# lidq92/LBDRN-MSIC

Hardware: AMD Instinct MI355X
Metric: Mpixels/s encode+decode (and bpp/PSNR parity) on D2/K5/bc64/nl2 (higher is better)
Workload: dtype f32; 1 GPU; synthetic 8-band 2048x2048 uint16 tile per step, K=5 D=2 bc=64 nl=2 bs=8192 e=10 (BASELINE.json configs[1] by default); encode fit + 16-bit weight truncation + decode; tiles_per_gpu=50, tiles_in_flight_per_gpu=4, tiles_per_launch=2, parallelism=image-sharded x1

## Files before the change

lbdrn-msic_amd/csrc/cabi.hip:

```cpp
#include <string>

#include "common.hpp"

namespace lbdrn {
const char* last_error();
bool mfma_train_supported(const lbdrn_geom& g, const lbdrn_net& net, int bs = 0);
int mfma_train_step_features(const lbdrn_geom& g, const lbdrn_net& net);
bool mfma_train_takes_groups(const lbdrn_geom& g, const lbdrn_net& net);
size_t mfma_train_workspace(const lbdrn_geom& g, const lbdrn_net& net, int bs);
int mfma_train_prepare(const lbdrn_geom& g, const lbdrn_net& net, const uint16_t* img,
                       const uint16_t* msb, int bs, void* ws, size_t ws_bytes, hipStream_t s);
int mfma_train_epoch(const lbdrn_geom& g, const lbdrn_net& net, const uint16_t* img,
                     const uint16_t* msb, const int64_t* perm, int64_t n, int bs, float* params,
                     float* m, float* v, int64_t step0, double lr, float* losses, void* ws,
                     size_t ws_bytes, hipStream_t s, bool alone);
int train_profile_mode(int mode);
size_t randperm_workspace(int64_t n, int count);
size_t plane_bound(int C, int H, int W);
size_t plane_workspace(int C, int H, int W);
int plane_encode(const uint16_t* planes, int C, int H, int W, void* body, size_t body_cap, uint64_t* body_bytes,
                 void* ws, size_t ws_bytes, hipStream_t s);
int plane_decode(const void* body, size_t body_bytes, int C, int H, int W, uint16_t* planes, int* status, void* ws,
                 size_t ws_bytes, hipStream_t s);
int64_t mt19937_jump_poly(int segment, uint32_t* out);
// ... 163 lines not shown
    if (check_geom(g) || check_net(net)) return 0;
    size_t a = generic_apply_workspace(*g, *net);
    size_t b = mfma_apply_supported(*g, *net) ? mfma_apply_workspace(*g, *net) : 0;
    return a > b ? a : b;
}

static int pick_apply(const lbdrn_geom* g, const lbdrn_net* net, int32_t path, bool* use_mfma)
{
    const bool ok = mfma_apply_supported(*g, *net);
    if (path == LBDRN_PATH_MFMA && !ok) {
        set_error("fused MFMA apply kernel does not support bc=%d nl=%d C=%d D=%d", net->bc, net->nl,
                  net->C, g->D);
        return LBDRN_E_UNSUPPORTED;
    }
    LBDRN_REQUIRE(path >= LBDRN_PATH_AUTO && path <= LBDRN_PATH_MFMA, "unknown path %d", path);
    *use_mfma = ok && path != LBDRN_PATH_GENERIC;
    return 0;
}

int lbdrn_decode_fused(const lbdrn_geom* g, const lbdrn_net* net, const uint16_t* msb,
                       const float* params, uint16_t* out, float* y_out, void* workspace,
                       size_t workspace_bytes, int32_t path, void* stream)
{
    if (int rc = check_geom(g)) return rc;
    if (int rc = check_net(net)) return rc;
    if (int rc = net_matches(g, net)) return rc;
    LBDRN_REQUIRE(msb && params && out, "msb, params and out must not be null");
    NEED_DEVICE();
    bool use_mfma = false;
    if (int rc = pick_apply(g, net, path, &use_mfma)) return rc;
    if (int rc = workspace_fits("apply", workspace, workspace_bytes, lbdrn_apply_workspace(g, net))) return rc;
    if (use_mfma)
        return mfma_decode(*g, *net, msb, params, out, y_out, workspace, workspace_bytes, (hipStream_t)stream);
    return generic_decode(*g, *net, msb, params, out, y_out, workspace, workspace_bytes, (hipStream_t)stream);
}

int lbdrn_eval_sse(const lbdrn_geom* g, const lbdrn_net* net, const uint16_t* img, const uint16_t* msb,
                   const float* params, double* sse, void* workspace, size_t workspace_bytes,
                   int32_t path, void* stream)
{
    if (int rc = check_geom(g)) return rc;
    if (int rc = check_net(net)) return rc;
    if (int rc = net_matches(g, net)) return rc;
    LBDRN_REQUIRE(img && msb && params && sse, "img, msb, params and sse must not be null");
    NEED_DEVICE();
    const bool background = (path & LBDRN_EVAL_BACKGROUND) != 0, fast = (path & LBDRN_EVAL_FAST) != 0;
    const bool x16 = fast && (path & LBDRN_EVAL_X16) != 0;
    path &= ~(LBDRN_EVAL_BACKGROUND | LBDRN_EVAL_FAST | LBDRN_EVAL_X16);
    bool use_mfma = false;
    if (int rc = pick_apply(g, net, path, &use_mfma)) return rc;
    if (int rc = workspace_fits("apply", workspace, workspace_bytes, lbdrn_apply_workspace(g, net))) return rc;
    if (use_mfma)
        return mfma_eval_sse(*g, *net, img, msb, params, sse, workspace, workspace_bytes, background, fast, x16,
                             (hipStream_t)stream);
    return generic_eval_sse(*g, *net, img, msb, params, sse, workspace, workspace_bytes, (hipStream_t)stream);
}

size_t lbdrn_train_workspace(const lbdrn_geom* g, const lbdrn_net* net, int32_t batch_size)
{
    if (check_geom(g) || check_net(net) || batch_size < 1) return 0;
    size_t a = generic_train_workspace(*net, batch_size);
    size_t b = mfma_train_supported(*g, *net, batch_size) ? mfma_train_workspace(*g, *net, batch_size) : 0;
    return a > b ? a : b;
}

int lbdrn_train_prepare(const lbdrn_geom* g, const lbdrn_net* net, const uint16_t* img,
                        const uint16_t* msb, int32_t batch_size, void* workspace, size_t workspace_bytes,
                        int32_t path, void* stream)
{
    if (int rc = check_geom(g)) return rc;
    if (int rc = check_net(net)) return rc;
    if (int rc = net_matches(g, net)) return rc;
    LBDRN_REQUIRE(img && msb && batch_size >= 1, "null pointer or bad batch size");
    LBDRN_REQUIRE(path >= LBDRN_PATH_AUTO && path <= LBDRN_PATH_MFMA, "unknown path %d", path);
    NEED_DEVICE();
    const bool ok = mfma_train_supported(*g, *net, batch_size);
    if (path == LBDRN_PATH_MFMA && !ok) {
        set_error("fused MFMA train kernel does not support this shape or minibatch size");
        return LBDRN_E_UNSUPPORTED;
    }
    if (int rc = workspace_fits("train", workspace, workspace_bytes, lbdrn_train_workspace(g, net, batch_size))) return rc;
    if (ok && path != LBDRN_PATH_GENERIC)
        return mfma_train_prepare(*g, *net, img, msb, batch_size, workspace, workspace_bytes, (hipStream_t)stream);
    return 0;
}

int lbdrn_train_epoch(const lbdrn_geom* g, const lbdrn_net* net, const uint16_t* img,
                      const uint16_t* msb, const int64_t* perm, int64_t n, int32_t batch_size,
                      float* params, float* exp_avg, float* exp_avg_sq, int64_t adam_step0, double lr,
                      float* losses, void* workspace, size_t workspace_bytes, int32_t path,
                      void* stream)
{
    if (int rc = check_geom(g)) return rc;
    if (int rc = check_net(net)) return rc;
    if (int rc = net_matches(g, net)) return rc;
    LBDRN_REQUIRE(img && msb && perm && params && exp_avg && exp_avg_sq, "null pointer");
    LBDRN_REQUIRE(n >= 0 && batch_size >= 1 && adam_step0 >= 0, "bad n/batch_size/adam_step0");
    NEED_DEVICE();
    const bool alone = (path & LBDRN_TRAIN_ALONE) != 0;
    path &= ~LBDRN_TRAIN_ALONE;
    const bool ok = mfma_train_supported(*g, *net, batch_size);
    if (path == LBDRN_PATH_MFMA && !ok) {
        set_error("fused MFMA train kernel does not support this shape or minibatch size");
        return LBDRN_E_UNSUPPORTED;
    }
    LBDRN_REQUIRE(path >= LBDRN_PATH_AUTO && path <= LBDRN_PATH_MFMA, "unknown path %d", path);
    if (int rc = workspace_fits("train", workspace, workspace_bytes, lbdrn_train_workspace(g, net, batch_size))) return rc;
    if (ok && path != LBDRN_PATH_GENERIC)
        return mfma_train_epoch(*g, *net, img, msb, perm, n, batch_size, params, exp_avg, exp_avg_sq,
                                adam_step0, lr, losses, workspace, workspace_bytes, (hipStream_t)stream, alone);
    return generic_train_epoch(*g, *net, img, msb, perm, n, batch_size, params, exp_avg, exp_avg_sq,
                               adam_step0, lr, losses, workspace, workspace_bytes, (hipStream_t)stream);
}

int lbdrn_train_group_max(void) { return 4; }

int32_t lbdrn_train_group_size(const lbdrn_geom* g, const lbdrn_net* net)
{
    if (!g || !net) return 1;
    return mfma_train_takes_groups(*g, *net) ? lbdrn_train_group_max() : 1;
}

int32_t lbdrn_train_step_features(const lbdrn_geom* g, const lbdrn_net* net)
{
    if (!g || !net) return 0;
    return mfma_train_step_features(*g, *net);
}

int lbdrn_train_epoch_group(int32_t count, const lbdrn_geom* const* g, const lbdrn_net* net, const uint16_t* const* img,
                            const uint16_t* const* msb, const int64_t* const* perm, int64_t n, int32_t batch_size,
                            float* const* params, float* const* exp_avg, float* const* exp_avg_sq, int64_t adam_step0,
                            double lr, float* const* losses, void* const* workspace, size_t workspace_bytes, int32_t path,
                            void* stream)
{
    LBDRN_REQUIRE(count >= 1 && count <= lbdrn_train_group_max(), "group of %d fits (1..%d)", count, lbdrn_train_group_max());
    LBDRN_REQUIRE(g && img && msb && perm && params && exp_avg && exp_avg_sq && workspace, "null pointer array");
    if (int rc = check_net(net)) return rc;
    for (int f = 0; f < count; ++f) {
        LBDRN_REQUIRE(g[f] && img[f] && msb[f] && perm[f] && params[f] && exp_avg[f] && exp_avg_sq[f], "null pointer (fit %d)", f);
        if (int rc = check_geom(g[f])) return rc;
        if (int rc = net_matches(g[f], net)) return rc;
        LBDRN_REQUIRE(g[f]->C == g[0]->C && g[f]->H == g[0]->H && g[f]->W == g[0]->W && g[f]->K == g[0]->K &&
                      g[f]->D == g[0]->D && g[f]->P == g[0]->P && g[f]->use_colors == g[0]->use_colors &&
                      g[f]->relative == g[0]->relative, "the fits of a group must have one shape (fit %d differs)", f);
    }
    LBDRN_REQUIRE(n >= 0 && batch_size >= 1 && adam_step0 >= 0, "bad n/batch_size/adam_step0");
    const int32_t hint = count == 1 ? (path & LBDRN_TRAIN_ALONE) : 0;
    path &= ~LBDRN_TRAIN_ALONE;
    LBDRN_REQUIRE(path >= LBDRN_PATH_AUTO && path <= LBDRN_PATH_MFMA, "unknown path %d", path);
    NEED_DEVICE();
    for (int f = 0; f < count; ++f)
        if (int rc = workspace_fits("train", workspace[f], workspace_bytes, lbdrn_train_workspace(g[f], net, batch_size))) return rc;
    if (count > 1 && path != LBDRN_PATH_GENERIC && mfma_train_supported(*g[0], *net, batch_size)) {
        const int rc = mfma_train_epoch_group(count, *g[0], *net, perm, n, batch_size, params, exp_avg, exp_avg_sq,
                                              adam_step0, lr, losses, workspace, workspace_bytes, (hipStream_t)stream, false);
        if (rc != LBDRN_E_UNSUPPORTED) return rc;
    }
    for (int f = 0; f < count; ++f)
        if (int rc = lbdrn_train_epoch(g[f], net, img[f], msb[f], perm[f], n, batch_size, params[f], exp_avg[f],
                                       exp_avg_sq[f], adam_step0, lr, losses ? losses[f] : nullptr, workspace[f],
                                       workspace_bytes, path | hint, stream))
            return rc;
    return 0;
}

int lbdrn_train_profile_mode(int32_t mode)
{
    LBDRN_REQUIRE(mode >= 0 && mode <= 5, "mode must be 0 .. 5");
    return train_profile_mode(mode);
}

size_t lbdrn_randperm_workspace(int64_t n, int32_t count)
{
    if (n < 0 || count < 1 || count > 32) return 0;
    return randperm_workspace(n, count);
}

int lbdrn_randperm(const uint64_t* seeds, int32_t count, int64_t n, int64_t* perm, void* workspace,
                   size_t workspace_bytes, void* stream)
{
    LBDRN_REQUIRE(n >= 0 && (perm || n == 0), "bad n or null output");
    NEED_DEVICE();
    return randperm_batch(seeds, count, n, perm, workspace, workspace_bytes, (hipStream_t)stream);
}

int64_t lbdrn_mt19937_jump_poly(int32_t segment, uint32_t* poly624)
{
    LBDRN_REQUIRE(poly624, "null output");
    return mt19937_jump_poly(segment, poly624);
}

size_t lbdrn_plane_bound(int32_t C, int32_t H, int32_t W) { return plane_bound(C, H, W); }
size_t lbdrn_plane_workspace(int32_t C, int32_t H, int32_t W) { return plane_workspace(C, H, W); }

int lbdrn_plane_encode(const uint16_t* planes, int32_t C, int32_t H, int32_t W, void* body, size_t body_capacity,
                       uint64_t* body_bytes, void* workspace, size_t workspace_bytes, void* stream)
{
    LBDRN_REQUIRE(C >= 1 && H >= 1 && W >= 1 && C <= 65535, "bad raster geometry");
    NEED_DEVICE();
    return plane_encode(planes, C, H, W, body, body_capacity, body_bytes, workspace, workspace_bytes,
                        (hipStream_t)stream);
}

int lbdrn_plane_decode(const void* body, size_t body_bytes, int32_t C, int32_t H, int32_t W, uint16_t* planes,
                       int32_t* status, void* workspace, size_t workspace_bytes, void* stream)
{
    LBDRN_REQUIRE(C >= 1 && H >= 1 && W >= 1 && C <= 65535, "bad raster geometry");
    NEED_DEVICE();
    return plane_decode(body, body_bytes, C, H, W, planes, status, workspace, workspace_bytes, (hipStream_t)stream);
}

int64_t lbdrn_jp2k_block_count(int32_t C, int32_t H, int32_t W) { return jp2k_block_count(C, H, W); }
size_t lbdrn_jp2k_bound(int32_t C, int32_t H, int32_t W) { return jp2k_bound(C, H, W); }
size_t lbdrn_jp2k_workspace(int32_t C, int32_t H, int32_t W) { return jp2k_workspace(C, H, W); }

int lbdrn_jp2k_encode(const uint16_t* planes, int32_t C, int32_t H, int32_t W, int32_t bits, void* out, size_t capacity,
                      size_t* nbytes, void* workspace, size_t workspace_bytes, void* stream)
{
    if (int rc = device_ok()) return rc;
    return jp2k_encode(planes, C, H, W, bits, (uint8_t*)out, capacity, nbytes, workspace, workspace_bytes, (hipStream_t)stream);
}

size_t lbdrn_weights_bound(int64_t n) { return n < 0 ? 0 : weights_bound(n); }

int lbdrn_weights_encode(const float* values, int64_t n, int32_t precision, void* out, size_t capacity, size_t* nbytes)
{
    LBDRN_REQUIRE((values || n == 0) && out && nbytes && n >= 0 && n < ((int64_t)1 << 32), "null pointer or bad count");
    LBDRN_REQUIRE(precision == 0 || (precision >= 2 && precision <= 32), "precision %d is not 0 or 2..32", precision);
    return weights_encode(values, n, precision, (uint8_t*)out, capacity, nbytes);
}

int lbdrn_weights_info(const void* stream, size_t nbytes, int64_t* n, int32_t* precision)
{
    LBDRN_REQUIRE(stream && n && precision, "null pointer");
    int prec = 0;
    const int rc = weights_info((const uint8_t*)stream, nbytes, n, &prec);
    *precision = prec;
    return rc;
}

int lbdrn_weights_decode(const void* stream, size_t nbytes, float* values, int64_t capacity)
{
    LBDRN_REQUIRE(stream && (values || capacity == 0) && capacity >= 0, "null pointer or bad capacity");
    return weights_decode((const uint8_t*)stream, nbytes, values, capacity);
}

int lbdrn_train_step(const lbdrn_net* net, const float* x, const float* t, int32_t B, float* params,
                     float* exp_avg, float* exp_avg_sq, int64_t adam_step, double lr,
                     int32_t apply_adam, float* loss, float* grads, void* workspace,
                     size_t workspace_bytes, void* stream)
{
    if (int rc = check_net(net)) return rc;
    LBDRN_REQUIRE(x && t && params, "x, t and params must not be null");
    LBDRN_REQUIRE(!apply_adam || (exp_avg && exp_avg_sq && adam_step >= 1), "Adam state missing or adam_step < 1");
    NEED_DEVICE();
    return generic_train_step(*net, x, t, B, params, exp_avg, exp_avg_sq, adam_step, lr, apply_adam,
                              loss, grads, workspace, workspace_bytes, (hipStream_t)stream);
}

}
```

lbdrn-msic_amd/csrc/common.hpp:

```cpp
#pragma once
#include <hip/hip_runtime.h>
#include <stdint.h>
#include <stdio.h>

#include <atomic>

#include "../../include/lbdrn_hip.h"

namespace lbdrn {

void set_error(const char* fmt, ...);

#define LBDRN_HIP_TRY(expr)                                                                  \
    do {                                                                                     \
        hipError_t e_ = (expr);                                                              \
        if (e_ != hipSuccess) {                                                              \
            ::lbdrn::set_error("%s failed: %s (%s:%d)", #expr, hipGetErrorString(e_), __FILE__, \
                               __LINE__);                                                    \
            return LBDRN_E_DEVICE;                                                           \
        }                                                                                    \
    } while (0)

#define LBDRN_REQUIRE(cond, ...)            \
    do {                                    \
        if (!(cond)) {                      \
            ::lbdrn::set_error(__VA_ARGS__); \
            return LBDRN_E_ARG;             \
        }                                   \
    } while (0)

#define LBDRN_LAUNCH_CHECK() LBDRN_HIP_TRY(hipGetLastError())

inline int64_t param_count(const lbdrn_net& n)
{
    int64_t c = 0;
    for (int l = 0; l < n.nl; ++l) c += (int64_t)n.bc * (l ? n.bc : n.F) + n.bc;
    return c + (int64_t)n.C * n.bc + n.C;
}
inline int64_t layer_offset(const lbdrn_net& n, int l)
{
    int64_t c = 0;
    for (int i = 0; i < l; ++i) c += (int64_t)n.bc * (i ? n.bc : n.F) + n.bc;
    return c;
}
inline int feature_dim(const lbdrn_geom& g)
{
    const int side = 2 * g.D + 1;
    return 2 * g.P + (g.use_colors ? g.C * side * side : 0);
}
inline size_t align_up(size_t x, size_t a) { return (x + a - 1) / a * a; }

template <class K>
static int configure_lds_once(K kern, int bytes, std::atomic<unsigned long long>& configured)
{
    int dev = 0;
    (void)hipGetDevice(&dev);
    const unsigned long long bit = 1ull << (dev & 63);
    if (!(configured.load(std::memory_order_relaxed) & bit)) {
        LBDRN_HIP_TRY(hipFuncSetAttribute(reinterpret_cast<const void*>(kern), hipFuncAttributeMaxDynamicSharedMemorySize, bytes));
        configured.fetch_or(bit, std::memory_order_relaxed);
    }
    return 0;
}

int check_geom(const lbdrn_geom* g);
int check_net(const lbdrn_net* n);

int generic_split_bits(const uint16_t* img, int C, int H, int W, int K, uint16_t* msb, int32_t* mx,
                       hipStream_t s);
int generic_labels(const uint16_t* img, int C, int H, int W, int K, const int64_t* idx, int64_t n,
                   float* labels, hipStream_t s);
int generic_features(const lbdrn_geom& g, const uint16_t* msb, const int64_t* idx, int64_t n,
                     int64_t first, float* out, hipStream_t s);
size_t generic_forward_workspace(const lbdrn_net& net, int64_t B);
int generic_forward(const lbdrn_net& net, const float* params, const float* x, int64_t B, float* y,
                    void* ws, size_t ws_bytes, hipStream_t s);
size_t generic_apply_workspace(const lbdrn_geom& g, const lbdrn_net& net);
int generic_decode(const lbdrn_geom& g, const lbdrn_net& net, const uint16_t* msb,
                   const float* params, uint16_t* out, float* y_out, void* ws, size_t ws_bytes,
                   hipStream_t s);
int generic_eval_sse(const lbdrn_geom& g, const lbdrn_net& net, const uint16_t* img,
                     const uint16_t* msb, const float* params, double* sse, void* ws,
                     size_t ws_bytes, hipStream_t s);
size_t generic_train_workspace(const lbdrn_net& net, int B);
int generic_train_step(const lbdrn_net& net, const float* x, const float* t, int B, float* params,
                       float* m, float* v, int64_t adam_step, double lr, int apply_adam,
                       float* loss, float* grads, void* ws, size_t ws_bytes, hipStream_t s);
size_t generic_tape_bytes(const lbdrn_net& net, int64_t B);
size_t generic_backward_workspace(const lbdrn_net& net, int64_t B);
int generic_forward_tape(const lbdrn_net& net, const float* params, const float* x, int64_t B, float* y, void* tape,
                         size_t tape_bytes, hipStream_t s);
int generic_backward(const lbdrn_net& net, const float* params, const float* x, int64_t B, const void* tape,
                     size_t tape_bytes, const float* y, const float* dy, float* grads, float* dx, void* ws,
                     size_t ws_bytes, hipStream_t s);
int generic_train_epoch(const lbdrn_geom& g, const lbdrn_net& net, const uint16_t* img,
                        const uint16_t* msb, const int64_t* perm, int64_t n, int bs, float* params,
                        float* m, float* v, int64_t step0, double lr, float* losses, void* ws,
                        size_t ws_bytes, hipStream_t s);

bool mfma_apply_supported(const lbdrn_geom& g, const lbdrn_net& net);
size_t mfma_apply_workspace(const lbdrn_geom& g, const lbdrn_net& net);
int mfma_decode(const lbdrn_geom& g, const lbdrn_net& net, const uint16_t* msb, const float* params,
                uint16_t* out, float* y_out, void* ws, size_t ws_bytes, hipStream_t s);
int mfma_eval_sse(const lbdrn_geom& g, const lbdrn_net& net, const uint16_t* img,
                  const uint16_t* msb, const float* params, double* sse, void* ws, size_t ws_bytes,
                  bool background, bool fast, bool x16, hipStream_t s);

int mfma_train_epoch_group(int count, const lbdrn_geom& g, const lbdrn_net& net, const int64_t* const* perm, int64_t n,
                           int bs, float* const* params, float* const* m, float* const* v, int64_t step0, double lr,
                           float* const* losses, void* const* ws, size_t ws_bytes, hipStream_t s, bool alone);

}
```

lbdrn-msic_amd/csrc/train_mfma.hip:

```cpp
#include <cmath>
#include <cstdlib>
#include <utility>
#include <vector>

#include "common.hpp"
#include "lbdrn_math.hpp"

namespace lbdrn {

typedef float f32x4 __attribute__((ext_vector_type(4)));

constexpr int MAX_GROUP = 4;
constexpr int TB = 32;
constexpr int TBC = 64;
constexpr int HP = 68;
constexpr int TP = 36;
constexpr int OP = 20;
constexpr int RED_SLICES = 8;
constexpr int RED_LANES = 32;
constexpr int SLAB_ROT = 4;
constexpr int TRAIN_THREADS = 512;

constexpr int WB = 64;
constexpr int WAVE_THREADS = 256;
constexpr int WOP = 16;
__host__ __device__ constexpr int wave_xp(int LQ) { return LQ == 16 ? 80 : LQ == 32 ? 144 : LQ == 48 || LQ == 52 ? 208 : 272; }
constexpr int TBC_W = 64;
constexpr int WPT = 68;

struct FeatMap {
    int Fe;
    int zP, zs2, zc;
};
__host__ __device__ __forceinline__ int feat_of_slot(int j, const FeatMap& m)
{
    if (m.zs2 == 0 || j < m.zP) return j;
    const int cj = j - m.zP, c = cj / (m.zs2 - 1), r = cj - c * (m.zs2 - 1);
    return m.zP + c * m.zs2 + r + (r >= m.zc ? 1 : 0);
}
__host__ __device__ __forceinline__ int slot_of_feat(int k, const FeatMap& m)
{
    if (m.zs2 == 0 || k < m.zP) return k;
    const int ck = k - m.zP, c = ck / m.zs2, r = ck - c * m.zs2;
    if (r == m.zc) return -1;
    return m.zP + c * (m.zs2 - 1) + r - (r > m.zc ? 1 : 0);
}

static FeatMap centre_skipping_map(const lbdrn_geom& g, const lbdrn_net& net)
{
    const int side = 2 * g.D + 1;
    if (g.use_colors && g.relative && g.D > 0 && net.F == 2 * g.P + g.C * side * side)
        return FeatMap{net.F - g.C, 2 * g.P, side * side, g.D * side + g.D};
    return FeatMap{net.F, 0, 0, 0};
}

constexpr int STEP_TILE = 0;
constexpr int STEP_STREAM = 2;

struct TrainPlan {
    FeatMap fm;
    int LQ;
    int XP;
    int NT0;
    int RP;
    int64_t NP;
    int64_t offW[5], offB[5];
    int pk_w0, pk_wh, pk_wl, pack_floats;
    int wave;
    int pk_wht, pk_wlt;
    int w_dp, w_df;
    int wave_lds_floats;
    int sl_hid, sl_out, sl_bias, slab_floats;
    int lds_x, lds_xt, lds_h, lds_ht, lds_z, lds_zt, lds_zo, lds_zot, lds_pix, lds_red, lds_floats;
};

#define STREAM_INSTANCES(X) \
    X(16, 1, 0) X(16, 2, 0)              \
    X(24, 1, 0) X(24, 2, 0) X(24, 2, 6)  \
    X(32, 1, 0) X(32, 2, 0)              \
    X(48, 1, 0) X(48, 2, 0) X(48, 2, 12) \
    X(52, 1, 0)             X(52, 2, 13) \
    X(64, 1, 0) X(64, 2, 0) X(64, 2, 16)
#define SPLIT_INSTANCES(X) X(24, 6) X(48, 12) X(64, 16) X(96, 24)
constexpr int SPLIT_WIDE_LQ = 96;
#define TILE_INSTANCES(X) X(16, 3) X(32, 3) X(52, 3)

#define X(LQ, NL, NT0C) if (lq == LQ && nl == NL && nt0 == NT0C) return NT0C;
constexpr int stream_nt0c(int lq, int nl, int nt0) { STREAM_INSTANCES(X) return 0; }
#undef X
#define X(LQ, NL, NT0C) if (nl == NL && fe <= 4 * LQ) return LQ;
constexpr int stream_lq(int fe, int nl) { STREAM_INSTANCES(X) return 0; }
#undef X
#define X(LQ, NT0C) if (lq == LQ) return NT0C;
constexpr int split_nt0c(int lq) { SPLIT_INSTANCES(X) return 0; }
#undef X
#define X(LQ, NL) static_assert(4 * LQ % 16 == 0, "16 NT0 > XP: dW0's last strip passes the X row"); if (nl == NL && F <= 4 * LQ && RP <= 4 * LQ + 4) return LQ;
constexpr int tile_lq(int F, int RP, int nl) { TILE_INSTANCES(X) return 0; }
#undef X

__host__ __device__ constexpr int stream_rp(int LQ);
static int stream_lds_total(int LQ, int NL);

static bool make_train_plan(const lbdrn_geom& g, const lbdrn_net& net, TrainPlan* out)
{
    if ((net.act != LBDRN_ACT_SINE && net.act != LBDRN_ACT_RELU) || net.bc != TBC || net.nl < 1 || net.nl > 3 || net.C > 16 || net.F < 1) return false;
    if (net.act == LBDRN_ACT_RELU && net.nl > 2) return false;
    TrainPlan p;
    p.wave = net.nl <= 2 ? STEP_STREAM : STEP_TILE;
    if (p.wave == STEP_STREAM) {
        p.fm = centre_skipping_map(g, net);
        p.LQ = stream_lq(p.fm.Fe, net.nl);
        if (!p.LQ && net.nl == 2 && p.fm.Fe <= 4 * SPLIT_WIDE_LQ) p.LQ = SPLIT_WIDE_LQ;
        if (!p.LQ) return false;
        p.NT0 = p.LQ == SPLIT_WIDE_LQ ? split_nt0c(SPLIT_WIDE_LQ) : (p.fm.Fe + 15) / 16;
        p.RP = stream_rp(p.LQ);
        p.wave_lds_floats = p.LQ == SPLIT_WIDE_LQ ? 0 : stream_lds_total(p.LQ, net.nl);
    } else {
        p.fm = FeatMap{net.F, 0, 0, 0};
        p.RP = (net.F + net.C + 3) / 4 * 4;
        p.LQ = tile_lq(net.F, p.RP, net.nl);
        if (!p.LQ) return false;
        p.NT0 = (net.F + 15) / 16;
        p.wave_lds_floats = 0;
    }
    p.XP = 4 * p.LQ + 4;
    p.NP = param_count(net);
    int64_t o = 0;
    for (int l = 0; l < net.nl; ++l) {
        int nin = l ? TBC : net.F;
        p.offW[l] = o; o += (int64_t)TBC * nin;
        p.offB[l] = o; o += TBC;
    }
    p.offW[net.nl] = o; o += (int64_t)net.C * TBC;
    p.offB[net.nl] = o;
    int k = 0;
    p.pk_w0 = k; k += 4 * p.LQ * 64;
    p.pk_wh = k; k += (net.nl - 1) * 4 * 16 * 64;
    p.pk_wl = k; k += 16 * 64;
    p.pk_wht = k; k += (net.nl - 1) * 4 * 16 * 64;
    p.pk_wlt = k; k += 16 * 64;
    p.pack_floats = k;
    p.w_dp = p.w_df = 0;
    int s = 4 * p.NT0 * 256;
    p.sl_hid = s; s += (net.nl - 1) * 16 * 256;
    p.sl_out = s; s += 4 * 256;
    p.sl_bias = s; s += net.nl * TBC + 16;
    p.slab_floats = (s + 127) / 128 * 128;
    int f = 0;
    p.lds_x = f; f += TB * p.XP;
    p.lds_xt = f; f += 16 * p.NT0 * TP;
    p.lds_h = f; f += net.nl * TB * HP;
    p.lds_ht = f; f += net.nl * TBC * TP;
    p.lds_z = f; f += net.nl * TB * HP;
    p.lds_zt = f; f += net.nl * TBC * TP;
    p.lds_zo = f; f += TB * OP;
    p.lds_zot = f; f += 16 * TP;
    p.lds_pix = f; f += TB;
    p.lds_red = f; f += 16;
    p.lds_floats = f;
    if (p.wave == STEP_TILE && (size_t)f * 4 > 160 * 1024) return false;
    *out = p;
    return true;
}

struct WidePlan;
static bool make_wide_plan(const lbdrn_geom& g, const lbdrn_net& net, WidePlan* out);
static bool wide_supported(const lbdrn_geom& g, const lbdrn_net& net);
static size_t wide_workspace(const lbdrn_geom& g, const lbdrn_net& net, int bs);

static bool slabs_addressable(const TrainPlan& p, int bs);

bool mfma_train_supported(const lbdrn_geom& g, const lbdrn_net& net, int bs)
{
    TrainPlan p;
    if (make_train_plan(g, net, &p)) return bs <= 0 || slabs_addressable(p, bs);
    return wide_supported(g, net);
}

bool mfma_train_takes_groups(const lbdrn_geom& g, const lbdrn_net& net)
{
    TrainPlan p;
    return make_train_plan(g, net, &p) && p.wave == STEP_STREAM;
}


struct TrainWsLayout {
    size_t off_rows, off_pack, off_slab, slab_bytes, off_loss, off_stage, stage_bytes, off_map, total;
};

static TrainWsLayout train_ws_layout(const lbdrn_geom& g, const lbdrn_net& net, const TrainPlan& p, int bs)
{
    TrainWsLayout L;
    size_t o = 0;
    L.off_rows = o; o += align_up((size_t)g.H * g.W * p.RP * sizeof(float), 256);
    L.off_pack = o; o += align_up((size_t)p.pack_floats * sizeof(float), 256);
    const size_t nwg = std::max((size_t)(bs + TB - 1) / TB, 2 * ((size_t)(bs + WB - 1) / WB));
    L.slab_bytes = align_up(nwg * (size_t)p.slab_floats * sizeof(float), 256);
    L.off_slab = o; o += SLAB_ROT * L.slab_bytes;
    L.off_loss = o; o += align_up(nwg * sizeof(double), 256);
    L.stage_bytes = align_up(align_up((size_t)bs, WB) * p.RP * sizeof(float), 256);
    L.off_stage = o; o += 2 * L.stage_bytes;
    L.off_map = o; o += align_up((size_t)p.slab_floats * 4 * sizeof(int), 256);
    L.total = o;
    return L;
}

static bool slabs_addressable(const TrainPlan& p, int bs)
{
    const size_t nwg = std::max((size_t)(bs + TB - 1) / TB, 2 * ((size_t)(bs + WB - 1) / WB));
    return nwg * (size_t)p.slab_floats * sizeof(float) < ((size_t)1 << 31);
}

size_t mfma_train_workspace(const lbdrn_geom& g, const lbdrn_net& net, int bs)
{
    TrainPlan p;
    if (!make_train_plan(g, net, &p)) return wide_workspace(g, net, bs);
    return train_ws_layout(g, net, p, bs).total;
}


__device__ __forceinline__ int row_source(int pos, int LQs, int F, int C, const FeatMap& fm)
{
    if (LQs == 0) return pos < fm.Fe ? feat_of_slot(pos, fm) : pos < fm.Fe + C ? F + (pos - fm.Fe) : -1;
    const int g = pos >> 4;
    if (g < (LQs >> 2)) {
        const int j = ((pos >> 2) & 3) * LQs + 4 * g + (pos & 3);
        return j < fm.Fe ? feat_of_slot(j, fm) : -1;
    }
    const int ch = pos - 4 * LQs;
    return ch < C ? F + ch : -1;
}

__global__ void __launch_bounds__(256)
    k_build_rows(lbdrn_geom g, int F, int RP, int LQs, FeatMap fm, const uint16_t* __restrict__ msb,
                 const uint16_t* __restrict__ img, float* __restrict__ rows)
{
    const int64_t HW = (int64_t)g.H * g.W;
    const int64_t e = (int64_t)blockIdx.x * blockDim.x + threadIdx.x;
    if (e >= HW * RP) return;
    const int64_t pix = e / RP;
    const int f = row_source((int)(e - pix * RP), LQs, F, g.C, fm);
    const int y = (int)(pix / g.W), x = (int)(pix - (int64_t)y * g.W);
    float v = 0.0f;
    if (f < 0) {
    } else if (f < g.P) {
        v = g.rowtab[(int64_t)y * g.P + f];
    } else if (f < 2 * g.P) {
        v = g.coltab[(int64_t)x * g.P + (f - g.P)];
    } else if (f < F) {
        const int side = 2 * g.D + 1;
        int cf = f - 2 * g.P;
        int c = cf / (side * side);
        int r = cf - c * side * side;
        int dy = r / side, dx = r - dy * side;
        const uint16_t* pl = msb + (int64_t)c * HW;
        const float mx = (float)g.msb_max;
        int yy = reflect_fast(y + dy - g.D, g.H), xx = reflect_fast(x + dx - g.D, g.W);
        v = (float)pl[(int64_t)yy * g.W + xx] / mx;
        if (g.relative && g.D > 0) v = v - (float)pl[pix] / mx;
    } else if (f < F + g.C) {
        const int mask = (1 << g.K) - 1;
        v = (float)((int)img[(int64_t)(f - F) * HW + pix] & mask) / (float)mask;
    }
    rows[e] = v;
}

constexpr int BR_TW = 32;
__global__ void __launch_bounds__(256)
    k_build_rows_tiled(lbdrn_geom g, int F, int RP, int LQs, FeatMap fm, const uint16_t* __restrict__ msb,
                       const uint16_t* __restrict__ img, float* __restrict__ rows)
{
    extern __shared__ float br_lds[];
    const int side = 2 * g.D + 1, SW = BR_TW + 2 * g.D;
    const int ncolor = F - 2 * g.P;
    float* tile = br_lds;
    int* nbo = reinterpret_cast<int*>(br_lds + g.C * side * SW);
    int* cto = nbo + ncolor;
    const int64_t HW = (int64_t)g.H * g.W;
    const int tiles_x = (g.W + BR_TW - 1) / BR_TW;
    const int y = blockIdx.x / tiles_x, x0 = (blockIdx.x - y * tiles_x) * BR_TW;
    const int tw = min(BR_TW, g.W - x0);
    const int tid = threadIdx.x;
    if (g.use_colors) {
        const float mx = (float)g.msb_max;
        const int total = g.C * side * SW;
        for (int e = tid; e < total; e += 256) {
            const int c = e / (side * SW), r = e - c * side * SW;
            const int sy = r / SW, sx = r - sy * SW;
            const int yy = reflect_fast(y + sy - g.D, g.H), xx = reflect_fast(min(x0 + sx - g.D, g.W - 1 + g.D), g.W);
            tile[e] = (float)msb[(int64_t)c * HW + (int64_t)yy * g.W + xx] / mx;
        }
        for (int k = tid; k < ncolor; k += 256) {
            const int c = k / (side * side), r = k - c * side * side;
            const int dy = r / side, dx = r - dy * side;
            nbo[k] = (c * side + dy) * SW + dx;
            cto[k] = (c * side + g.D) * SW + g.D;
        }
    }
    __syncthreads();
    const bool rel = g.relative && g.D > 0;
    int2* ptab = reinterpret_cast<int2*>(cto + ncolor);
    float* labs = reinterpret_cast<float*>(ptab + RP);
    {
        const int lmask = (1 << g.K) - 1;
        const float lmaskf = (float)lmask;
        for (int e = tid; e < g.C * BR_TW; e += 256) {
            const int c = e / BR_TW, px = e - c * BR_TW;
            labs[e] = (float)((int)img[(int64_t)c * HW + (int64_t)y * g.W + min(x0 + px, g.W - 1)] & lmask) / lmaskf;
        }
    }
    for (int pos = tid; pos < RP; pos += 256) {
        const int f = row_source(pos, LQs, F, g.C, fm);
        int2 t = make_int2(-1, 0);
        if (f < 0) {
        } else if (f < g.P) t = make_int2(-2, f);
        else if (f < 2 * g.P) t = make_int2(-3, f - g.P);
        else if (f < F) t = make_int2(nbo[f - 2 * g.P], rel ? cto[f - 2 * g.P] : -1);
        else if (f < F + g.C) t = make_int2(-4, f - F);
        ptab[pos] = t;
    }
    __syncthreads();
    float* out = rows + ((int64_t)y * g.W + x0) * RP;
    auto value = [&](int pos, int pix) -> float {
        const int2 t = ptab[pos];
        if (t.x >= 0) {
            const float nb = tile[t.x + pix];
            return t.y >= 0 ? nb - tile[t.y + pix] : nb;
        }
        if (t.x == -1) return 0.0f;
        if (t.x == -2) return g.rowtab[(int64_t)y * g.P + t.y];
        if (t.x == -3) return g.coltab[(int64_t)(x0 + pix) * g.P + t.y];
        return labs[t.y * BR_TW + pix];
    };
    if ((RP & 3) == 0) {
        const int RQ = RP >> 2;
        int pix = tid / RQ, pq = tid - pix * RQ;
        const int dp = 256 / RQ, dq = 256 - dp * RQ;
        while (pix < tw) {
            const int pos = 4 * pq;
            const float4 v = make_float4(value(pos, pix), value(pos + 1, pix), value(pos + 2, pix), value(pos + 3, pix));
            *reinterpret_cast<float4*>(out + (int64_t)pix * RP + pos) = v;
            pix += dp;
            pq += dq;
            if (pq >= RQ) { pq -= RQ; pix += 1; }
        }
    } else {
        int pix = tid / RP, pos = tid - pix * RP;
        const int dp = 256 / RP, df = 256 - dp * RP;
        for (int e = tid; pix < tw; e += 256) {
            out[e] = value(pos, pix);
            pix += dp;
            pos += df;
            if (pos >= RP) { pos -= RP; pix += 1; }
        }
    }
}

__device__ __forceinline__ int2 frag_pos(int64_t idx, const TrainPlan& p, int F, int nl, int C)
{
    if (idx < p.offB[0]) {
        int n = (int)(idx / F), k = slot_of_feat((int)(idx - (int64_t)n * F), p.fm);
        if (k < 0) return make_int2(-1, -1);
        int q = k / p.LQ, s = k - q * p.LQ;
        return make_int2(p.pk_w0 + ((((n >> 4) * (p.LQ >> 2) + (s >> 2)) * 64 + q * 16 + (n & 15)) * 4 + (s & 3)), -1);
    }
    for (int l = 1; l < nl; ++l) {
        if (idx >= p.offW[l] && idx < p.offB[l]) {
            int e = (int)(idx - p.offW[l]);
            int n = e >> 6, k = e & 63;
            if (!p.wave) {
                int sq = k & 15;
                return make_int2(p.pk_wh + (((((l - 1) * 4 + (n >> 4)) * 4 + (sq >> 2)) * 64 + (k >> 4) * 16 + (n & 15)) * 4 + (sq & 3)), -1);
            }
            const int fwd = p.pk_wh + (((((l - 1) * 4 + (n >> 4)) * 4 + (k >> 4)) * 64 + ((k >> 2) & 3) * 16 + (n & 15)) * 4 + (k & 3));
            const int bwd = p.pk_wht + (((((l - 1) * 4 + (k >> 4)) * 4 + (n >> 4)) * 64 + ((n >> 2) & 3) * 16 + (k & 15)) * 4 + (n & 3));
            return make_int2(fwd, bwd);
        }
    }
    if (idx >= p.offW[nl] && idx < p.offB[nl]) {
        int e = (int)(idx - p.offW[nl]);
        int c = e >> 6, k = e & 63;
        if (!p.wave) {
            int sq = k & 15;
            return make_int2(p.pk_wl + (((sq >> 2) * 64 + (k >> 4) * 16 + c) * 4 + (sq & 3)), -1);
        }
        const int fwd = p.pk_wl + (((k >> 4) * 64 + ((k >> 2) & 3) * 16 + c) * 4 + (k & 3));
        const int bwd = p.pk_wlt + (((k >> 4) * 64 + (c >> 2) * 16 + (k & 15)) * 4 + (c & 3));
        return make_int2(fwd, bwd);
    }
    return make_int2(-1, -1);
}

__device__ __forceinline__ int64_t slab_to_param(int e, const TrainPlan& p, int F, int nl, int C)
{
    if (e >= p.sl_bias) {
        int b = e - p.sl_bias;
        if (b < nl * TBC) return p.offB[b >> 6] + (b & 63);
        int ch = b - nl * TBC;
        return ch < C ? p.offB[nl] + ch : -1;
    }
    const int tile = e >> 8, lane = (e >> 2) & 63, r = e & 3;
    const int row = 4 * (lane >> 4) + r, col = lane & 15;
    if (e < p.sl_hid) {
        int w = tile / p.NT0, nt = tile - w * p.NT0;
        int k = 16 * nt + col;
        return k < p.fm.Fe ? p.offW[0] + (int64_t)(16 * w + row) * F + feat_of_slot(k, p.fm) : -1;
    }
    if (e < p.sl_out) {
        int t2 = tile - 4 * p.NT0;
        int l = 1 + (t2 >> 4), w = (t2 >> 2) & 3, nt = t2 & 3;
        return p.offW[l] + (int64_t)(16 * w + row) * TBC + 16 * nt + col;
    }
    int w = tile - (p.sl_out >> 8);
    return row < C ? p.offW[nl] + (int64_t)row * TBC + 16 * w + col : -1;
}

__global__ void __launch_bounds__(256)
    k_pack_train(const float* __restrict__ params, TrainPlan p, int F, int nl, int C, float* __restrict__ packed)
{
    int64_t idx = (int64_t)blockIdx.x * blockDim.x + threadIdx.x;
    if (idx >= p.NP) return;
    const int2 pos = frag_pos(idx, p, F, nl, C);
    if (pos.x >= 0) packed[pos.x] = params[idx];
    if (pos.y >= 0) packed[pos.y] = params[idx];
}

__global__ void __launch_bounds__(256)
    k_build_map(TrainPlan p, int F, int nl, int C, int4* __restrict__ map)
{
    int e = blockIdx.x * blockDim.x + threadIdx.x;
    if (e >= p.slab_floats) return;
    int64_t idx = e < p.sl_bias + nl * TBC + 16 ? slab_to_param(e, p, F, nl, C) : -1;
    const int2 pos = idx >= 0 ? frag_pos(idx, p, F, nl, C) : make_int2(-1, -1);
    map[e] = make_int4((int)idx, pos.x, pos.y, 0);
}

constexpr int RED_AUX = 0x00;
#ifdef LBDRN_TIMELINE
constexpr int TL_SLOTS = 2048;
__device__ __forceinline__ void timeline_store(unsigned long long* tl, int slot, bool drain)
{
    if (!tl || slot >= TL_SLOTS) return;
    unsigned long long t;
    if (drain) asm volatile("s_waitcnt vmcnt(0)" ::: "memory");
    asm volatile("s_memrealtime %0\n\ts_waitcnt lgkmcnt(0)" : "=s"(t)::"memory");
    tl[slot] = t;
}
#endif
struct ReduceFit {
    const float* slabs;
    float *params, *m, *v, *packed;
    const double* loss_part;
    float* loss_out;
};
struct ReduceArgs {
    ReduceFit fit[MAX_GROUP];
    unsigned long long* tl;
    int nloss;
};

__global__ void __launch_bounds__(RED_SLICES * RED_LANES)
    k_reduce_adam(ReduceArgs R, int nwg, int slab_floats, const int4* __restrict__ map, float step_size, float bc2_sqrt,
                  double loss_count, int pairs)
{
    __shared__ __attribute__((aligned(16))) float part[RED_SLICES][4 * RED_LANES];
    __builtin_amdgcn_s_setprio(3);
#ifdef LBDRN_TIMELINE
    if (threadIdx.x == 0 && blockIdx.x == 0 && blockIdx.y == 0) timeline_store(R.tl, 1, false);
#endif
    const ReduceFit& F = R.fit[blockIdx.y];
    const float* __restrict__ slabs = F.slabs;
    float* __restrict__ params = F.params;
    float* __restrict__ m = F.m;
    float* __restrict__ v = F.v;
    float* __restrict__ packed = F.packed;
    const int l16 = threadIdx.x % RED_LANES, slice = threadIdx.x / RED_LANES;
    const int base = blockIdx.x * (4 * RED_LANES);
    int4 me = make_int4(-1, -1, -1, 0);
    float pm = 0.f, pv = 0.f, pp = 0.f;
    if (threadIdx.x < 4 * RED_LANES) {
        me = map[base + threadIdx.x];
        const int j = me.x < 0 ? 0 : me.x;
        pm = m[j]; pv = v[j]; pp = params[j];
    }
    const int per = (nwg + RED_SLICES - 1) / RED_SLICES;
    const int w0 = slice * per, w1 = min(nwg, w0 + per);
    float4 acc = make_float4(0.f, 0.f, 0.f, 0.f);
    const __amdgpu_buffer_rsrc_t srs = __builtin_amdgcn_make_buffer_rsrc(const_cast<float*>(slabs), (short)0,
                                                                         (int)((size_t)nwg * (pairs ? 2 : 1) * slab_floats * 4), 0x00020000);
    const int voff = (base + 4 * l16) * 4;
    auto slab4 = [&](int slab) -> float4 {
        typedef int v4i __attribute__((ext_vector_type(4)));
        const v4i x = __builtin_amdgcn_raw_buffer_load_b128(srs, voff + slab * slab_floats * 4, 0, RED_AUX);
        return make_float4(__int_as_float(x[0]), __int_as_float(x[1]), __int_as_float(x[2]), __int_as_float(x[3]));
    };
    int w = w0;
    if (pairs) {
        for (; w + 8 <= w1; w += 8) {
            float4 t[8], o[8];
#pragma unroll
            for (int u = 0; u < 8; ++u) {
                t[u] = slab4(2 * (w + u));
                o[u] = slab4(2 * (w + u) + 1);
            }
#pragma unroll
            for (int u = 0; u < 8; ++u) { acc.x += t[u].x + o[u].x; acc.y += t[u].y + o[u].y; acc.z += t[u].z + o[u].z; acc.w += t[u].w + o[u].w; }
        }
        for (; w < w1; ++w) {
            const float4 t = slab4(2 * w), o = slab4(2 * w + 1);
            acc.x += t.x + o.x; acc.y += t.y + o.y; acc.z += t.z + o.z; acc.w += t.w + o.w;
        }
    }
    for (; w + 16 <= w1; w += 16) {
        float4 t[16];
#pragma unroll
        for (int u = 0; u < 16; ++u) t[u] = slab4(w + u);
#pragma unroll
        for (int u = 0; u < 16; ++u) { acc.x += t[u].x; acc.y += t[u].y; acc.z += t[u].z; acc.w += t[u].w; }
    }
    for (; w < w1; ++w) {
        const float4 t = slab4(w);
        acc.x += t.x; acc.y += t.y; acc.z += t.z; acc.w += t.w;
    }
    *reinterpret_cast<float4*>(&part[slice][4 * l16]) = acc;
    __syncthreads();
    if (threadIdx.x < 4 * RED_LANES && me.x >= 0) {
        float g = part[0][threadIdx.x];
#pragma unroll
        for (int s = 1; s < RED_SLICES; ++s) g += part[s][threadIdx.x];
        const float w1c = (float)(1.0 - 0.9), b2 = 0.999f, w2c = (float)(1.0 - 0.999), eps = 1e-8f;
        float mi = pm + w1c * (g - pm);
        float vi = pv * b2 + w2c * (g * g);
        float denom = __builtin_sqrtf(vi) / bc2_sqrt + eps;
        float pi = pp + (-step_size) * (mi / denom);
        m[me.x] = mi;
        v[me.x] = vi;
        params[me.x] = pi;
        if (me.y >= 0) packed[me.y] = pi;
        if (me.z >= 0) packed[me.z] = pi;
    }
    if (blockIdx.x == 0 && threadIdx.x == 0 && F.loss_out) {
        double s = 0.0;
        if (pairs) for (int k = 0; k + 1 < R.nloss; k += 2) s += F.loss_part[k] + F.loss_part[k + 1];
        else for (int k = 0; k < R.nloss; ++k) s += F.loss_part[k];
        *F.loss_out = (float)(s / loss_count);
    }
#ifdef LBDRN_TIMELINE
    __syncthreads();
    if (threadIdx.x == 0 && blockIdx.y == 0) timeline_store(R.tl, 514 + blockIdx.x, true);
#endif
}

static void launch_reduce(const ReduceArgs& R, int blocks, int count, bool pairs, int nwg, int slab_floats, const int4* map,
                          float step_size, float bc2_sqrt, double loss_count, hipStream_t s)
{
    k_reduce_adam<<<dim3((unsigned)blocks, (unsigned)count), RED_SLICES * RED_LANES, 0, s>>>(R, nwg, slab_floats, map, step_size, bc2_sqrt,
                                                                                            loss_count, pairs ? 1 : 0);
}


struct TrainFit {
    const float* rows;
    const int64_t* perm;
    const float* params;
    const float* packed;
    float* slabs;
    double* loss_part;
};
struct TrainArgs {
    lbdrn_net net;
    TrainPlan p;
    int64_t npix;
    int batch_n;
    float inv;
    TrainFit fit[MAX_GROUP];
    const float* stage_in;
    float* stage_out;
    const int64_t* perm_next;
    int next_n;
    int touch_row_bytes;
    unsigned long long* stamps;
    unsigned long long* tl;
};
constexpr int TOUCH_ROW_BYTES = 256;


#ifdef LBDRN_TRAIN_STAMPS
#define STAMP(k)                                                                        \
    do {                                                                                \
        __builtin_amdgcn_sched_barrier(0);                                              \
        asm volatile("s_memtime %0\n\ts_waitcnt lgkmcnt(0)" : "=s"(stamp[k])::"memory"); \
        __builtin_amdgcn_sched_barrier(0);                                              \
    } while (0)
#else
#define STAMP(k)
#endif

#define MFMA16(a, b, c) __builtin_amdgcn_mfma_f32_16x16x4f32((a), (b), (c), 0, 0, 0)

typedef int v4i32 __attribute__((ext_vector_type(4)));
struct WtBuf {
    __amdgpu_buffer_rsrc_t r;
    float* base;
    __device__ __forceinline__ WtBuf(float* p, size_t bytes) : base(p)
    {
        r = __builtin_amdgcn_make_buffer_rsrc(p, (short)0, (int)bytes, 0x00020000);
    }
    __device__ __forceinline__ void store_plain(int float_off, float a, float b, float c, float d) const
    {
        *reinterpret_cast<float4*>(base + float_off) = make_float4(a, b, c, d);
    }
    __device__ __forceinline__ void store(int float_off, float a, float b, float c, float d) const
    {
        v4i32 v = {__float_as_int(a), __float_as_int(b), __float_as_int(c), __float_as_int(d)};
        __builtin_amdgcn_raw_buffer_store_b128(v, r, float_off * 4, 0, 16 );
    }
};

template <int N>
__device__ __forceinline__ void lds_load(const float* src, float (&dst)[N])
{
#pragma unroll
    for (int g = 0; g < N / 4; ++g) {
        float4 v = *reinterpret_cast<const float4*>(src + 4 * g);
        dst[4 * g] = v.x; dst[4 * g + 1] = v.y; dst[4 * g + 2] = v.z; dst[4 * g + 3] = v.w;
    }
}

template <int LQ, int NL>
__global__ void __launch_bounds__(TRAIN_THREADS, 2) k_train_mfma(TrainArgs A)
{
    extern __shared__ __attribute__((aligned(16))) float lds[];
    const TrainPlan& p = A.p;
    const TrainFit& Ft = A.fit[0];
    const int tid = threadIdx.x, lane = tid & 63, w8 = tid >> 6;
    const int w = w8 & 3, st = w8 >> 2;
    const int i = lane & 15, q = lane >> 4;
    const int C = A.net.C, F = A.net.F;
    constexpr int XP = 4 * LQ + 4;
    float* Xs = lds + p.lds_x;
    float* XT = lds + p.lds_xt;
    float* Hs = lds + p.lds_h;
    float* HT = lds + p.lds_ht;
    float* Zs = lds + p.lds_z;
    float* ZT = lds + p.lds_zt;
    float* Zo = lds + p.lds_zo;
    float* ZoT = lds + p.lds_zot;
    int* pixs = reinterpret_cast<int*>(lds + p.lds_pix);
    double* red = reinterpret_cast<double*>(lds + p.lds_red);
    const int wg = blockIdx.x;
    const int first = wg * TB;
    const int nvalid = min(TB, A.batch_n - first);
    const int srow = i + 16 * st;
    float* slab = Ft.slabs + (size_t)wg * p.slab_floats;
    const WtBuf slabw(slab, (size_t)p.slab_floats * 4);
#ifdef LBDRN_TRAIN_STAMPS
    unsigned long long stamp[16] = {};
    asm volatile("s_memrealtime %0\n\ts_waitcnt lgkmcnt(0)" : "=s"(stamp[12])::"memory");
#endif
    STAMP(0);

    const bool staged = A.stage_in != nullptr;
    int64_t mypix = 0;
    if (!staged && tid < TB) mypix = Ft.perm[first + min(tid, nvalid - 1)];
    const int rs = tid >> 4, rsub = tid & 15;
    constexpr int NLD = (XP / 4 + 15) / 16;
    const int rp4 = p.RP >> 2;
    float4 v[NLD];
    if (staged) {
        const float* src = A.stage_in + ((size_t)wg * TB + rs) * p.RP;
#pragma unroll
        for (int u = 0; u < NLD; ++u) v[u] = *reinterpret_cast<const float4*>(src + 4 * min(rsub + 16 * u, rp4 - 1));
    }
    int64_t nextpix = -1;
    if (A.stage_out && first < A.next_n) nextpix = A.perm_next[min(first + rs, A.next_n - 1)];

    float a0[LQ];
    {
        const float4* wf0 = reinterpret_cast<const float4*>(Ft.packed + p.pk_w0) + (size_t)w * (LQ / 4) * 64 + lane;
#pragma unroll
        for (int g = 0; g < LQ / 4; ++g) {
            const float4 t = wf0[g * 64];
            a0[4 * g] = t.x; a0[4 * g + 1] = t.y; a0[4 * g + 2] = t.z; a0[4 * g + 3] = t.w;
        }
    }
    float ah[NL > 1 ? NL - 1 : 1][16];
#pragma unroll
    for (int l = 1; l < NL; ++l) {
        const float4* wfh = reinterpret_cast<const float4*>(Ft.packed + p.pk_wh) + (size_t)((l - 1) * 4 + w) * 4 * 64 + lane;
#pragma unroll
        for (int g = 0; g < 4; ++g) {
            const float4 t = wfh[g * 64];
            ah[l - 1][4 * g] = t.x; ah[l - 1][4 * g + 1] = t.y; ah[l - 1][4 * g + 2] = t.z; ah[l - 1][4 * g + 3] = t.w;
        }
    }
    float al[16];
    {
        const float4* wfl = reinterpret_cast<const float4*>(Ft.packed + p.pk_wl) + lane;
#pragma unroll
        for (int g = 0; g < 4; ++g) {
            const float4 t = wfl[g * 64];
            al[4 * g] = t.x; al[4 * g + 1] = t.y; al[4 * g + 2] = t.z; al[4 * g + 3] = t.w;
        }
    }
    float atl[4];
#pragma unroll
    for (int s = 0; s < 4; ++s) {
        int ch = 4 * q + s;
        atl[s] = ch < C ? Ft.params[p.offW[NL] + (int64_t)ch * TBC + 16 * w + i] : 0.0f;
    }
    float ath[NL > 1 ? NL - 1 : 1][16];
#pragma unroll
    for (int l = 1; l < NL; ++l)
#pragma unroll
        for (int s = 0; s < 16; ++s) ath[l - 1][s] = Ft.params[p.offW[l] + (int64_t)(16 * q + s) * TBC + 16 * w + i];
    f32x4 bias[NL];
#pragma unroll
    for (int l = 0; l < NL; ++l) {
        float4 b4 = *reinterpret_cast<const float4*>(Ft.params + p.offB[l] + 16 * w + 4 * q);
        bias[l][0] = b4.x; bias[l][1] = b4.y; bias[l][2] = b4.z; bias[l][3] = b4.w;
// ... 107 lines not shown
#pragma unroll
        for (int r = 0; r < 4; ++r) ZoT[(4 * q + r) * TP + srow] = dzo[r];
        for (int o = 32; o > 0; o >>= 1) lsum += __shfl_down(lsum, o);
        if (lane == 0) red[st] = lsum;
    }
    __syncthreads();
    if (tid == 0) Ft.loss_part[wg] = red[0] + red[1];
    STAMP(6);
    if (nextpix >= 0) {
        const WtBuf stw(A.stage_out + (size_t)wg * TB * p.RP, (size_t)TB * p.RP * 4);
#pragma unroll
        for (int u = 0; u < NLD; ++u) {
            const int c4 = rsub + 16 * u;
            if (c4 < rp4) stw.store(rs * p.RP + 4 * c4, vnext[u].x, vnext[u].y, vnext[u].z, vnext[u].w);
        }
    }

    auto backprop_store = [&](int l) {
        float dz[4];
#pragma unroll
        for (int r = 0; r < 4; ++r) dz[r] = (acc[r] * cs[l][r]) * 30.0f;
        *reinterpret_cast<float4*>(Zs + (size_t)l * TB * HP + srow * HP + 16 * w + 4 * q) =
            make_float4(dz[0], dz[1], dz[2], dz[3]);
#pragma unroll
        for (int r = 0; r < 4; ++r) ZT[(size_t)l * TBC * TP + (16 * w + 4 * q + r) * TP + srow] = dz[r];
    };

    {
        const f32x4 zero = {0.f, 0.f, 0.f, 0.f};
        acc = zero;
        float bz[4];
        lds_load<4>(Zo + srow * OP + 4 * q, bz);
#pragma unroll
        for (int s = 0; s < 4; ++s) acc = MFMA16(atl[s], bz[s], acc);
        backprop_store(NL - 1);
    }
    __syncthreads();
#pragma unroll
    for (int l = NL - 1; l >= 1; --l) {
        const f32x4 zero = {0.f, 0.f, 0.f, 0.f};
        acc = zero;
        float bz[16];
        lds_load<16>(Zs + (size_t)l * TB * HP + srow * HP + 16 * q, bz);
#pragma unroll
        for (int s = 0; s < 16; ++s) acc = MFMA16(ath[l - 1][s], bz[s], acc);
        backprop_store(l - 1);
        __syncthreads();
    }
    STAMP(7);

    auto grad_tiles = [&](const float* zt, const float* bt, int ntiles, int out, bool early) {
        float az[8];
        lds_load<8>(zt + (16 * w + i) * TP + 8 * q, az);
        for (int nt = st; nt < ntiles; nt += 4) {
            const int nt1 = nt + 2;
            const bool two = nt1 < ntiles;
            float b0[8], b1[8];
            lds_load<8>(bt + (16 * nt + i) * TP + 8 * q, b0);
            lds_load<8>(bt + (16 * (two ? nt1 : nt) + i) * TP + 8 * q, b1);
            const f32x4 zero = {0.f, 0.f, 0.f, 0.f};
            f32x4 g0 = zero, g1 = zero;
#pragma unroll
            for (int s = 0; s < 8; ++s) {
                g0 = MFMA16(az[s], b0[s], g0);
                g1 = MFMA16(az[s], b1[s], g1);
            }
            if (early) {
                slabw.store(out + ((w * ntiles + nt) * 64 + lane) * 4, g0[0], g0[1], g0[2], g0[3]);
                if (two) slabw.store(out + ((w * ntiles + nt1) * 64 + lane) * 4, g1[0], g1[1], g1[2], g1[3]);
            } else {
                slabw.store_plain(out + ((w * ntiles + nt) * 64 + lane) * 4, g0[0], g0[1], g0[2], g0[3]);
                if (two) slabw.store_plain(out + ((w * ntiles + nt1) * 64 + lane) * 4, g1[0], g1[1], g1[2], g1[3]);
            }
        }
    };
    grad_tiles(ZT, XT, p.NT0, 0, true);
    STAMP(10);
#pragma unroll
    for (int l = 1; l < NL; ++l)
        grad_tiles(ZT + (size_t)l * TBC * TP, HT + (size_t)(l - 1) * TBC * TP, 4, p.sl_hid + (l - 1) * 16 * 256, false);
    if (st == 0) {
        float az[8], bv[8];
        lds_load<8>(ZoT + i * TP + 8 * q, az);
        lds_load<8>(HT + (size_t)(NL - 1) * TBC * TP + (16 * w + i) * TP + 8 * q, bv);
        const f32x4 zero = {0.f, 0.f, 0.f, 0.f};
        f32x4 g0 = zero, g1 = zero;
#pragma unroll
        for (int s = 0; s < 8; s += 2) {
            g0 = MFMA16(az[s], bv[s], g0);
            g1 = MFMA16(az[s + 1], bv[s + 1], g1);
        }
        slabw.store_plain(p.sl_out + (w * 64 + lane) * 4, g0[0] + g1[0], g0[1] + g1[1], g0[2] + g1[2], g0[3] + g1[3]);
    }
    STAMP(11);
    for (int u = tid; u < NL * TBC + 16; u += TRAIN_THREADS) {
        float zz[TB];
        lds_load<TB>(u < NL * TBC ? ZT + (size_t)u * TP : ZoT + (size_t)(u - NL * TBC) * TP, zz);
        float v = 0.0f;
#pragma unroll
        for (int s = 0; s < TB; ++s) v += zz[s];
        slab[p.sl_bias + u] = v;
    }
    for (int u = p.sl_bias + NL * TBC + 16 + tid; u < p.slab_floats; u += TRAIN_THREADS) slab[u] = 0.0f;
    STAMP(8);
#ifdef LBDRN_TRAIN_STAMPS
    asm volatile("s_waitcnt vmcnt(0)" ::: "memory");
    STAMP(9);
    asm volatile("s_memrealtime %0\n\ts_waitcnt lgkmcnt(0)" : "=s"(stamp[13])::"memory");
    if (tid == 0 && A.stamps)
        for (int k = 0; k < 16; ++k) A.stamps[(size_t)wg * 16 + k] = stamp[k];
#endif
}

__device__ __forceinline__ float train_sigmoid(float z) { return fast_sigmoid(z); }
template <int ACT> __device__ __forceinline__ void train_act(float z, float& h, float& d);
template <int ACT> __device__ __forceinline__ float train_act_back(float dh, float d)
{
    if constexpr (ACT == LBDRN_ACT_RELU) return d != 0.0f ? dh : 0.0f;
    else return (dh * d) * 30.0f;
}
__device__ __forceinline__ void train_sincos(float x, float& sn, float& cs) { fast_sincos(x, sn, cs); }
template <int ACT> __device__ __forceinline__ void train_act(float z, float& h, float& d)
{
    if constexpr (ACT == LBDRN_ACT_RELU) { h = z > 0.0f ? z : 0.0f; d = z > 0.0f ? 1.0f : 0.0f; }
    else train_sincos(30.0f * z, h, d);
}

__device__ __forceinline__ float row_sum16(float x)
{
    x += __int_as_float(__builtin_amdgcn_update_dpp(0, __float_as_int(x), 0x111, 0xf, 0xf, true));
    x += __int_as_float(__builtin_amdgcn_update_dpp(0, __float_as_int(x), 0x112, 0xf, 0xf, true));
    x += __int_as_float(__builtin_amdgcn_update_dpp(0, __float_as_int(x), 0x114, 0xf, 0xf, true));
    x += __int_as_float(__builtin_amdgcn_update_dpp(0, __float_as_int(x), 0x118, 0xf, 0xf, true));
    return x;
}

__device__ __forceinline__ float wave_sum(float x)
{
    const int xi = __float_as_int(row_sum16(x));
    const float a = __int_as_float(__builtin_amdgcn_readlane(xi, 15)), b = __int_as_float(__builtin_amdgcn_readlane(xi, 31));
    const float c = __int_as_float(__builtin_amdgcn_readlane(xi, 47)), d = __int_as_float(__builtin_amdgcn_readlane(xi, 63));
    return (a + b) + (c + d);
}

static thread_local int g_prof_mode = 0;
int train_profile_mode(int mode)
{
    g_prof_mode = mode;
    return 0;
}

#include "train_stream.inc"

static int stream_lds_total(int LQ, int NL) { return stream_lds(LQ, NL).total; }
#define X(LQ, NL, NT0C) static_assert(stream_lds(LQ, NL).total * 4 <= 160 * 1024, "k_train_stream's LDS map passes 160 KB");
STREAM_INSTANCES(X)
#undef X

#include "train_split.inc"

#include "train_wide.inc"

int mfma_train_step_features(const lbdrn_geom& g, const lbdrn_net& net)
{
    TrainPlan p;
    if (make_train_plan(g, net, &p)) return p.fm.Fe;
    WidePlan wp;
    return make_wide_plan(g, net, &wp) ? wide_plan_features(wp) : net.F;
}

static bool wide_supported(const lbdrn_geom& g, const lbdrn_net& net)
{
    WidePlan p;
    return make_wide_plan(g, net, &p);
}
static size_t wide_workspace(const lbdrn_geom& g, const lbdrn_net& net, int bs)
{
    WidePlan p;
    if (!make_wide_plan(g, net, &p)) return 0;
    return wide_ws_layout(g, net, p, bs).total;
}


template <int LQ, int NL>
static int launch_train(const TrainArgs& A, int nwg, hipStream_t s)
{
    auto kern = k_train_mfma<LQ, NL>;
    const size_t lds_bytes = (size_t)A.p.lds_floats * 4;
    static std::atomic<unsigned long long> configured{0};
    if (int rc = configure_lds_once(kern, 160 * 1024, configured)) return rc;
    kern<<<nwg, TRAIN_THREADS, lds_bytes, s>>>(A);
    LBDRN_LAUNCH_CHECK();
    return 0;
}

template <int LQ, int NL, int NT0C, int ACT>
static int launch_stream(const TrainArgs& A, int nwg, int count, hipStream_t s)
{
    auto kern = k_train_stream<LQ, NL, STREAM_PD, NT0C, ACT>;
    static std::atomic<unsigned long long> configured{0};
    if (int rc = configure_lds_once(kern, A.p.wave_lds_floats * 4, configured)) return rc;
    kern<<<dim3((unsigned)nwg, (unsigned)count), STREAM_THREADS, (size_t)A.p.wave_lds_floats * 4, s>>>(A);
    LBDRN_LAUNCH_CHECK();
    return 0;
}

template <int LQ, int NT0C, int ACT>
static int launch_split(const TrainArgs& A, int nwg, int count, hipStream_t s)
{
    auto kern = k_train_split<LQ, NT0C, ACT>;
    constexpr int bytes = split_lds(LQ).total * 4;
    static std::atomic<unsigned long long> configured{0};
    if (int rc = configure_lds_once(kern, bytes, configured)) return rc;
    kern<<<dim3((unsigned)nwg, (unsigned)count), WAVE_THREADS, (size_t)bytes, s>>>(A);
    LBDRN_LAUNCH_CHECK();
    return 0;
}

static bool split_available(const TrainPlan& p, const lbdrn_net& net)
{
    return p.wave == STEP_STREAM && net.nl == 2 && split_nt0c(p.LQ) == p.NT0;
}
static bool split_only(const TrainPlan& p) { return p.LQ == SPLIT_WIDE_LQ; }

static int dispatch_train(const TrainArgs& A, int nwg, int count, bool split, hipStream_t s)
{
    const TrainPlan& p = A.p;
    const int nl = A.net.nl, nt0c = stream_nt0c(p.LQ, nl, p.NT0);
    const bool relu = A.net.act == LBDRN_ACT_RELU;
#define ACTS(launch, ...) return relu ? launch<__VA_ARGS__, LBDRN_ACT_RELU>(A, nwg, count, s) : launch<__VA_ARGS__, LBDRN_ACT_SINE>(A, nwg, count, s);
#define SPLIT(lq, c) if (split && p.LQ == lq && p.NT0 == c) ACTS(launch_split, lq, c)
#define STREAM(lq, n, c) if (!split && p.wave == STEP_STREAM && p.LQ == lq && nl == n && nt0c == c) ACTS(launch_stream, lq, n, c)
#define TILE(lq, n) if (!split && p.wave == STEP_TILE && p.LQ == lq && nl == n) return launch_train<lq, n>(A, nwg, s);
    SPLIT_INSTANCES(SPLIT) STREAM_INSTANCES(STREAM) TILE_INSTANCES(TILE)
#undef ACTS
#undef SPLIT
#undef STREAM
#undef TILE
    set_error("no fused step is built for LQ = %d, nl = %d, NT0 = %d%s", p.LQ, nl, p.NT0, split ? " (k_train_split)" : "");
    return LBDRN_E_UNSUPPORTED;
}

int mfma_train_prepare(const lbdrn_geom& g, const lbdrn_net& net, const uint16_t* img,
                       const uint16_t* msb, int bs, void* ws, size_t ws_bytes, hipStream_t s)
{
    TrainPlan p;
    size_t need = 0, off_rows = 0;
    int LQs = 0;
    if (make_train_plan(g, net, &p)) {
        const TrainWsLayout L = train_ws_layout(g, net, p, bs);
        need = L.total; off_rows = L.off_rows;
        if (p.wave == STEP_STREAM) LQs = p.LQ;
    } else {
        WidePlan wp;
        if (!make_wide_plan(g, net, &wp)) {
            set_error("shape not supported by the MFMA train kernels");
            return LBDRN_E_UNSUPPORTED;
        }
        const WideWsLayout L = wide_ws_layout(g, net, wp, bs);
        need = L.total; off_rows = L.off_rows;
        p.RP = wp.RP;
        p.fm = wp.fm;
    }
    if (!ws || ws_bytes < need) {
        set_error("train workspace too small: %zu < %zu", ws_bytes, need);
        return LBDRN_E_WORKSPACE;
    }
    float* rows = (float*)((char*)ws + off_rows);
    const int64_t total = (int64_t)g.H * g.W * p.RP;
    LBDRN_REQUIRE((total + 255) / 256 < ((int64_t)1 << 31), "image too large for one launch");
    const int side = 2 * g.D + 1;
    const size_t ncol = (size_t)std::max(net.F - 2 * g.P, 0);
    const size_t tile_lds = ((size_t)g.C * side * (BR_TW + 2 * g.D) + 2 * ncol + 2 * (size_t)p.RP + (size_t)g.C * BR_TW) * 4;
    const int64_t nblk = (int64_t)g.H * ((g.W + BR_TW - 1) / BR_TW);
    if (tile_lds <= 48 * 1024 && g.D < g.H && g.D < g.W && nblk < ((int64_t)1 << 31)) {
        k_build_rows_tiled<<<(unsigned)nblk, 256, tile_lds, s>>>(g, net.F, p.RP, LQs, p.fm, msb, img, rows);
    } else {
        k_build_rows<<<(unsigned)((total + 255) / 256), 256, 0, s>>>(g, net.F, p.RP, LQs, p.fm, msb, img, rows);
    }
    LBDRN_LAUNCH_CHECK();
    return 0;
}


int mfma_train_epoch_group(int count, const lbdrn_geom& g, const lbdrn_net& net, const int64_t* const* perm, int64_t n,
                           int bs, float* const* params, float* const* m, float* const* v, int64_t step0, double lr,
                           float* const* losses, void* const* ws, size_t ws_bytes, hipStream_t s, bool alone)
{
    TrainArgs A;
    if (!make_train_plan(g, net, &A.p)) {
        if (count != 1) { set_error("groups of fits run on the bc = 64 fused step only"); return LBDRN_E_UNSUPPORTED; }
        return wide_train_epoch(g, net, perm[0], n, bs, params[0], m[0], v[0], step0, lr, losses ? losses[0] : nullptr,
                                ws[0], ws_bytes, s);
    }
    if (count < 1 || count > MAX_GROUP || (count > 1 && A.p.wave != STEP_STREAM)) {
        set_error("a group of %d fits is not supported by this shape's train kernel", count);
        return LBDRN_E_UNSUPPORTED;
    }
    if (!slabs_addressable(A.p, bs)) {
        set_error("minibatch of %d rows: one step's gradient slabs pass 2 GiB, the fused step does not address them", bs);
        return LBDRN_E_UNSUPPORTED;
    }
    const TrainWsLayout L = train_ws_layout(g, net, A.p, bs);
    if (ws_bytes < L.total) {
        set_error("train workspace too small: %zu < %zu", ws_bytes, L.total);
        return LBDRN_E_WORKSPACE;
    }
    A.net = net; A.npix = (int64_t)g.H * g.W;
    ReduceArgs R;
    for (int f = 0; f < MAX_GROUP; ++f) {
        const int k = f < count ? f : 0;
        if (!ws[k]) { set_error("null train workspace"); return LBDRN_E_WORKSPACE; }
        float* packed = (float*)((char*)ws[k] + L.off_pack);
        A.fit[f].rows = (float*)((char*)ws[k] + L.off_rows);
        A.fit[f].params = params[k];
        A.fit[f].packed = packed;
        A.fit[f].slabs = (float*)((char*)ws[k] + L.off_slab);
        A.fit[f].loss_part = (double*)((char*)ws[k] + L.off_loss);
        A.fit[f].perm = perm[k];
        R.fit[f].slabs = A.fit[f].slabs; R.fit[f].params = params[k]; R.fit[f].m = m[k]; R.fit[f].v = v[k];
        R.fit[f].packed = packed; R.fit[f].loss_part = A.fit[f].loss_part; R.fit[f].loss_out = nullptr;
        if (f < count) {
            LBDRN_HIP_TRY(hipMemsetAsync(packed, 0, (size_t)A.p.pack_floats * sizeof(float), s));
            k_pack_train<<<(unsigned)((A.p.NP + 255) / 256), 256, 0, s>>>(params[k], A.p, net.F, net.nl, net.C, packed);
            LBDRN_LAUNCH_CHECK();
        }
    }
    int4* map = (int4*)((char*)ws[0] + L.off_map);
    k_build_map<<<(unsigned)((A.p.slab_floats + 255) / 256), 256, 0, s>>>(A.p, net.F, net.nl, net.C, map);
    LBDRN_LAUNCH_CHECK();
    float* stage[2] = {(float*)((char*)ws[0] + L.off_stage), (float*)((char*)ws[0] + L.off_stage + L.stage_bytes)};
    A.stamps = nullptr;
#ifdef LBDRN_TRAIN_STAMPS
    const int max_wg = (bs + TB - 1) / TB;
    LBDRN_HIP_TRY(hipMalloc(&A.stamps, (size_t)max_wg * 8 * 16 * sizeof(unsigned long long)));
#endif
    A.tl = nullptr; R.tl = nullptr;
#ifdef LBDRN_TIMELINE
    const int tl_steps = (int)((n + bs - 1) / bs);
    unsigned long long* tl_buf = nullptr;
    {
        LBDRN_HIP_TRY(hipMalloc(&tl_buf, (size_t)tl_steps * TL_SLOTS * sizeof(unsigned long long)));
        LBDRN_HIP_TRY(hipMemset(tl_buf, 0, (size_t)tl_steps * TL_SLOTS * sizeof(unsigned long long)));
    }
#endif
    const int rows_per_wg = A.p.wave == STEP_STREAM ? WB : TB;
    const bool split = (alone && count == 1 && split_available(A.p, net)) || split_only(A.p);
    const int red_blocks = A.p.slab_floats / (4 * RED_LANES);
    int64_t step = step0;
    int si = 0;
    for (int64_t first = 0; first < n; first += bs, ++si) {
        const int B = (int)std::min<int64_t>(bs, n - first);
        const int nwg = (B + rows_per_wg - 1) / rows_per_wg;
        for (int f = 0; f < MAX_GROUP; ++f) {
            const int k = f < count ? f : 0;
            A.fit[f].perm = perm[k] + first;
            R.fit[f].loss_out = (f < count && losses && losses[k]) ? losses[k] + si : nullptr;
        }
        A.batch_n = B;
        for (int f = 0; f < MAX_GROUP; ++f) {
            const int k = f < count ? f : 0;
            A.fit[f].slabs = (float*)((char*)ws[k] + L.off_slab + (size_t)(si % SLAB_ROT) * L.slab_bytes);
            R.fit[f].slabs = A.fit[f].slabs;
        }
#ifdef LBDRN_TIMELINE
        A.tl = tl_buf + (size_t)TL_SLOTS * si; R.tl = A.tl;
#endif
        A.inv = 1.0f / ((float)B * (float)net.C);
        const int64_t nextB = std::max<int64_t>(0, std::min<int64_t>(bs, n - first - bs));
        A.stage_in = si > 0 ? stage[si & 1] : nullptr;
        A.stage_out = nextB > 0 ? stage[(si + 1) & 1] : nullptr;
        if (A.p.wave == STEP_STREAM) A.stage_in = nullptr, A.stage_out = nullptr;
        A.perm_next = perm[0] + first + bs;
        A.next_n = (int)nextB;
        A.touch_row_bytes = (alone && count == 1) ? TOUCH_ROW_BYTES : 0;
        const bool split_now = split && (B >= 2 || split_only(A.p));
        auto train_launch = [&]() { return dispatch_train(A, split_now ? 2 * nwg : nwg, count, split_now, s); };
        if (int rc = train_launch()) return rc;
        if (g_prof_mode == 2)
            if (int rc = train_launch()) return rc;
        ++step;
        const double bc1 = 1.0 - std::pow(0.9, (double)step), bc2 = 1.0 - std::pow(0.999, (double)step);
        R.nloss = split_now ? 2 * nwg : nwg;
        if (g_prof_mode != 3 && g_prof_mode != 4)
                launch_reduce(R, red_blocks, count, split_now, nwg, A.p.slab_floats, map, (float)(lr / bc1), (float)std::sqrt(bc2), (double)B * net.C, s);
        if (g_prof_mode == 1) {
            ReduceArgs R0 = R;
            for (int f = 0; f < MAX_GROUP; ++f) R0.fit[f].loss_out = nullptr;
            launch_reduce(R0, red_blocks, count, split_now, nwg, A.p.slab_floats, map, 0.0f, (float)std::sqrt(bc2), (double)B * net.C, s);
        }
        LBDRN_LAUNCH_CHECK();
    }
#ifdef LBDRN_TIMELINE
    {
        LBDRN_HIP_TRY(hipStreamSynchronize(s));
        std::vector<unsigned long long> h((size_t)tl_steps * TL_SLOTS);
        LBDRN_HIP_TRY(hipMemcpy(h.data(), tl_buf, h.size() * sizeof(unsigned long long), hipMemcpyDeviceToHost));
        (void)hipFree(tl_buf);
        double tr = 0, g1 = 0, rd = 0, g2 = 0; int cnt = 0;
        auto last = [&](int k, int lo, int hi) { unsigned long long m = 0; for (int j = lo; j < hi; ++j) m = std::max(m, h[(size_t)k * TL_SLOTS + j]); return m; };
        for (int k = 8; k + 1 < tl_steps; ++k) {
            const unsigned long long ts = h[(size_t)k * TL_SLOTS], rs = h[(size_t)k * TL_SLOTS + 1], te = last(k, 2, 514), re = last(k, 514, TL_SLOTS);
            const unsigned long long ts2 = h[(size_t)(k + 1) * TL_SLOTS];
            tr += (double)(te - ts); g1 += (double)((long long)(rs - te)); rd += (double)(re - rs); g2 += (double)((long long)(ts2 - re));
            ++cnt;
        }
        const double u = 0.01 / std::max(cnt, 1);
        fprintf(stderr, "[lbdrn timeline] per step over %d steps: train first start -> last end %.2f us | -> reduce starts %.2f | reduce %.2f | -> next train starts %.2f | step %.2f us\n",
                cnt, tr * u, g1 * u, rd * u, g2 * u, (tr + g1 + rd + g2) * u);
    }
#endif
#ifdef LBDRN_TRAIN_STAMPS
    if (A.p.wave == STEP_STREAM) {
        LBDRN_HIP_TRY(hipStreamSynchronize(s));
        const int nw = ((int)std::min<int64_t>(bs, n) + rows_per_wg - 1) / rows_per_wg * 4 * count * (split ? 2 : 1);
        std::vector<unsigned long long> h((size_t)nw * 16);
        LBDRN_HIP_TRY(hipMemcpy(h.data(), A.stamps, h.size() * sizeof(unsigned long long), hipMemcpyDeviceToHost));
        (void)hipFree(A.stamps);
        double d[14] = {}, clk = 0, span = 0;
        unsigned long long t0min = ~0ull, t1max = 0;
        for (int k = 0; k < nw; ++k) {
            for (int j = 1; j <= 13; ++j) d[j] += (double)(h[k * 16 + j] - h[k * 16 + j - 1]);
            clk += (double)(h[k * 16 + 13] - h[k * 16 + 0]) / (double)(h[k * 16 + 15] - h[k * 16 + 14]) * 100.0;
            span += (double)(h[k * 16 + 13] - h[k * 16 + 0]);
            t0min = std::min(t0min, h[k * 16 + 14]);
            t1max = std::max(t1max, h[k * 16 + 15]);
        }
        if (split)
            fprintf(stderr, "[lbdrn stamps, split kernel] clock %.0f MHz; wave lifetime %.0f cycles; first start -> last end %.2f us; "
                            "mean cycles: requests out %.0f | layer 0 (waits for W0 and the rows in it) %.0f | act0 %.0f | barrier, h0 read %.0f | hidden + act1 %.0f | "
                            "barrier, h1 read %.0f | out + loss %.0f | dh1, dz1 parked %.0f | barrier, dh0, dz0 parked %.0f | barrier, gradient operands read %.0f | "
                            "gradient products, stores, bias sums %.0f | drain %.0f\n",
                    clk / nw, span / nw, (double)(t1max - t0min) / 100.0, d[1] / nw, d[2] / nw, d[3] / nw, d[4] / nw, d[5] / nw, d[6] / nw,
                    d[7] / nw, d[8] / nw, d[9] / nw, d[10] / nw, (d[11] + d[12]) / nw, d[13] / nw);
        else
        fprintf(stderr, "[lbdrn stamps, stream kernel] clock %.0f MHz; wave lifetime %.0f cycles; first start -> last end %.2f us; "
                        "mean cycles: indices + first requests out %.0f | first stage landed %.0f | layer 0 under the stream %.0f | all landed, barrier %.0f | "
                        "act0 %.0f | hidden+act %.0f | out+loss %.0f | backward %.0f | barrier 3 %.0f | dW0 strips %.0f | dW tail+hidden %.0f | "
                        "bias sums %.0f | drain %.0f\n",
                clk / nw, span / nw, (double)(t1max - t0min) / 100.0, d[1] / nw, d[2] / nw, d[3] / nw, d[4] / nw, d[5] / nw, d[6] / nw,
                d[7] / nw, d[8] / nw, d[9] / nw, d[10] / nw, d[11] / nw, d[12] / nw, d[13] / nw);
    } else {
        LBDRN_HIP_TRY(hipStreamSynchronize(s));
        std::vector<unsigned long long> h((size_t)max_wg * 16);
        LBDRN_HIP_TRY(hipMemcpy(h.data(), A.stamps, h.size() * sizeof(unsigned long long), hipMemcpyDeviceToHost));
        (void)hipFree(A.stamps);
        double sum[12] = {}, d10 = 0, d11 = 0, d8 = 0, clk = 0;
        for (int wq = 0; wq < max_wg; ++wq) {
            for (int k = 1; k < 10; ++k)
                if (k != 8) sum[k] += (double)(h[wq * 16 + k] - h[wq * 16 + (k == 9 ? 8 : k - 1)]);
            d10 += (double)(h[wq * 16 + 10] - h[wq * 16 + 7]);
            d11 += (double)(h[wq * 16 + 11] - h[wq * 16 + 10]);
            d8 += (double)(h[wq * 16 + 8] - h[wq * 16 + 11]);
            clk += (double)(h[wq * 16 + 9] - h[wq * 16 + 0]) / (double)(h[wq * 16 + 13] - h[wq * 16 + 12]) * 100.0;
        }
        fprintf(stderr, "[lbdrn stamps] in-kernel clock %.0f MHz; mean cycles/phase: perm %.0f rows %.0f L0 %.0f act0 %.0f "
                        "hidden %.0f out+loss %.0f backprop %.0f dW0 %.0f dWhid+out %.0f bias %.0f drain %.0f\n",
                clk / max_wg, sum[1] / max_wg, sum[2] / max_wg, sum[3] / max_wg, sum[4] / max_wg, sum[5] / max_wg,
                sum[6] / max_wg, sum[7] / max_wg, d10 / max_wg, d11 / max_wg, d8 / max_wg, sum[9] / max_wg);
    }
#endif
    return 0;
}

int mfma_train_epoch(const lbdrn_geom& g, const lbdrn_net& net, const uint16_t* img,
                     const uint16_t* msb, const int64_t* perm, int64_t n, int bs, float* params,
                     float* m, float* v, int64_t step0, double lr, float* losses, void* ws,
                     size_t ws_bytes, hipStream_t s, bool alone)
{
    return mfma_train_epoch_group(1, g, net, &perm, n, bs, &params, &m, &v, step0, lr, &losses, &ws, ws_bytes, s, alone);
}

}
```

lbdrn-msic_amd/csrc/train_split.inc:

```
constexpr int SPB = 32;
constexpr int SP_HP = 68;
constexpr int SP_OP = 20;
constexpr int SP_PT = 36;
constexpr int SP_SM = 40;

constexpr int SP_RING = 12;
__host__ __device__ constexpr bool split_ring(int LQ) { return LQ > 64; }
__host__ __device__ constexpr int split_w0_groups(int LQ) { return split_ring(LQ) ? SP_RING : LQ / 4; }
__host__ __device__ constexpr int split_small_through(int k, int SPI) { return k * SPI < SP_SM / 4 ? k * SPI : SP_SM / 4; }

struct SplitLds { int w0, sm, x, xt, h0, red, idx, bias, h1, e, zo, zt, total; };
__host__ __device__ constexpr SplitLds split_lds(int LQ)
{
    SplitLds L{};
    const int G0 = LQ / 4, RG = split_w0_groups(LQ);
    int o = 0;
    const int over = 2 * SPB * SP_HP + SPB * SP_OP + 2 * 64 * SP_PT;
    L.w0 = o; o += RG * 4 * 256 > over ? RG * 4 * 256 : over;
    L.sm = o; o += SP_SM * 256;
    L.xt = (G0 + 1) * SGP + 16;
    L.x = o; o += 2 * L.xt;
    L.h0 = o; o += SPB * SP_HP;
    L.red = o; o += 4 + 4 * 16 + 12;
    L.idx = o; o += 4 * 256;
    L.bias = o; o += 4 * 64;
    L.total = o;
    int a = L.w0;
    L.h1 = a; a += SPB * SP_HP;
    L.e = a; a += SPB * SP_HP;
    L.zo = a; a += SPB * SP_OP;
    L.zt = a; a += 2 * 64 * SP_PT;
    if (a > L.sm) L.total = -1;
    return L;
}

__device__ __forceinline__ float split_sum8(float x)
{
    x += __int_as_float(__builtin_amdgcn_update_dpp(0, __float_as_int(x), 0x111, 0xf, 0xf, true));
    x += __int_as_float(__builtin_amdgcn_update_dpp(0, __float_as_int(x), 0x112, 0xf, 0xf, true));
    x += __int_as_float(__builtin_amdgcn_update_dpp(0, __float_as_int(x), 0x118, 0xf, 0xf, true));
    return x;
}
__host__ __device__ constexpr int split_slot(int r) { return (r & ~5) | ((r & 1) << 2) | ((r >> 2) & 1); }

__host__ __device__ constexpr int split_row_requests(int lo, int hi, int u)
{
    int c = 0;
    for (int g = lo; g < hi; ++g) c += (g & 1) == u;
    return c;
}

template <int LQ, int NT0C, int ACT>
__global__ void __launch_bounds__(WAVE_THREADS, 1) k_train_split(TrainArgs A)
{
    extern __shared__ __attribute__((aligned(16))) float lds[];
    const TrainPlan& p = A.p;
    const TrainFit& F = A.fit[blockIdx.y];
    constexpr int NL = 2, G0 = LQ / 4, NGR = G0 + 1, HP = SP_HP, OP = SP_OP, PT = SP_PT, RPM = stream_rp(LQ);
    constexpr SplitLds L = split_lds(LQ);
    static_assert(L.total > 0 && L.total * 4 <= 160 * 1024, "LDS map does not fit");
    static_assert(16 * NT0C == 4 * LQ && G0 >= 4, "the first layer's strips fill its slots");
    constexpr int NFS = NT0C / 4, REM = NT0C % 4, NIT = NFS + REM, GA = split_w0_groups(LQ) / 2;
    static_assert(NFS >= 1 && REM <= 2, "strip counts of the shapes this is instantiated for");
    constexpr int SPI = (SP_SM / 4 + G0 - 2) / (G0 - 1);
    constexpr bool RING = split_ring(LQ);
    constexpr int RG = split_w0_groups(LQ), HR = RG / 2, W0B = RG - GA;
    static_assert(!RING || (G0 == 2 * RG && GA == HR), "the ring holds half of W_0, its quarters land one behind the other");
    const int tid = threadIdx.x, lane = tid & 63;
    const int wv = __builtin_amdgcn_readfirstlane(tid >> 6);
    const int st = wv >> 1, uh = wv & 1;
    const int i = lane & 15, q = lane >> 4;
    const int C = A.net.C;
    const float* W0s = lds + L.w0;
    const float* SMs = lds + L.sm;
    const float* Xs = lds + L.x;
    float* H0 = lds + L.h0;
    float* H1 = lds + L.h1;
    float* E = lds + L.e;
    float* Zo = lds + L.zo;
    float* ZT = lds + L.zt;
    float* red = lds + L.red;
    const unsigned lds0 = (unsigned)(size_t)(__attribute__((address_space(3))) void*)lds;
    const int wg = blockIdx.x, grp = wg >> 1, par = wg & 1;
    const int qb = (i >> 2) & 1, jr = (i & 3) + 4 * (i >> 3);
    const int rho = 16 * (2 * st + qb) + 2 * jr + par;
    const int grow = grp * WB + rho;
    const bool live = grow < A.batch_n;
    const int srow = 16 * st + i;
    const int sig = 8 * (2 * st + qb) + jr;
    const int t0 = 2 * uh;
    float* slab = F.slabs + (size_t)wg * p.slab_floats;
    const WtBuf slabw(slab, (size_t)p.slab_floats * 4);
#ifdef LBDRN_TRAIN_STAMPS
    unsigned long long stamp[16] = {};
    asm volatile("s_memrealtime %0\n\ts_waitcnt lgkmcnt(0)" : "=s"(stamp[14])::"memory");
#endif
#ifdef LBDRN_TIMELINE
    if (lane == 0 && wv == 0 && wg == 0 && blockIdx.y == 0) timeline_store(A.tl, 0, false);
#endif
    STAMP(0);

    {
        const void* a0 = F.perm; const void* a1 = F.params; const void* a2 = F.packed; const void* a3 = F.rows;
        int b0 = p.pk_w0, b1 = p.pk_wh, b2 = p.pk_wht, b3 = p.pk_wl, b4 = p.pk_wlt, b5 = A.batch_n;
        long long c0 = p.offB[0], c1 = p.offB[1], c2 = p.offB[2], c3 = A.npix;
        asm volatile("" ::"s"(a0), "s"(a1), "s"(a2), "s"(a3), "s"(b0), "s"(b1), "s"(b2), "s"(b3), "s"(b4), "s"(b5), "s"(c0), "s"(c1), "s"(c2), "s"(c3));
    }
    if constexpr (RING) {
        const int64_t* isrc = F.perm + min(grp * WB + lane, A.batch_n - 1);
        stream_dma_dword(reinterpret_cast<const float*>(isrc), lds0 + 4u * (unsigned)(L.idx + 256 * wv));
    } else {
        const int64_t* isrc = F.perm + min(grp * WB + 2 * (lane & 31), A.batch_n - 2);
        stream_dma(reinterpret_cast<const float*>(isrc), lds0 + 4u * (unsigned)(L.idx + 256 * wv));
    }
    {
        const int l = wv < 3 ? wv : 2, n = l < 2 ? 64 : C;
        const float* bsrc = F.params + p.offB[l] + min(lane, n - 1);
        stream_dma_dword(bsrc, lds0 + 4u * (unsigned)(L.bias + 64 * wv));
    }
    const float* fsrc = F.packed + lane * 4;
    auto w0_requests = [&](int g_lo, int g_hi) {
#pragma unroll
        for (int g = g_lo; g < g_hi; ++g)
            stream_dma(fsrc + p.pk_w0 + 256 * (wv * G0 + g), lds0 + 4u * (unsigned)(L.w0 + ((g % RG) * 4 + wv) * 256));
    };
    w0_requests(0, GA);
    stream_wait_vm<GA + 1>();
    int64_t raw;
    if constexpr (RING) {
        raw = reinterpret_cast<const int*>(lds + L.idx + 256 * wv)[min(grow, A.batch_n - 1) - grp * WB];
    } else {
        const int g = min(grow, A.batch_n - 1), l = (g - grp * WB) >> 1;
        const int pos = 2 * l + (g - min(grp * WB + 2 * l, A.batch_n - 2));
        raw = reinterpret_cast<const int64_t*>(lds + L.idx + 256 * wv)[pos];
    }
    const int pix = (int)(raw < 0 ? 0 : (raw >= A.npix ? A.npix - 1 : raw));
    const float* rsrc = F.rows + (size_t)__shfl(pix, 16 * q + split_slot(lane >> 2)) * RPM + 4 * (lane & 3);
    auto row_requests = [&](int g_lo, int g_hi) {
#pragma unroll
        for (int g = g_lo; g < g_hi; ++g)
            if ((g & 1) == uh) stream_dma(rsrc + 16 * g, lds0 + 4u * (unsigned)(L.x + st * L.xt + g * SGP));
    };
    row_requests(0, GA);
    w0_requests(GA, RG);
    row_requests(GA, NGR);
    auto small_request = [&](int b) {
        const int blk = 4 * b + wv;
        const int src = blk < 16 ? p.pk_wh + 256 * blk : blk < 32 ? p.pk_wht + 256 * (blk - 16) : blk < 36 ? p.pk_wl + 256 * (blk - 32) : p.pk_wlt + 256 * (blk - 36);
        stream_dma(fsrc + src, lds0 + 4u * (unsigned)(L.sm + 256 * blk));
    };
    long long touched = 0;
    if (A.next_n > 0 && wv == 0 && lane < 8) touched = F.perm[A.batch_n + min(grp * WB + 8 * lane, A.next_n - 1)];
    STAMP(1);
    constexpr int ROWS_B0 = split_row_requests(GA, NGR, 0), ROWS_B1 = split_row_requests(GA, NGR, 1);
    if (uh == 0) stream_wait_vm<W0B + ROWS_B0>(); else stream_wait_vm<W0B + ROWS_B1>();
    stream_barrier();
    STAMP(2);

    auto sel4 = [](const float4& x, int e) -> float { return e == 0 ? x.x : e == 1 ? x.y : e == 2 ? x.z : x.w; };
    f32x4 bias0[2], bias1[2], bias_last;
    {
        const float* B = lds + L.bias;
#pragma unroll
        for (int tt = 0; tt < 2; ++tt) {
            const float4 b4 = *reinterpret_cast<const float4*>(B + 16 * (t0 + tt) + 4 * q);
            const float4 c4 = *reinterpret_cast<const float4*>(B + 64 + 16 * (t0 + tt) + 4 * q);
            bias0[tt][0] = b4.x; bias0[tt][1] = b4.y; bias0[tt][2] = b4.z; bias0[tt][3] = b4.w;
            bias1[tt][0] = c4.x; bias1[tt][1] = c4.y; bias1[tt][2] = c4.z; bias1[tt][3] = c4.w;
        }
        const float4 l4 = *reinterpret_cast<const float4*>(B + 128 + 4 * q);
        bias_last[0] = 4 * q + 0 < C ? l4.x : 0.0f; bias_last[1] = 4 * q + 1 < C ? l4.y : 0.0f;
        bias_last[2] = 4 * q + 2 < C ? l4.z : 0.0f; bias_last[3] = 4 * q + 3 < C ? l4.w : 0.0f;
    }
    f32x4 acc[2] = {bias0[0], bias0[1]};
    {
        const float* wbase = W0s + t0 * 256 + lane * 4;
        const float* xbase = Xs + st * L.xt + (4 * split_slot(i) + q) * 4;
        float4 aq[2][2], bq[2];
        auto reads = [&](int g) {
            aq[g & 1][0] = *reinterpret_cast<const float4*>(wbase + (g % RG) * 1024);
            aq[g & 1][1] = *reinterpret_cast<const float4*>(wbase + (g % RG) * 1024 + 256);
            bq[g & 1] = *reinterpret_cast<const float4*>(xbase + g * SGP);
        };
        auto mfmas = [&](int g) {
#pragma unroll
            for (int e = 0; e < 4; ++e)
#pragma unroll
                for (int tt = 0; tt < 2; ++tt) acc[tt] = MFMA16(sel4(aq[g & 1][tt], e), sel4(bq[g & 1], e), acc[tt]);
        };
        reads(0);
#pragma unroll
        for (int g = 1; g < G0; ++g) {
            if (g == GA) {
                stream_wait_vm<((GA - 1) * SPI < SP_SM / 4 ? (GA - 1) * SPI : SP_SM / 4)>();
                stream_barrier();
            }
            if constexpr (RING) {
                if (g == GA + 1 || g == 2 * HR + 1) {
                    asm volatile("s_waitcnt lgkmcnt(0)" ::: "memory");
                    stream_barrier();
                    const int q0 = g == GA + 1 ? 2 * HR : 3 * HR;
                    w0_requests(q0, q0 + HR);
                }
                if (g == 2 * HR) {
                    stream_wait_vm<split_small_through(2 * HR - 1, SPI) - split_small_through(GA, SPI)>();
                    stream_barrier();
                }
                if (g == 3 * HR) {
                    stream_wait_vm<split_small_through(3 * HR - 1, SPI) - split_small_through(2 * HR, SPI)>();
                    stream_barrier();
                }
            }
#pragma unroll
            for (int b = (g - 1) * SPI; b < g * SPI; ++b)
                if (b < SP_SM / 4) small_request(b);
            reads(g);
            mfmas(g - 1);
#pragma unroll
            for (int k = 0; k < 3; ++k) {
                __builtin_amdgcn_sched_group_barrier(0x100, 1, 0);
                __builtin_amdgcn_sched_group_barrier(0x008, 2, 0);
            }
            __builtin_amdgcn_sched_group_barrier(0x008, 2, 0);
            __builtin_amdgcn_sched_barrier(0);
        }
        mfmas(G0 - 1);
        __builtin_amdgcn_sched_barrier(0);
    }
    const float4 lab = *reinterpret_cast<const float4*>(Xs + st * L.xt + G0 * SGP + (4 * split_slot(i) + q) * 4);
    STAMP(3);
    float hf[4][4];
    f32x4 cs[NL][2];
    auto activate = [&](int l, float* H) {
#pragma unroll
        for (int tt = 0; tt < 2; ++tt) {
            float sn[4];
#pragma unroll
            for (int r = 0; r < 4; ++r) {
                float co;
                train_act<ACT>(acc[tt][r], sn[r], co);
                cs[l][tt][r] = co;
            }
            *reinterpret_cast<float4*>(H + srow * HP + 16 * (t0 + tt) + 4 * q) = make_float4(sn[0], sn[1], sn[2], sn[3]);
        }
    };
    auto all_units = [&](const float* H, float (&dst)[4][4]) {
#pragma unroll
        for (int t = 0; t < 4; ++t) {
            const float4 x = *reinterpret_cast<const float4*>(H + srow * HP + 16 * t + 4 * q);
            dst[t][0] = x.x; dst[t][1] = x.y; dst[t][2] = x.z; dst[t][3] = x.w;
        }
    };
    auto small = [&](int blk) -> float4 { return *reinterpret_cast<const float4*>(SMs + 256 * blk + lane * 4); };
    activate(0, H0);
    stream_wait_vm<0>();
    __syncthreads();
    all_units(H0, hf);
    float4 wh[2][4];
#pragma unroll
    for (int tt = 0; tt < 2; ++tt)
#pragma unroll
        for (int tk = 0; tk < 4; ++tk) wh[tt][tk] = small((t0 + tt) * 4 + tk);
    STAMP(4);

    acc[0] = bias1[0]; acc[1] = bias1[1];
#pragma unroll
    for (int tk = 0; tk < 4; ++tk)
#pragma unroll
        for (int r = 0; r < 4; ++r)
#pragma unroll
            for (int tt = 0; tt < 2; ++tt) acc[tt] = MFMA16(sel4(wh[tt][tk], r), hf[tk][r], acc[tt]);
    float4 wl[4], wlt[2];
#pragma unroll
    for (int tk = 0; tk < 4; ++tk) wl[tk] = small(32 + tk);
#pragma unroll
    for (int tt = 0; tt < 2; ++tt) wlt[tt] = small(36 + t0 + tt);
    activate(1, H1);
    STAMP(5);
    __syncthreads();
    all_units(H1, hf);
    STAMP(6);

    float dzo[4];
    {
        f32x4 oe = bias_last, oo = {0.f, 0.f, 0.f, 0.f};
#pragma unroll
        for (int tk = 0; tk < 4; ++tk) {
            const float4 x = wl[tk];
            oe = MFMA16(x.x, hf[tk][0], oe);
            oo = MFMA16(x.y, hf[tk][1], oo);
            oe = MFMA16(x.z, hf[tk][2], oe);
            oo = MFMA16(x.w, hf[tk][3], oo);
        }
        const float labv[4] = {lab.x, lab.y, lab.z, lab.w};
        float lsum = 0.0f;
#pragma unroll
        for (int r = 0; r < 4; ++r) {
            const bool ok = live && (4 * q + r) < C;
            const float y = train_sigmoid(oe[r] + oo[r]);
            const float d = y - ((4 * q + r) < C ? labv[r] : 0.0f);
            lsum += ok ? d * d : 0.0f;
            dzo[r] = ok ? ((2.0f * d) * A.inv) * (y * (1.0f - y)) : 0.0f;
        }
        if (uh == 0) {
            *reinterpret_cast<float4*>(Zo + srow * OP + 4 * q) = make_float4(dzo[0], dzo[1], dzo[2], dzo[3]);
            const int li = __float_as_int(split_sum8(lsum));
            auto rl = [&](int l) { return __int_as_float(__builtin_amdgcn_readlane(li, l)); };
            const float l0 = (rl(11) + rl(27)) + (rl(43) + rl(59)), l1 = (rl(15) + rl(31)) + (rl(47) + rl(63));
            if (lane == 0) { red[2 * st] = l0; red[2 * st + 1] = l1; }
            float bs[4];
#pragma unroll
            for (int r = 0; r < 4; ++r) bs[r] = split_sum8(dzo[r]);
            if (i == 11 || i == 15)
                *reinterpret_cast<float4*>(red + 4 + 16 * (2 * st + (i == 15)) + 4 * q) = make_float4(bs[0], bs[1], bs[2], bs[3]);
        }
    }
    STAMP(7);

    float dzf[4][4], dzm[2][4];
    auto backprop = [&](int l) {
#pragma unroll
        for (int tt = 0; tt < 2; ++tt)
#pragma unroll
            for (int r = 0; r < 4; ++r) {
                dzm[tt][r] = train_act_back<ACT>(acc[tt][r], cs[l][tt][r]);
                ZT[(size_t)l * 64 * PT + (16 * (t0 + tt) + 4 * q + r) * PT + sig] = dzm[tt][r];
            }
    };
    float4 wht[2][4];
    {
        const f32x4 zero = {0.f, 0.f, 0.f, 0.f};
        acc[0] = zero; acc[1] = zero;
#pragma unroll
        for (int s4 = 0; s4 < 4; ++s4)
#pragma unroll
            for (int tt = 0; tt < 2; ++tt) acc[tt] = MFMA16(sel4(wlt[tt], s4), dzo[s4], acc[tt]);
#pragma unroll
        for (int tt = 0; tt < 2; ++tt)
#pragma unroll
            for (int to = 0; to < 4; ++to) wht[tt][to] = small(16 + (t0 + tt) * 4 + to);
        backprop(1);
#pragma unroll
        for (int tt = 0; tt < 2; ++tt)
            *reinterpret_cast<float4*>(E + srow * HP + 16 * (t0 + tt) + 4 * q) = make_float4(dzm[tt][0], dzm[tt][1], dzm[tt][2], dzm[tt][3]);
    }
    STAMP(8);
    __syncthreads();
    all_units(E, dzf);
    __builtin_amdgcn_sched_barrier(0);

    const int w = wv;
    const int rq = 16 * (q >> 1) + 4 * (q & 1);
    auto ldcol = [&](const float* base, int pitch, float (&dst)[8]) {
#pragma unroll
        for (int j = 0; j < 8; ++j) dst[j] = base[(rq + (j & 3) + 8 * (j >> 2)) * pitch];
    };
    auto ldx = [&](int nt, float (&dst)[8]) {
        const int f = 16 * nt + i;
        const int kq = f / LQ, fl = f - kq * LQ;
        const float* base = Xs + (q >> 1) * L.xt + (fl >> 2) * SGP + kq * 4 + (fl & 3);
#pragma unroll
        for (int j = 0; j < 8; ++j) dst[j] = base[16 * split_slot(4 * (q & 1) + (j & 3) + 8 * (j >> 2))];
    };
    auto ldrow8 = [&](const float* row, float (&dst)[8]) {
#pragma unroll
        for (int g = 0; g < 2; ++g) {
            const float4 x = *reinterpret_cast<const float4*>(row + 4 * g);
            dst[4 * g] = x.x; dst[4 * g + 1] = x.y; dst[4 * g + 2] = x.z; dst[4 * g + 3] = x.w;
        }
    };
    auto put = [&](int off, const f32x4& g) {
        slabw.store(off + lane * 4, g[0], g[1], g[2], g[3]);
    };
    const f32x4 zero4 = {0.f, 0.f, 0.f, 0.f};
    const float* ZT1 = ZT + 64 * PT;
    float az[4][8], a1[4][8], azw[8], a1w[8], ao[8], bo[8], bh[8], bb[NFS][8], br[REM > 0 ? REM : 1][8];
    auto item = [&](auto n_) {
        constexpr int n = decltype(n_)::value;
        if constexpr (n < NFS) ldx(w + 4 * n, bb[n]);
        else if constexpr (n < NIT) ldx(4 * NFS + (n - NFS), br[n - NFS]);
    };
#pragma unroll
    for (int t = 0; t < 4; ++t) ldrow8(ZT1 + (16 * t + i) * PT + 8 * q, a1[t]);
    ldrow8(ZT1 + (16 * w + i) * PT + 8 * q, a1w);
    ldcol(Zo + i, OP, ao);
    ldcol(H1 + 16 * w + i, HP, bo);
    ldcol(H0 + 16 * w + i, HP, bh);
    item(std::integral_constant<int, 0>{});
    {
        acc[0] = zero4; acc[1] = zero4;
#pragma unroll
        for (int to = 0; to < 4; ++to)
#pragma unroll
            for (int r = 0; r < 4; ++r)
#pragma unroll
                for (int tt = 0; tt < 2; ++tt) acc[tt] = MFMA16(sel4(wht[tt][to], r), dzf[to][r], acc[tt]);
        stream_deal<32, 32, 0>();
        backprop(0);
    }
    STAMP(9);
    __syncthreads();
    if (tid == 0) F.loss_part[wg] = ((double)red[0] + (double)red[1]) + ((double)red[2] + (double)red[3]);
    STAMP(10);
#pragma unroll
    for (int t = 0; t < 4; ++t) ldrow8(ZT + (16 * t + i) * PT + 8 * q, az[t]);
    ldrow8(ZT + (16 * w + i) * PT + 8 * q, azw);
    item(std::integral_constant<int, 1>{});
    f32x4 go = zero4, g1[4] = {zero4, zero4, zero4, zero4};
#pragma unroll
    for (int j = 0; j < 8; ++j) {
        go = MFMA16(ao[j], bo[j], go);
#pragma unroll
        for (int t = 0; t < 4; ++t) g1[t] = MFMA16(a1[t][j], bh[j], g1[t]);
    }
    stream_deal<40, (NIT > 1 ? 18 : 10), 0>();
    f32x4 gs[2][4];
    stream_for<NFS>([&](auto k_) {
        constexpr int k = decltype(k_)::value;
#pragma unroll
        for (int t = 0; t < 4; ++t) gs[k & 1][t] = zero4;
        item(std::integral_constant<int, k + 2>{});
#pragma unroll
        for (int j = 0; j < 8; ++j)
#pragma unroll
            for (int t = 0; t < 4; ++t) gs[k & 1][t] = MFMA16(az[t][j], bb[k][j], gs[k & 1][t]);
        if constexpr (k == 0) {
            put(p.sl_out + w * 256, go);
#pragma unroll
            for (int t = 0; t < 4; ++t) put(p.sl_hid + (t * 4 + w) * 256, g1[t]);
            stream_deal<32, (k + 2 < NIT ? 8 : 0), 5>();
        } else {
#pragma unroll
            for (int t = 0; t < 4; ++t) put((t * NT0C + w + 4 * (k - 1)) * 256, gs[(k - 1) & 1][t]);
            stream_deal<32, (k + 2 < NIT ? 8 : 0), 4>();
        }
    });
    if constexpr (REM > 0) {
        f32x4 grem[REM];
#pragma unroll
        for (int r = 0; r < REM; ++r) grem[r] = zero4;
#pragma unroll
        for (int j = 0; j < 8; ++j)
#pragma unroll
            for (int r = 0; r < REM; ++r) grem[r] = MFMA16(azw[j], br[r][j], grem[r]);
#pragma unroll
        for (int t = 0; t < 4; ++t) put((t * NT0C + w + 4 * (NFS - 1)) * 256, gs[(NFS - 1) & 1][t]);
        stream_deal<REM * 8, 0, 4>();
#pragma unroll
        for (int r = 0; r < REM; ++r) put((w * NT0C + 4 * NFS + r) * 256, grem[r]);
    } else {
#pragma unroll
        for (int t = 0; t < 4; ++t) put((t * NT0C + w + 4 * (NFS - 1)) * 256, gs[(NFS - 1) & 1][t]);
    }
    {
        float s0 = 0.f, s1 = 0.f;
#pragma unroll
        for (int j = 0; j < 8; ++j) { s0 += azw[j]; s1 += a1w[j]; }
        s0 += __shfl_xor(s0, 16); s1 += __shfl_xor(s1, 16);
        s0 += __shfl_xor(s0, 32); s1 += __shfl_xor(s1, 32);
        if (lane < 16) {
            slab[p.sl_bias + 16 * w + lane] = s0;
            slab[p.sl_bias + TBC_W + 16 * w + lane] = s1;
        }
    }
    if (w == 3 && lane < 16)
        slab[p.sl_bias + NL * TBC_W + lane] = (red[4 + lane] + red[20 + lane]) + (red[36 + lane] + red[52 + lane]);
    asm volatile("" ::"v"(touched));
    STAMP(11); STAMP(12);
#ifdef LBDRN_TIMELINE
    if (lane == 0 && uh == 0 && blockIdx.y == 0) timeline_store(A.tl, 2 + 2 * wg + st, true);
#endif
#ifdef LBDRN_TRAIN_STAMPS
    asm volatile("s_waitcnt vmcnt(0)" ::: "memory");
    STAMP(13);
    asm volatile("s_memrealtime %0\n\ts_waitcnt lgkmcnt(0)" : "=s"(stamp[15])::"memory");
    if (lane == 0 && A.stamps)
        for (int k = 0; k < 16; ++k) A.stamps[(((size_t)blockIdx.y * gridDim.x + wg) * 4 + wv) * 16 + k] = stamp[k];
#endif
}
```

lbdrn-msic_amd/csrc/train_stream.inc:

```
constexpr int SGP = 260;
__host__ __device__ constexpr int stream_groups(int LQ) { return LQ / 4 + 1; }
__host__ __device__ constexpr int stream_rp(int LQ) { return 16 * stream_groups(LQ); }
__host__ __device__ constexpr int stream_wpx(int LQ)
{
    const int n = stream_groups(LQ) * SGP;
    return n + ((16 - n % 32) + 32) % 32;
}
constexpr int SHP = 68, SOP = 20;
constexpr int SHSZ = WB * SHP + 48;
constexpr int SZOSZ = WB * SOP + 48;
constexpr int SZTSZ = TBC_W * WPT;

constexpr int SRED = 8 + 2 * 64;
struct StreamLds { int x, stage, h0, red, h1, zo, zt, wh, wht, idx, total, small; };
__host__ __device__ constexpr StreamLds stream_lds(int LQ, int NL)
{
    StreamLds L{};
    const int G0 = LQ / 4, NST = (G0 + 2) / 2;
    L.x = 0;
    L.stage = 4 * stream_wpx(LQ);
    const int stage_end = L.stage + 4 * G0 * 256;
    const bool alias = 2 * (NST - 1) - 1 >= (SHSZ + SRED + 1023) / 1024 - 1;
    int r = alias ? L.stage + ((SHSZ + SRED + 3) & ~3) : L.stage;
    L.h1 = r; r += (NL - 1) * SHSZ;
    L.zo = r; r += SZOSZ;
    L.zt = r; r += NL * SZTSZ;
    const int small_floats = (NL - 1) * 16 * 256;
    int total = r > stage_end ? r : stage_end;
    L.small = 0;
    if (NL > 1) {
        const int wht = r > stage_end + small_floats ? r : stage_end + small_floats;
        const int h0_extra = alias ? 0 : SHSZ + SRED;
        if ((wht + small_floats + h0_extra) * 4 <= 160 * 1024) {
            L.small = 1;
            L.wh = stage_end;
            L.wht = wht;
            total = wht + small_floats;
        }
    }
    if (alias) { L.h0 = L.stage; L.red = L.stage + SHSZ; }
    else { L.h0 = total; L.red = total + SHSZ; total += SHSZ + SRED; }
    L.idx = total; total += 256;
    L.total = total;
    return L;
}

__host__ __device__ constexpr int stream_row_cnt(int LQ, int s)
{
    int c = 0;
    for (int g = 2 * s; g < 2 * s + 2; ++g) c += g < LQ / 4 + 1;
    return c;
}
__host__ __device__ constexpr int stream_frag_cnt(int LQ, int s)
{
    int c = 0;
    for (int g = 2 * s; g < 2 * s + 2; ++g) c += g < LQ / 4;
    return c;
}
__host__ __device__ constexpr int stream_small_batch(int LQ, int NL, int PD, int k)
{
    const int NST = (LQ / 4 + 2) / 2;
    if (!stream_lds(LQ, NL).small || k + PD < NST) return 0;
    const int nsw = (NL - 1) * 32, per = (nsw + PD - 1) / PD, done = per * (k + PD - NST);
    return done >= nsw ? 0 : (nsw - done < per ? nsw - done : per);
}
__host__ __device__ constexpr int stream_vg(int LQ, int NL, int k)
{
    const int NST = (LQ / 4 + 2) / 2;
    if (stream_lds(LQ, NL).small) return k == NST - 1 ? 8 : 0;
    const int nv = (NL - 1) * 32 + 8;
    const int per = (nv + NST - 1) / NST, done = per * k;
    return done >= nv ? 0 : (nv - done < per ? nv - done : per);
}
__host__ __device__ constexpr int stream_allow(int LQ, int NL, int PD, int s)
{
    const int NST = (LQ / 4 + 2) / 2;
    int total = 0, last = 0;
    for (int k = 0; k < PD && k < NST; ++k) { total += 4 * stream_frag_cnt(LQ, k); if (k == s) last = total; }
    for (int k = 0; k < PD && k < NST; ++k) { total += 4 * stream_row_cnt(LQ, k); if (k == s) last = total; }
    for (int it = 0; it < s; ++it) {
        if (it + PD < NST) {
            total += 4 * stream_row_cnt(LQ, it + PD) + 4 * stream_frag_cnt(LQ, it + PD);
            if (it + PD == s) last = total;
        } else {
            total += stream_small_batch(LQ, NL, PD, it);
        }
    }
    return total - last;
}

template <int N>
__device__ __forceinline__ void stream_wait_vm()
{
    static_assert(N >= 0 && N < 64, "vmcnt is a 6-bit counter");
    asm volatile("s_waitcnt vmcnt(%0)" ::"n"(N) : "memory");
}
__device__ __forceinline__ void stream_barrier() { asm volatile("s_barrier" ::: "memory"); }
#pragma clang diagnostic push
#pragma clang diagnostic ignored "-Winline-asm"
__device__ __forceinline__ void stream_dma(const float* g, unsigned lds_byte)
{
    asm volatile("s_mov_b32 m0, %0\n\tglobal_load_lds_dwordx4 %1, off" ::"s"(lds_byte), "v"(g) : "memory", "m0");
}
__device__ __forceinline__ void stream_dma_dword(const float* g, unsigned lds_byte)
{
    asm volatile("s_mov_b32 m0, %0\n\tglobal_load_lds_dword %1, off" ::"s"(lds_byte), "v"(g) : "memory", "m0");
}
#pragma clang diagnostic pop
template <int... Is, class F>
__device__ __forceinline__ void stream_for_impl(std::integer_sequence<int, Is...>, F&& f)
{
    (f(std::integral_constant<int, Is>{}), ...);
}
template <int N, class F>
__device__ __forceinline__ void stream_for(F&& f)
{
    stream_for_impl(std::make_integer_sequence<int, N>{}, f);
}

constexpr int TAIL_PLAIN = 1;
constexpr int STREAM_PD = 3;

constexpr int STREAM_THREADS = WAVE_THREADS + 64;

#ifdef LBDRN_STAMP_DW
#define SE(k) do { if ((k) == 9) STAMP(0); } while (0)
#define SD(k) STAMP(k)
#else
#define SE(k) STAMP(k)
#define SD(k)
#endif

template <int M, int R, int S>
__device__ __forceinline__ void stream_deal()
{
    constexpr int RR = R < M ? R : M;
#pragma unroll
    for (int k = 0; k < RR; ++k) {
        __builtin_amdgcn_sched_group_barrier(0x008, 1, 0);
        __builtin_amdgcn_sched_group_barrier(0x100, 1, 0);
    }
    constexpr int left = M - RR, per = S > 0 ? (left / (S + 1) > 0 ? left / (S + 1) : 1) : 0;
#pragma unroll
    for (int k = 0; k < S; ++k) {
        __builtin_amdgcn_sched_group_barrier(0x008, per, 0);
        __builtin_amdgcn_sched_group_barrier(0x040, 1, 0);
    }
    if constexpr (left - S * per > 0) __builtin_amdgcn_sched_group_barrier(0x008, left - S * per, 0);
    __builtin_amdgcn_sched_barrier(0);
}

__device__ __forceinline__ float stream_sum8(float x)
{
    x += __int_as_float(__builtin_amdgcn_update_dpp(0, __float_as_int(x), 0x112, 0xf, 0xf, true));
    x += __int_as_float(__builtin_amdgcn_update_dpp(0, __float_as_int(x), 0x114, 0xf, 0xf, true));
    x += __int_as_float(__builtin_amdgcn_update_dpp(0, __float_as_int(x), 0x118, 0xf, 0xf, true));
    return x;
}
__device__ __forceinline__ f32x4 stream_join(const f32x4& even, const f32x4& odd)
{
    f32x4 g = {even[0] + odd[0], even[1] + odd[1], even[2] + odd[2], even[3] + odd[3]};
    return g;
}

template <int LQ, int NL, int PD, int NT0C, int ACT>
__global__ void __launch_bounds__(STREAM_THREADS, 1) k_train_stream(TrainArgs A)
{
    extern __shared__ __attribute__((aligned(16))) float lds[];
    const TrainPlan& p = A.p;
    const TrainFit& F = A.fit[blockIdx.y];
    constexpr int G0 = LQ / 4, NGR = G0 + 1, NST = (NGR + 1) / 2, WPX = stream_wpx(LQ), RPM = stream_rp(LQ);
    constexpr int HP = SHP, OP = SOP, PT = WPT;
    constexpr StreamLds L = stream_lds(LQ, NL);
    constexpr bool SMALL = L.small != 0;
    constexpr int NH = (NL - 1) * 16;
    static_assert(L.total * 4 <= 160 * 1024, "LDS map does not fit");
    const int tid = threadIdx.x, lane = tid & 63;
    const int w = __builtin_amdgcn_readfirstlane(tid >> 6);
    const int i = lane & 15, q = lane >> 4;
    const int C = A.net.C;
    float* Xs = lds + L.x;
    const float* ST = lds + L.stage;
    float* H0 = lds + L.h0;
    float* red = lds + L.red;
    float* ZT = lds + L.zt;
    float* Zo = lds + L.zo;
    auto Hl = [&](int l) -> float* { return l == 0 ? H0 : lds + L.h1 + (size_t)(l - 1) * SHSZ; };
    const unsigned lds0 = (unsigned)(size_t)(__attribute__((address_space(3))) void*)lds;
    const int wg = blockIdx.x, first = wg * WB;
    const int nvalid = min(WB, A.batch_n - first);
    const int srow = 16 * w + i;
    float* slab = F.slabs + (size_t)wg * p.slab_floats;
    const WtBuf slabw(slab, (size_t)p.slab_floats * 4);
    if (w == 4) {
        const float* fsrc = F.packed + p.pk_w0 + lane * 4;
        auto issue_frags = [&](int s) {
#pragma unroll
            for (int g = 2 * s; g < 2 * s + 2; ++g)
                if (g < G0)
#pragma unroll
                    for (int t = 0; t < 4; ++t) stream_dma(fsrc + 256 * (t * G0 + g), lds0 + 4u * (unsigned)(L.stage + (g * 4 + t) * 256));
        };
        if (A.batch_n >= 2) {
            const int64_t* isrc = F.perm + min(first + 2 * (lane & 31), A.batch_n - 2);
            stream_dma(reinterpret_cast<const float*>(isrc), lds0 + 4u * (unsigned)L.idx);
        } else {
            stream_dma_dword(reinterpret_cast<const float*>(F.perm) + (lane & 1), lds0 + 4u * (unsigned)L.idx);
        }
        stream_for<PD>([&](auto s_) { if (decltype(s_)::value < NST) issue_frags(decltype(s_)::value); });
        {
            constexpr int up = 4 * (stream_frag_cnt(LQ, 0) + (PD > 1 ? stream_frag_cnt(LQ, 1) : 0) + (PD > 2 ? stream_frag_cnt(LQ, 2) : 0) +
                                    (PD > 3 ? stream_frag_cnt(LQ, 3) : 0));
            static_assert(PD <= 4, "prefetch depth");
            stream_wait_vm<up>();
        }
        int64_t raw;
        {
            const int g = min(first + lane, A.batch_n - 1), l = (g - first) >> 1;
            raw = reinterpret_cast<const int64_t*>(lds + L.idx)[2 * l + (g - max(min(first + 2 * l, A.batch_n - 2), 0))];
        }
        const int pix = (int)(raw < 0 ? 0 : (raw >= A.npix ? A.npix - 1 : raw));
        const float* rsrc[4];
#pragma unroll
        for (int v = 0; v < 4; ++v) rsrc[v] = F.rows + (size_t)__shfl(pix, 16 * v + (lane >> 2)) * RPM + 4 * (lane & 3);
        auto issue_rows = [&](int s) {
#pragma unroll
            for (int g = 2 * s; g < 2 * s + 2; ++g)
                if (g < NGR)
#pragma unroll
                    for (int v = 0; v < 4; ++v) stream_dma(rsrc[v] + 16 * g, lds0 + 4u * (unsigned)(L.x + v * WPX + g * SGP));
        };
        stream_for<PD>([&](auto s_) { if (decltype(s_)::value < NST) issue_rows(decltype(s_)::value); });
        auto issue_small = [&](int k) {
            constexpr int nsw = 2 * NH, per = (nsw + PD - 1) / PD;
            const int b = k + PD - NST;
#pragma unroll
            for (int u = 0; u < per; ++u) {
                const int j = b * per + u;
                if (j < NH) stream_dma(F.packed + p.pk_wh + lane * 4 + 256 * j, lds0 + 4u * (unsigned)(L.wh + 256 * j));
                else if (j < nsw) stream_dma(F.packed + p.pk_wht + lane * 4 + 256 * (j - NH), lds0 + 4u * (unsigned)(L.wht + 256 * (j - NH)));
            }
        };
        stream_for<NST>([&](auto s_) {
            constexpr int s = decltype(s_)::value;
            stream_wait_vm<stream_allow(LQ, NL, PD, s)>();
            stream_barrier();
            if (s + PD < NST) { issue_rows(s + PD); issue_frags(s + PD); }
            else if (SMALL) issue_small(s);
        });
        stream_wait_vm<0>();
        stream_barrier();
        if (A.next_n > 0) {
            const long long t = F.perm[A.batch_n + min(first + lane, A.next_n - 1)];
            const int touch_bytes = min(A.touch_row_bytes, RPM * 4);
            if (touch_bytes > 0) {
                const int pn = (int)(t < 0 ? 0 : (t >= A.npix ? A.npix - 1 : t));
                const float* rn = F.rows + (size_t)pn * RPM;
                float acc = 0.f;
#pragma unroll
                for (int k = 0; k < 7; ++k) acc += rn[min(128 * k, touch_bytes - 4) / 4];
                asm volatile("" ::"v"(acc));
            } else {
                asm volatile("" ::"v"(t));
            }
        }
        return;
    }
#ifdef LBDRN_TRAIN_STAMPS
    unsigned long long stamp[16] = {};
    asm volatile("s_memrealtime %0\n\ts_waitcnt lgkmcnt(0)" : "=s"(stamp[14])::"memory");
#endif
#ifdef LBDRN_TIMELINE
    if (lane == 0 && w == 0 && wg == 0 && blockIdx.y == 0) timeline_store(A.tl, 0, false);
#endif
    SE(0);

    f32x4 bias[NL][4];
#pragma unroll
    for (int l = 0; l < NL; ++l)
#pragma unroll
        for (int t = 0; t < 4; ++t) {
            const float4 b4 = *reinterpret_cast<const float4*>(F.params + p.offB[l] + 16 * t + 4 * q);
            bias[l][t][0] = b4.x; bias[l][t][1] = b4.y; bias[l][t][2] = b4.z; bias[l][t][3] = b4.w;
        }
    f32x4 bias_last;
#pragma unroll
    for (int r = 0; r < 4; ++r) bias_last[r] = (4 * q + r) < C ? F.params[p.offB[NL] + 4 * q + r] : 0.0f;
    SE(1);

    const __amdgpu_buffer_rsrc_t wrs = __builtin_amdgcn_make_buffer_rsrc(const_cast<float*>(F.packed), (short)0,
                                                                         p.pack_floats * 4, 0x00020000);
    const int lane16 = lane * 16;
    auto ldw = [&](int float_base, int block) -> float4 {
        const v4i32 x = __builtin_amdgcn_raw_buffer_load_b128(wrs, lane16, float_base * 4 + block * 1024, 0);
        return make_float4(__int_as_float(x[0]), __int_as_float(x[1]), __int_as_float(x[2]), __int_as_float(x[3]));
    };
    float4 wh[NL > 1 ? NL - 1 : 1][4][4];
    float4 wl[4];
    float4 wlt[4];
    float4 wht[NL > 1 ? NL - 1 : 1][4][4];
    auto vg_load = [&](int j) {
        constexpr int NHV = SMALL ? 0 : NH;
        if (j < NHV) wh[j / 16][(j >> 2) & 3][j & 3] = ldw(p.pk_wh, j);
        else if (j < 2 * NHV) { const int k = j - NHV; wht[k / 16][(k >> 2) & 3][k & 3] = ldw(p.pk_wht, k); }
        else if (j < 2 * NHV + 4) wl[j - 2 * NHV] = ldw(p.pk_wl, j - 2 * NHV);
        else if (j < 2 * NHV + 8) wlt[j - 2 * NHV - 4] = ldw(p.pk_wlt, j - 2 * NHV - 4);
    };

    f32x4 acc[4];
#pragma unroll
    for (int t = 0; t < 4; ++t) acc[t] = bias[0][t];
    {
        const float* wbase = ST + lane * 4;
        const float* xbase = Xs + w * WPX + (i * 4 + q) * 4;
        float4 aq[2][4], bq[2];
        auto reads = [&](int g) {
#pragma unroll
            for (int t = 0; t < 4; ++t) aq[g & 1][t] = *reinterpret_cast<const float4*>(wbase + (g * 4 + t) * 256);
            bq[g & 1] = *reinterpret_cast<const float4*>(xbase + g * SGP);
        };
        auto mfmas = [&](int g) {
            const float bx[4] = {bq[g & 1].x, bq[g & 1].y, bq[g & 1].z, bq[g & 1].w};
#pragma unroll
            for (int e = 0; e < 4; ++e)
#pragma unroll
                for (int t = 0; t < 4; ++t) {
                    const float4 x = aq[g & 1][t];
                    acc[t] = MFMA16(e == 0 ? x.x : e == 1 ? x.y : e == 2 ? x.z : x.w, bx[e], acc[t]);
                }
        };
        int vgj = 0;
        stream_for<NST>([&](auto s_) {
            constexpr int s = decltype(s_)::value;
            stream_barrier();
#ifdef LBDRN_TRAIN_STAMPS
            if (s == 0) { SE(1); SE(2); }
#endif
#pragma unroll
            for (int u = 0; u < stream_vg(LQ, NL, s); ++u) vg_load(vgj + u);
            vgj += stream_vg(LQ, NL, s);
            __builtin_amdgcn_sched_barrier(0);
#pragma unroll
            for (int g = 2 * s; g < 2 * s + 2; ++g)
                if (g < G0) {
                    reads(g);
                    if (g > 0) {
                        mfmas(g - 1);
#pragma unroll
                        for (int k = 0; k < 5; ++k) {
                            __builtin_amdgcn_sched_group_barrier(0x100, 1, 0);
                            __builtin_amdgcn_sched_group_barrier(0x008, 2, 0);
                        }
                        __builtin_amdgcn_sched_group_barrier(0x008, 6, 0);
                    }
                    __builtin_amdgcn_sched_barrier(0);
                }
        });
        mfmas(G0 - 1);
        __builtin_amdgcn_sched_barrier(0);
    }
    SE(3);
    float h[4][4];
    f32x4 cs[NL][4];
    auto activate_tile = [&](int l, int t) {
#pragma unroll
        for (int r = 0; r < 4; ++r) {
            float sn, co;
            train_act<ACT>(acc[t][r], sn, co);
            h[t][r] = sn;
            cs[l][t][r] = co;
        }
        *reinterpret_cast<float4*>(Hl(l) + srow * HP + 16 * w + 16 * t + 4 * q) = make_float4(h[t][0], h[t][1], h[t][2], h[t][3]);
    };
    auto activate = [&](int l) {
#pragma unroll
        for (int t = 0; t < 4; ++t) activate_tile(l, t);
    };
    activate_tile(0, 0);
    activate_tile(0, 1);
    __builtin_amdgcn_sched_barrier(0);
    stream_barrier();
    SE(4);
    if constexpr (SMALL) {
#pragma unroll
        for (int l = 1; l < NL; ++l)
#pragma unroll
            for (int j = 0; j < 16; ++j)
                wh[l - 1][j >> 2][j & 3] = *reinterpret_cast<const float4*>(lds + L.wh + ((l - 1) * 16 + j) * 256 + lane * 4);
    }
    activate_tile(0, 2);
    activate_tile(0, 3);
    SE(5);

#pragma unroll
    for (int l = 1; l < NL; ++l) {
#pragma unroll
        for (int t = 0; t < 4; ++t) acc[t] = bias[l][t];
#pragma unroll
        for (int tk = 0; tk < 4; ++tk) {
#pragma unroll
            for (int r = 0; r < 4; ++r)
#pragma unroll
                for (int to = 0; to < 4; ++to) {
                    const float4 x = wh[l - 1][to][tk];
                    const float a = r == 0 ? x.x : r == 1 ? x.y : r == 2 ? x.z : x.w;
                    acc[to] = MFMA16(a, h[tk][r], acc[to]);
                }
        }
        if constexpr (SMALL) {
            if (l == NL - 1) {
                asm volatile("s_waitcnt lgkmcnt(0)" ::: "memory");
                stream_barrier();
            }
        }
        activate(l);
    }
    if constexpr (SMALL) {
#pragma unroll
        for (int l = 1; l < NL; ++l)
#pragma unroll
            for (int j = 0; j < 16; ++j)
                wht[l - 1][j >> 2][j & 3] = *reinterpret_cast<const float4*>(lds + L.wht + ((l - 1) * 16 + j) * 256 + lane * 4);
    }
    SE(6);

    float dzo[4];
    {
        f32x4 oe = bias_last, oo = {0.f, 0.f, 0.f, 0.f};
#pragma unroll
        for (int tk = 0; tk < 4; ++tk) {
            const float4 x = wl[tk];
            oe = MFMA16(x.x, h[tk][0], oe);
            oo = MFMA16(x.y, h[tk][1], oo);
            oe = MFMA16(x.z, h[tk][2], oe);
            oo = MFMA16(x.w, h[tk][3], oo);
        }
        const bool live = srow < nvalid;
        const float4 lab = *reinterpret_cast<const float4*>(Xs + w * WPX + G0 * SGP + (i * 4 + q) * 4);
        const float labv[4] = {lab.x, lab.y, lab.z, lab.w};
        float lsum = 0.0f;
#pragma unroll
        for (int r = 0; r < 4; ++r) {
            const bool ok = live && (4 * q + r) < C;
            const float y = train_sigmoid(oe[r] + oo[r]);
            const float d = y - ((4 * q + r) < C ? labv[r] : 0.0f);
            lsum += ok ? d * d : 0.0f;
            dzo[r] = ok ? ((2.0f * d) * A.inv) * (y * (1.0f - y)) : 0.0f;
        }
        *reinterpret_cast<float4*>(Zo + srow * OP + 16 * w + 4 * q) = make_float4(dzo[0], dzo[1], dzo[2], dzo[3]);
        {
            const int li = __float_as_int(stream_sum8(lsum));
            auto rl = [&](int l) { return __int_as_float(__builtin_amdgcn_readlane(li, l)); };
            const float l0 = (rl(14) + rl(30)) + (rl(46) + rl(62)), l1 = (rl(15) + rl(31)) + (rl(47) + rl(63));
            if (lane == 0) { red[w] = l0; red[4 + w] = l1; }
        }
        float bs[4];
#pragma unroll
        for (int r = 0; r < 4; ++r) bs[r] = stream_sum8(dzo[r]);
        if (i >= 14) *reinterpret_cast<float4*>(red + 8 + 64 * (i - 14) + 16 * w + 4 * q) = make_float4(bs[0], bs[1], bs[2], bs[3]);
    }
    SE(7);

    float dz[4][4];
    auto backprop = [&](int l) {
#pragma unroll
        for (int t = 0; t < 4; ++t)
#pragma unroll
            for (int r = 0; r < 4; ++r) {
                dz[t][r] = train_act_back<ACT>(acc[t][r], cs[l][t][r]);
                ZT[(size_t)l * SZTSZ + (16 * t + 4 * q + r) * PT + srow] = dz[t][r];
            }
    };
    {
        const f32x4 zero = {0.f, 0.f, 0.f, 0.f};
#pragma unroll
        for (int t = 0; t < 4; ++t) acc[t] = zero;
#pragma unroll
        for (int s = 0; s < 4; ++s)
#pragma unroll
            for (int t = 0; t < 4; ++t) {
                const float4 x = wlt[t];
                const float a = s == 0 ? x.x : s == 1 ? x.y : s == 2 ? x.z : x.w;
                acc[t] = MFMA16(a, dzo[s], acc[t]);
            }
        backprop(NL - 1);
    }
    auto ldrow = [&](const float* row, float (&dst)[16]) {
#pragma unroll
        for (int g = 0; g < 4; ++g) {
            const float4 x = *reinterpret_cast<const float4*>(row + 4 * g);
            dst[4 * g] = x.x; dst[4 * g + 1] = x.y; dst[4 * g + 2] = x.z; dst[4 * g + 3] = x.w;
        }
    };
    auto ldx = [&](int nt, float (&dst)[16]) {
        const int f = 16 * nt + i;
        const int kq = f / LQ, fl = f - kq * LQ;
        const float* base = Xs + q * WPX + (fl >> 2) * SGP + kq * 4 + (fl & 3);
#pragma unroll
        for (int s = 0; s < 16; ++s) dst[s] = base[16 * s];
    };
    auto ldh = [&](const float* H, int strip, float (&dst)[16]) {
        const float* base = H + (16 * q) * HP + 16 * q + 16 * strip + i;
#pragma unroll
        for (int s = 0; s < 16; ++s) dst[s] = base[s * HP];
    };
    auto put = [&](int off, const f32x4& g, bool early) {
        if (early) slabw.store(off + lane * 4, g[0], g[1], g[2], g[3]);
        else slabw.store_plain(off + lane * 4, g[0], g[1], g[2], g[3]);
    };
    const f32x4 zero4 = {0.f, 0.f, 0.f, 0.f};
    if constexpr (NT0C > 0) {
        static_assert(NL == 2, "the straight-line schedule is written for two hidden layers");
        constexpr int NFS = NT0C / 4, REM = NT0C % 4;
        static_assert(NFS >= 1 && NFS <= 4 && REM <= 2, "strip counts of the shapes this is instantiated for");
        constexpr int NIT = NFS + REM;
        const float* ZT1 = ZT + SZTSZ;
        __syncthreads();
        float ao[16], bo[16], bh[16], a1[4][16];
        {
            const float* base = Zo + (16 * q) * OP + 16 * q + i;
#pragma unroll
            for (int s = 0; s < 16; ++s) ao[s] = base[s * OP];
        }
        ldh(Hl(1), w, bo);
        ldh(Hl(0), w, bh);
        ldrow(ZT1 + (0 + i) * PT + 16 * q, a1[0]);
        ldrow(ZT1 + (16 + i) * PT + 16 * q, a1[1]);
        {
            const f32x4 zero = {0.f, 0.f, 0.f, 0.f};
#pragma unroll
            for (int t = 0; t < 4; ++t) acc[t] = zero;
#pragma unroll
            for (int to = 0; to < 4; ++to)
#pragma unroll
                for (int r = 0; r < 4; ++r)
#pragma unroll
                    for (int ti = 0; ti < 4; ++ti) {
                        const float4 x = wht[0][ti][to];
                        const float a = r == 0 ? x.x : r == 1 ? x.y : r == 2 ? x.z : x.w;
                        acc[ti] = MFMA16(a, dz[to][r], acc[ti]);
                    }
            stream_deal<64, 56, 0>();
            backprop(0);
        }
        SE(8);
        __syncthreads();
        if (tid == 0) F.loss_part[wg] = (((double)red[0] + (double)red[1]) + ((double)red[2] + (double)red[3])) +
                                        (((double)red[4] + (double)red[5]) + ((double)red[6] + (double)red[7]));
        SE(9);
        float az[4][16], azw[16], a1w[16], bb[NFS][16], br[REM > 0 ? REM : 1][16];
        auto item = [&](auto n_) {
            constexpr int n = decltype(n_)::value;
            if constexpr (n < NFS) ldx(w + 4 * n, bb[n]);
            else if constexpr (n < NIT) ldx(4 * NFS + (n - NFS), br[n - NFS]);
        };
        ldrow(ZT1 + (32 + i) * PT + 16 * q, a1[2]);
        ldrow(ZT1 + (48 + i) * PT + 16 * q, a1[3]);
#pragma unroll
        for (int t = 0; t < 4; ++t) ldrow(ZT + (16 * t + i) * PT + 16 * q, az[t]);
        item(std::integral_constant<int, 0>{});
        f32x4 go[2] = {zero4, zero4}, g1[4][2] = {{zero4, zero4}, {zero4, zero4}, {zero4, zero4}, {zero4, zero4}};
#pragma unroll
        for (int s = 0; s < 16; ++s) {
            go[s & 1] = MFMA16(ao[s], bo[s], go[s & 1]);
            g1[0][s & 1] = MFMA16(a1[0][s], bh[s], g1[0][s & 1]);
            g1[1][s & 1] = MFMA16(a1[1][s], bh[s], g1[1][s & 1]);
        }
        stream_deal<48, 40, 0>();
        item(std::integral_constant<int, 1>{});
        ldrow(ZT + (16 * w + i) * PT + 16 * q, azw);
        ldrow(ZT1 + (16 * w + i) * PT + 16 * q, a1w);
#pragma unroll
        for (int s = 0; s < 16; ++s) {
            g1[2][s & 1] = MFMA16(a1[2][s], bh[s], g1[2][s & 1]);
            g1[3][s & 1] = MFMA16(a1[3][s], bh[s], g1[3][s & 1]);
        }
        put(p.sl_out + w * 256, stream_join(go[0], go[1]), true);
        put(p.sl_hid + (0 * 4 + w) * 256, stream_join(g1[0][0], g1[0][1]), true);
        put(p.sl_hid + (1 * 4 + w) * 256, stream_join(g1[1][0], g1[1][1]), true);
        stream_deal<32, (NIT > 1 ? 24 : 8), 3>();
        SD(1);
        f32x4 gs[2][4][2];
        stream_for<NFS>([&](auto k_) {
            constexpr int k = decltype(k_)::value;
#pragma unroll
            for (int t = 0; t < 4; ++t) gs[k & 1][t][0] = gs[k & 1][t][1] = zero4;
            constexpr int nreads = k + 2 < NIT ? 16 : 0;
            item(std::integral_constant<int, k + 2>{});
#pragma unroll
            for (int s = 0; s < 16; ++s)
#pragma unroll
                for (int t = 0; t < 4; ++t) gs[k & 1][t][s & 1] = MFMA16(az[t][s], bb[k][s], gs[k & 1][t][s & 1]);
            if constexpr (k == 0) {
                put(p.sl_hid + (2 * 4 + w) * 256, stream_join(g1[2][0], g1[2][1]), true);
                put(p.sl_hid + (3 * 4 + w) * 256, stream_join(g1[3][0], g1[3][1]), true);
                stream_deal<64, nreads, 2>();
            } else {
#pragma unroll
                for (int t = 0; t < 4; ++t)
                    put((t * NT0C + w + 4 * (k - 1)) * 256, stream_join(gs[(k - 1) & 1][t][0], gs[(k - 1) & 1][t][1]), k - 1 < NFS - TAIL_PLAIN);
                stream_deal<64, nreads, 4>();
            }
#ifdef LBDRN_STAMP_DW
            if (k == 0) { SD(2); stamp[3] = stamp[2]; } else if (k == 1) { SD(4); stamp[5] = stamp[4]; } else if (k == 2) { SD(6); stamp[7] = stamp[6]; }
#endif
        });
        f32x4 grem[REM > 0 ? REM : 1][2];
#pragma unroll
        for (int r = 0; r < (REM > 0 ? REM : 1); ++r) grem[r][0] = grem[r][1] = zero4;
        if constexpr (REM > 0) {
#pragma unroll
            for (int s = 0; s < 16; ++s)
#pragma unroll
                for (int r = 0; r < REM; ++r) grem[r][s & 1] = MFMA16(azw[s], br[r][s], grem[r][s & 1]);
        }
#pragma unroll
        for (int t = 0; t < 4; ++t)
            put((t * NT0C + w + 4 * (NFS - 1)) * 256, stream_join(gs[(NFS - 1) & 1][t][0], gs[(NFS - 1) & 1][t][1]), false);
        stream_deal<REM * 16, 0, 4>();
        {
            float s0[2] = {0.f, 0.f}, s1[2] = {0.f, 0.f};
#pragma unroll
            for (int s = 0; s < 16; ++s) { s0[s & 1] += azw[s]; s1[s & 1] += a1w[s]; }
#pragma unroll
            for (int h = 0; h < 2; ++h) {
                s0[h] += __shfl_xor(s0[h], 16); s1[h] += __shfl_xor(s1[h], 16);
                s0[h] += __shfl_xor(s0[h], 32); s1[h] += __shfl_xor(s1[h], 32);
            }
            if (lane < 16) {
                slab[p.sl_bias + 16 * w + lane] = s0[0] + s0[1];
                slab[p.sl_bias + TBC_W + 16 * w + lane] = s1[0] + s1[1];
            }
        }
        if constexpr (REM > 0) {
#pragma unroll
            for (int r = 0; r < REM; ++r) put((w * NT0C + 4 * NFS + r) * 256, stream_join(grem[r][0], grem[r][1]), false);
        }
#ifdef LBDRN_STAMP_DW
        SD(8); stamp[9] = stamp[8];
#endif
        STAMP(10); STAMP(11);
        if (w == 3 && lane < 16)
            slab[p.sl_bias + NL * TBC_W + lane] = ((red[8 + lane] + red[24 + lane]) + (red[40 + lane] + red[56 + lane])) +
                                                  ((red[72 + lane] + red[88 + lane]) + (red[104 + lane] + red[120 + lane]));
    } else {
    #pragma unroll
        for (int l = NL - 1; l >= 1; --l) {
            const f32x4 zero = {0.f, 0.f, 0.f, 0.f};
    #pragma unroll
// ... 150 lines not shown
```

lbdrn-msic_amd/lbdrn_hip/codec.py:

```python
import collections
import copy
import os
import threading
import time
from concurrent.futures import ThreadPoolExecutor

import numpy as np
import torch

from . import ops
from .features import FeatCfg
from .model import LBDRNModel
from .sampler import DevicePermutationStream, GPU_RANDPERM_MAX, draw_pass_seeds, epoch_plan


def lr_schedule(lr, epochs):
    step = max(1, int(epochs / 3))
    out, cur = [], float(lr)
    for e in range(1, epochs + 1):
        out.append(cur)
        if e % step == 0:
            cur *= 0.1
    return out


def skip_fit_rng(n_feature, base_channel, channels, num_layers, epochs, val_duration=1):
    draw_fit(n_feature, base_channel, channels, num_layers, epochs, val_duration)


class FitDraws:

    def __init__(self, params, train_seeds):
        self.params, self.train_seeds = params, train_seeds


def draw_fit(n_feature, base_channel, channels, num_layers, epochs, val_duration=1):
    model = LBDRNModel(dim_in=n_feature, dim_hidden=base_channel, dim_out=channels, num_layers=num_layers)
    return FitDraws(model.flat_parameters(), draw_pass_seeds(epoch_plan(epochs, val_duration)))


class FitResult:
    def __init__(self):
        self.params = None
        self.best_epoch = -1
        self.best_mse = None
        self.epoch_mse = []
        self.losses = None
        self.msb = None
        self.msb_device = None
        self.msb_max = None
        self.n_feature = None
        self.channels = None
        self.n_subpixels = None
        self.seconds = {}


class DeviceFit:

    def __init__(self):
        self.best_params = None
        self.msb = None
        self.msb_max = None
        self.geom = None
        self.net = None
        self.mse_log = None
        self.evaluated = []
        self.losses = None
        self.epochs = 0


_RNG_LOCK = threading.Lock()
_POOL_LOCK = threading.Lock()
_FIT_STREAMS = {}


def _fit_stream_pool(dev, n):
    with _POOL_LOCK:
        pool_ = _FIT_STREAMS.setdefault(dev, [])
        while len(pool_) < n:
            pool_.append(torch.cuda.Stream(device=dev))
        return pool_


def fast_evaluation():
    return os.environ.get("LBDRN_EVAL_CANONICAL") != "1"


def exact16_evaluation():
    return os.environ.get("LBDRN_EVAL_X16") == "1"


def alone_streams_fit_queues():
    return 3 <= int(os.environ.get("GPU_MAX_HW_QUEUES", "4"))


def overlap_evaluation(dev, alone):
    env = os.environ.get("LBDRN_OVERLAP_EVAL")
    if env in ("0", "1"):
        return env == "1"
    if not alone or device_shared():
        return False
    return alone_streams_fit_queues()


def device_shared():
    return os.environ.get("LBDRN_DEVICE_SHARED", "0") not in ("", "0")


def fit_bytes(C, H, W, K, D, base_channel, num_layers, batch_size, epochs, cfg=None):
    cfg = cfg or FeatCfg.from_constants()
    N = H * W
    g = ops._lib.Geom(C, H, W, K, D, 1, int(cfg.use_colors), int(cfg.relative), int(cfg.P), 0, None, None)
    net = ops.make_net(cfg.feature_dim(C, D), base_channel, C, num_layers, cfg.act)
    L = ops.lib()
    import ctypes
    train = int(L.lbdrn_train_workspace(ctypes.byref(g), ctypes.byref(net), batch_size))
    apply_ws = int(L.lbdrn_apply_workspace(ctypes.byref(g), ctypes.byref(net)))
    perms = epochs * N * 8 + int(L.lbdrn_randperm_workspace(N, min(32, max(epochs - 1, 1))))
    planes = 3 * C * N * 2
    return train + apply_ws + perms + planes + (epochs + 4) * int(ops.param_count(net)) * 4 + (64 << 20)


def default_in_flight(C, H, W, K, D, base_channel, num_layers, cfg=None, path=None):
    cfg = cfg or FeatCfg.from_constants()
    if path == ops._lib.PATH_GENERIC:
        return 4
    if base_channel >= 128:
        return 3
    return 4


def memory_limited_in_flight(images, wanted, K, D, base_channel, num_layers, batch_size, epochs, cfg=None):
    if not images:
        return wanted
    dev = images[0].device
    need = max(fit_bytes(*tuple(t.shape), K, D, base_channel, num_layers, batch_size, epochs, cfg) for t in images)
    free, total = torch.cuda.mem_get_info(dev)
    free += torch.cuda.memory_reserved(dev) - torch.cuda.memory_allocated(dev)
    if device_shared():
        free //= 2
    fits = int(0.85 * free // need)
    if fits < 1:
        raise ops._lib.LbdrnError(f"one fit of this shape holds {need / 2**30:.1f} GiB on the device, {free / 2**30:.1f} GiB are free "
                                  f"(of {total / 2**30:.0f}): split the image (-sr)")
    return max(1, min(wanted, fits))


EVAL_PASS_FRAC_OF_PEAK, HALF_CHIP_STEP_FRAC_OF_PEAK, HALF_CHIP_STEP_OVERHEAD_S, PEAK_FLOPS = 0.65, 0.26, 5.0e-6, 157.3e12
_HEAD_LOCK = threading.Lock()
_HEAD_MEASURED = {}
_HEAD_PENDING = {}


def _head_key(dev, net, n_pixels, batch_size):
    return (dev.index, int(net.F), int(net.bc), int(net.C), int(net.nl), int(net.act), int(n_pixels), int(batch_size))


def _calibrated_head(key, guess, steps_per_epoch):
    with _HEAD_LOCK:
        pend = _HEAD_PENDING.get(key)
        if pend is not None and pend[0][1].query() and pend[0][3].query():
            (p0, p1, h0, h1), head = pend
            del _HEAD_PENDING[key]
            t_pass, t_head = p0.elapsed_time(p1), h0.elapsed_time(h1)
            if t_pass > 0 and t_head > 0 and head > 0:
                _HEAD_MEASURED[key] = int(round(min(max(head * t_pass / t_head, 0.5 * guess), 2.0 * guess)))
        return max(0, min(steps_per_epoch, _HEAD_MEASURED.get(key, guess)))


def head_calibration():
    with _HEAD_LOCK:
        return dict(_HEAD_MEASURED)


def background_steps(steps_per_epoch, net=None, n_pixels=None, batch_size=None):
    env = os.environ.get("LBDRN_LONE_HEAD_FRAC")
    if env is not None:
        return int(round(float(env) * steps_per_epoch))
    if net is None:
        return int(round(0.27 * steps_per_epoch))
    F, bc, C, nl = int(net.F), int(net.bc), int(net.C), int(net.nl)
    fwd = 2 * (F * bc + (nl - 1) * bc * bc + bc * C)
    step = 2 * fwd + 2 * ((nl - 1) * bc * bc + bc * C)
    t_pass = 2.0 * n_pixels * fwd / (EVAL_PASS_FRAC_OF_PEAK * PEAK_FLOPS)
    t_step = min(batch_size, n_pixels) * step / (HALF_CHIP_STEP_FRAC_OF_PEAK * PEAK_FLOPS) + HALF_CHIP_STEP_OVERHEAD_S
    return max(0, min(steps_per_epoch, int(round(t_pass / t_step))))


def _eval_stream(dev, main):
    for s in _fit_stream_pool(dev, 2):
        if s.cuda_stream != main.cuda_stream:
            return s


def fit_device(img_d, K, D, base_channel, num_layers, lr, batch_size, epochs, val_duration=1,
               cfg=None, path=ops.PATH_AUTO, keep_losses=False, seed=None, draws=None, alone=True):
    cfg = cfg or FeatCfg.from_constants()
    out = DeviceFit()
    dev = img_d.device
    C, H, W = img_d.shape
    N = H * W
    alone = alone and not device_shared()
    msb_d, msb_max = ops.split_bits(img_d, K)
    geom = ops.FeatureGeometry(C, H, W, K, D, msb_max, cfg, dev)
    if N >= GPU_RANDPERM_MAX:
        raise ops._lib.LbdrnError(
            f"{N} pixels in one fit: torch.randperm switches algorithm at 2^32/20 elements and lbdrn_randperm "
            "implements the Fisher-Yates branch only; split the image (-sr) -- there is no host fallback")
    if draws is None:
        with _RNG_LOCK:
            if seed is not None:
                torch.manual_seed(seed)
            draws = draw_fit(geom.F, base_channel, C, num_layers, epochs, val_duration)
    stream = DevicePermutationStream(N, epochs, val_duration, dev, train_seeds=draws.train_seeds)
    net = ops.make_net(geom.F, base_channel, C, num_layers, cfg.act)
    params = draws.params.to(dev).contiguous()
    if params.numel() != ops.param_count(net):
        raise ValueError("draws were made for another network shape")
    draws_params0 = params.clone()
    exp_avg = torch.zeros_like(params)
    exp_avg_sq = torch.zeros_like(params)
    lrs = lr_schedule(lr, epochs)
    steps_per_epoch = (N + batch_size - 1) // batch_size
    losses = torch.zeros((epochs, steps_per_epoch), dtype=torch.float32, device=dev) if keep_losses else None
    train_ws = ops.TrainWorkspace(geom, net, batch_size, dev).prepare(img_d, msb_d, path)
    apply_ws = ops.ApplyWorkspace(geom, net, dev)
    mse_log = torch.zeros((epochs, 2), dtype=torch.float32, device=dev)
    eval_epochs = [] if epochs == 1 else [e for e in range(1, epochs + 1) if e % min(val_duration, epochs) == 0]
    main = torch.cuda.current_stream(dev)
    side = _eval_stream(dev, main) if len(eval_epochs) > 1 and overlap_evaluation(dev, alone) else None
    snaps = torch.empty((max(len(eval_epochs), 1), params.numel()), dtype=torch.float32, device=dev)
    mses = torch.zeros((max(len(eval_epochs), 1),), dtype=torch.float32, device=dev)
    if side is not None:
        side.wait_stream(main)
    adam_steps = 0
    hkey = _head_key(dev, net, N, batch_size)
    cal_epoch = eval_epochs[0] if eval_epochs else 0
    cal_events = [torch.cuda.Event(enable_timing=True) for _ in range(4)] if (side is not None and alone and cal_epoch + 1 <= epochs) else None
    try:
        for e in range(1, epochs + 1):
            perm = stream.get(e).to(dev, non_blocking=True)
            head = 0
            if side is not None and alone and e - 1 in eval_epochs:
                head = background_steps(steps_per_epoch, net, N, batch_size)
                if "LBDRN_LONE_HEAD_FRAC" not in os.environ:
                    head = _calibrated_head(hkey, head, steps_per_epoch)
            for lo, hi, hint in ((0, head, False), (head, steps_per_epoch, alone)):
                if hi > lo:
                    timed = cal_events is not None and lo == 0 and head > 0 and e == cal_epoch + 1
                    if timed:
                        cal_events[2].record(main)
                    ops.train_epoch(geom, net, img_d, msb_d, perm[lo * batch_size:hi * batch_size], batch_size, params, exp_avg,
                                    exp_avg_sq, adam_steps + lo, lrs[e - 1], losses[e - 1][lo:hi] if keep_losses else None, path,
                                    train_ws, alone=hint)
                    if timed:
                        cal_events[3].record(main)
                        with _HEAD_LOCK:
                            _HEAD_PENDING[hkey] = (cal_events, head)
            adam_steps += steps_per_epoch
            if e in eval_epochs:
                k = eval_epochs.index(e)
                snaps[k].copy_(params)
                if side is not None:
                    side.wait_stream(main)
                with torch.cuda.stream(side if side is not None else main):
# ... 394 lines not shown
```

Baseline: 69.12 Mpixels/s.

## Store relative-MSB training rows as packed fp16 integer differences

Adds a compact row format for relative color features. The MSB neighbour differences are stored as unscaled integer values in fp16 pairs, which halves the per-pixel row footprint and the DMA and LDS traffic in the stream and split training kernels. The 1/max scaling moves into an FMA applied after the first-layer MFMA and into the weight-gradient reduction, using a hi/lo split of the inverse to keep precision. This adds new template instances, reworks the schedule barriers, and relies on fp16 holding the integer differences exactly, hence the msb_max <= 2047 guard.

```diff
diff --git a/lbdrn-msic_amd/csrc/cabi.hip b/lbdrn-msic_amd/csrc/cabi.hip
--- a/lbdrn-msic_amd/csrc/cabi.hip
+++ b/lbdrn-msic_amd/csrc/cabi.hip
@@ -339,7 +339,7 @@
     for (int f = 0; f < count; ++f)
         if (int rc = workspace_fits("train", workspace[f], workspace_bytes, lbdrn_train_workspace(g[f], net, batch_size))) return rc;
     if (count > 1 && path != LBDRN_PATH_GENERIC && mfma_train_supported(*g[0], *net, batch_size)) {
-        const int rc = mfma_train_epoch_group(count, *g[0], *net, perm, n, batch_size, params, exp_avg, exp_avg_sq,
+        const int rc = mfma_train_epoch_group(count, g, *net, perm, n, batch_size, params, exp_avg, exp_avg_sq,
                                               adam_step0, lr, losses, workspace, workspace_bytes, (hipStream_t)stream, false);
         if (rc != LBDRN_E_UNSUPPORTED) return rc;
     }
diff --git a/lbdrn-msic_amd/csrc/common.hpp b/lbdrn-msic_amd/csrc/common.hpp
--- a/lbdrn-msic_amd/csrc/common.hpp
+++ b/lbdrn-msic_amd/csrc/common.hpp
@@ -106,7 +106,7 @@
                   const uint16_t* msb, const float* params, double* sse, void* ws, size_t ws_bytes,
                   bool background, bool fast, bool x16, hipStream_t s);
 
-int mfma_train_epoch_group(int count, const lbdrn_geom& g, const lbdrn_net& net, const int64_t* const* perm, int64_t n,
+int mfma_train_epoch_group(int count, const lbdrn_geom* const* g, const lbdrn_net& net, const int64_t* const* perm, int64_t n,
                            int bs, float* const* params, float* const* m, float* const* v, int64_t step0, double lr,
                            float* const* losses, void* const* ws, size_t ws_bytes, hipStream_t s, bool alone);
 
diff --git a/lbdrn-msic_amd/csrc/train_mfma.hip b/lbdrn-msic_amd/csrc/train_mfma.hip
--- a/lbdrn-msic_amd/csrc/train_mfma.hip
+++ b/lbdrn-msic_amd/csrc/train_mfma.hip
@@ -72,6 +72,7 @@
     int wave_lds_floats;
     int sl_hid, sl_out, sl_bias, slab_floats;
     int lds_x, lds_xt, lds_h, lds_ht, lds_z, lds_zt, lds_zo, lds_zot, lds_pix, lds_red, lds_floats;
+    int compact;
 };
 
 #define STREAM_INSTANCES(X) \
@@ -98,8 +99,12 @@
 constexpr int tile_lq(int F, int RP, int nl) { TILE_INSTANCES(X) return 0; }
 #undef X
 
-__host__ __device__ constexpr int stream_rp(int LQ);
-static int stream_lds_total(int LQ, int NL);
+__host__ __device__ constexpr int stream_rp(int LQ, int CR);
+static int stream_lds_total(int LQ, int NL, int CR);
+
+constexpr int compact_nt0c(int lq) { return lq == 48 ? 12 : lq == 24 ? 6 : 0; }
+constexpr bool COMPACT_ROWS_SELECTED = true;
+constexpr int COMPACT_MSB_MAX = 2047;
 
 static bool make_train_plan(const lbdrn_geom& g, const lbdrn_net& net, TrainPlan* out)
 {
@@ -113,8 +118,11 @@
         if (!p.LQ && net.nl == 2 && p.fm.Fe <= 4 * SPLIT_WIDE_LQ) p.LQ = SPLIT_WIDE_LQ;
         if (!p.LQ) return false;
         p.NT0 = p.LQ == SPLIT_WIDE_LQ ? split_nt0c(SPLIT_WIDE_LQ) : (p.fm.Fe + 15) / 16;
-        p.RP = stream_rp(p.LQ);
-        p.wave_lds_floats = p.LQ == SPLIT_WIDE_LQ ? 0 : stream_lds_total(p.LQ, net.nl);
+        p.compact = COMPACT_ROWS_SELECTED && g.use_colors && g.relative && g.P == 0 && g.D > 0 && g.msb_max >= 1 &&
+                    g.msb_max <= COMPACT_MSB_MAX && net.nl == 2 && p.LQ != SPLIT_WIDE_LQ && compact_nt0c(p.LQ) == p.NT0 &&
+                    p.fm.zs2 > 0 && p.fm.Fe == 4 * p.LQ;
+        p.RP = stream_rp(p.LQ, p.compact);
+        p.wave_lds_floats = p.LQ == SPLIT_WIDE_LQ ? 0 : stream_lds_total(p.LQ, net.nl, p.compact);
     } else {
         p.fm = FeatMap{net.F, 0, 0, 0};
         p.RP = (net.F + net.C + 3) / 4 * 4;
@@ -122,6 +130,7 @@
         if (!p.LQ) return false;
         p.NT0 = (net.F + 15) / 16;
         p.wave_lds_floats = 0;
+        p.compact = 0;
     }
     p.XP = 4 * p.LQ + 4;
     p.NP = param_count(net);
@@ -168,12 +177,12 @@
 static bool wide_supported(const lbdrn_geom& g, const lbdrn_net& net);
 static size_t wide_workspace(const lbdrn_geom& g, const lbdrn_net& net, int bs);
 
-static bool slabs_addressable(const TrainPlan& p, int bs);
+static bool slabs_addressable(const TrainPlan& p, size_t rows);
 
 bool mfma_train_supported(const lbdrn_geom& g, const lbdrn_net& net, int bs)
 {
     TrainPlan p;
-    if (make_train_plan(g, net, &p)) return bs <= 0 || slabs_addressable(p, bs);
+    if (make_train_plan(g, net, &p)) return bs <= 0 || slabs_addressable(p, (size_t)bs);
     return wide_supported(g, net);
 }
 
@@ -194,7 +203,7 @@
     size_t o = 0;
     L.off_rows = o; o += align_up((size_t)g.H * g.W * p.RP * sizeof(float), 256);
     L.off_pack = o; o += align_up((size_t)p.pack_floats * sizeof(float), 256);
-    const size_t nwg = std::max((size_t)(bs + TB - 1) / TB, 2 * ((size_t)(bs + WB - 1) / WB));
+    const size_t nwg = std::max(((size_t)bs + TB - 1) / TB, 2 * (((size_t)bs + WB - 1) / WB));
     L.slab_bytes = align_up(nwg * (size_t)p.slab_floats * sizeof(float), 256);
     L.off_slab = o; o += SLAB_ROT * L.slab_bytes;
     L.off_loss = o; o += align_up(nwg * sizeof(double), 256);
@@ -205,9 +214,9 @@
     return L;
 }
 
-static bool slabs_addressable(const TrainPlan& p, int bs)
-{
-    const size_t nwg = std::max((size_t)(bs + TB - 1) / TB, 2 * ((size_t)(bs + WB - 1) / WB));
+static bool slabs_addressable(const TrainPlan& p, size_t rows)
+{
+    const size_t nwg = std::max((rows + TB - 1) / TB, 2 * ((rows + WB - 1) / WB));
     return nwg * (size_t)p.slab_floats * sizeof(float) < ((size_t)1 << 31);
 }
 
@@ -231,14 +240,43 @@
     return ch < C ? F + ch : -1;
 }
 
+__device__ __forceinline__ int compact_source(int hpos, int LQs, const FeatMap& fm)
+{
+    return feat_of_slot(((hpos >> 3) & 3) * LQs + 8 * (hpos >> 5) + (hpos & 7), fm);
+}
+__device__ __forceinline__ unsigned half_bits(float x) { return __builtin_bit_cast(unsigned short, (_Float16)x); }
+
 __global__ void __launch_bounds__(256)
-    k_build_rows(lbdrn_geom g, int F, int RP, int LQs, FeatMap fm, const uint16_t* __restrict__ msb,
+    k_build_rows(lbdrn_geom g, int F, int RP, int LQs, int compact, FeatMap fm, const uint16_t* __restrict__ msb,
                  const uint16_t* __restrict__ img, float* __restrict__ rows)
 {
     const int64_t HW = (int64_t)g.H * g.W;
     const int64_t e = (int64_t)blockIdx.x * blockDim.x + threadIdx.x;
     if (e >= HW * RP) return;
     const int64_t pix = e / RP;
+    if (compact) {
+        const int pos = (int)(e - pix * RP);
+        const int y = (int)(pix / g.W), x = (int)(pix - (int64_t)y * g.W);
+        const int side = 2 * g.D + 1;
+        float v = 0.0f;
+        if (pos < 2 * LQs) {
+            unsigned bits = 0;
+            for (int h = 0; h < 2; ++h) {
+                const int cf = compact_source(2 * pos + h, LQs, fm);
+                const int c = cf / (side * side), r = cf - c * side * side;
+                const int dy = r / side, dx = r - dy * side;
+                const uint16_t* pl = msb + (int64_t)c * HW;
+                const int yy = reflect_fast(y + dy - g.D, g.H), xx = reflect_fast(x + dx - g.D, g.W);
+                bits |= half_bits((float)((int)pl[(int64_t)yy * g.W + xx] - (int)pl[pix])) << (16 * h);
+            }
+            v = __uint_as_float(bits);
+        } else if (pos - 2 * LQs < g.C) {
+            const int mask = (1 << g.K) - 1;
+            v = (float)((int)img[(int64_t)(pos - 2 * LQs) * HW + pix] & mask) / (float)mask;
+        }
+        rows[e] = v;
+        return;
+    }
     const int f = row_source((int)(e - pix * RP), LQs, F, g.C, fm);
     const int y = (int)(pix / g.W), x = (int)(pix - (int64_t)y * g.W);
     float v = 0.0f;
@@ -267,7 +305,7 @@
 
 constexpr int BR_TW = 32;
 __global__ void __launch_bounds__(256)
-    k_build_rows_tiled(lbdrn_geom g, int F, int RP, int LQs, FeatMap fm, const uint16_t* __restrict__ msb,
+    k_build_rows_tiled(lbdrn_geom g, int F, int RP, int LQs, int compact, FeatMap fm, const uint16_t* __restrict__ msb,
                        const uint16_t* __restrict__ img, float* __restrict__ rows)
 {
     extern __shared__ float br_lds[];
@@ -288,7 +326,8 @@
             const int c = e / (side * SW), r = e - c * side * SW;
             const int sy = r / SW, sx = r - sy * SW;
             const int yy = reflect_fast(y + sy - g.D, g.H), xx = reflect_fast(min(x0 + sx - g.D, g.W - 1 + g.D), g.W);
-            tile[e] = (float)msb[(int64_t)c * HW + (int64_t)yy * g.W + xx] / mx;
+            const float m = (float)msb[(int64_t)c * HW + (int64_t)yy * g.W + xx];
+            tile[e] = compact ? m : m / mx;
         }
         for (int k = tid; k < ncolor; k += 256) {
             const int c = k / (side * side), r = k - c * side * side;
@@ -299,8 +338,9 @@
     }
     __syncthreads();
     const bool rel = g.relative && g.D > 0;
+    const int npos = compact ? 4 * LQs + 16 : RP;
     int2* ptab = reinterpret_cast<int2*>(cto + ncolor);
-    float* labs = reinterpret_cast<float*>(ptab + RP);
+    float* labs = reinterpret_cast<float*>(ptab + npos);
     {
         const int lmask = (1 << g.K) - 1;
         const float lmaskf = (float)lmask;
@@ -309,8 +349,9 @@
             labs[e] = (float)((int)img[(int64_t)c * HW + (int64_t)y * g.W + min(x0 + px, g.W - 1)] & lmask) / lmaskf;
         }
     }
-    for (int pos = tid; pos < RP; pos += 256) {
-        const int f = row_source(pos, LQs, F, g.C, fm);
+    for (int pos = tid; pos < npos; pos += 256) {
+        const int f = !compact ? row_source(pos, LQs, F, g.C, fm)
+                               : pos < 4 * LQs ? compact_source(pos, LQs, fm) : pos - 4 * LQs < g.C ? F + (pos - 4 * LQs) : -1;
         int2 t = make_int2(-1, 0);
         if (f < 0) {
         } else if (f < g.P) t = make_int2(-2, f);
@@ -332,7 +373,27 @@
         if (t.x == -3) return g.coltab[(int64_t)(x0 + pix) * g.P + t.y];
         return labs[t.y * BR_TW + pix];
     };
-    if ((RP & 3) == 0) {
+    if (compact) {
+        const int RQ = RP >> 2, NQ = LQs >> 1;
+        int pix = tid / RQ, pq = tid - pix * RQ;
+        const int dp = 256 / RQ, dq = 256 - dp * RQ;
+        while (pix < tw) {
+            float4 v;
+            if (pq < NQ) {
+                unsigned b[4];
+#pragma unroll
+                for (int k = 0; k < 4; ++k) b[k] = half_bits(value(8 * pq + 2 * k, pix)) | (half_bits(value(8 * pq + 2 * k + 1, pix)) << 16);
+                v = make_float4(__uint_as_float(b[0]), __uint_as_float(b[1]), __uint_as_float(b[2]), __uint_as_float(b[3]));
+            } else {
+                const int pos = 4 * LQs + 4 * (pq - NQ);
+                v = make_float4(value(pos, pix), value(pos + 1, pix), value(pos + 2, pix), value(pos + 3, pix));
+            }
+            *reinterpret_cast<float4*>(out + (int64_t)pix * RP + 4 * pq) = v;
+            pix += dp;
+            pq += dq;
+            if (pq >= RQ) { pq -= RQ; pix += 1; }
+        }
+    } else if ((RP & 3) == 0) {
         const int RQ = RP >> 2;
         int pix = tid / RQ, pq = tid - pix * RQ;
         const int dp = 256 / RQ, dq = 256 - dp * RQ;
@@ -432,7 +493,7 @@
     if (e >= p.slab_floats) return;
     int64_t idx = e < p.sl_bias + nl * TBC + 16 ? slab_to_param(e, p, F, nl, C) : -1;
     const int2 pos = idx >= 0 ? frag_pos(idx, p, F, nl, C) : make_int2(-1, -1);
-    map[e] = make_int4((int)idx, pos.x, pos.y, 0);
+    map[e] = make_int4((int)idx, pos.x, pos.y, (p.compact && e < p.sl_hid && idx >= 0) ? 1 : 0);
 }
 
 constexpr int RED_AUX = 0x00;
@@ -452,6 +513,7 @@
     float *params, *m, *v, *packed;
     const double* loss_part;
     float* loss_out;
+    float inv_max, inv_max_lo;
 };
 struct ReduceArgs {
     ReduceFit fit[MAX_GROUP];
@@ -528,6 +590,7 @@
         float g = part[0][threadIdx.x];
 #pragma unroll
         for (int s = 1; s < RED_SLICES; ++s) g += part[s][threadIdx.x];
+        if (me.w) g = __builtin_fmaf(g, F.inv_max, g * F.inv_max_lo);
         const float w1c = (float)(1.0 - 0.9), b2 = 0.999f, w2c = (float)(1.0 - 0.999), eps = 1e-8f;
         float mi = pm + w1c * (g - pm);
         float vi = pv * b2 + w2c * (g * g);
@@ -566,6 +629,7 @@
     const float* packed;
     float* slabs;
     double* loss_part;
+    float inv_max, inv_max_lo;
 };
 struct TrainArgs {
     lbdrn_net net;
@@ -979,10 +1043,11 @@
 
 #include "train_stream.inc"
 
-static int stream_lds_total(int LQ, int NL) { return stream_lds(LQ, NL).total; }
+static int stream_lds_total(int LQ, int NL, int CR) { return stream_lds(LQ, NL, CR).total; }
 #define X(LQ, NL, NT0C) static_assert(stream_lds(LQ, NL).total * 4 <= 160 * 1024, "k_train_stream's LDS map passes 160 KB");
 STREAM_INSTANCES(X)
 #undef X
+static_assert(stream_lds(48, 2, 1).total <= stream_lds(48, 2).total && stream_lds(24, 2, 1).total <= stream_lds(24, 2).total, "compact rows take less LDS");
 
 #include "train_split.inc"
 
@@ -1021,10 +1086,10 @@
     return 0;
 }
 
-template <int LQ, int NL, int NT0C, int ACT>
+template <int LQ, int NL, int NT0C, int CR, int ACT>
 static int launch_stream(const TrainArgs& A, int nwg, int count, hipStream_t s)
 {
-    auto kern = k_train_stream<LQ, NL, STREAM_PD, NT0C, ACT>;
+    auto kern = k_train_stream<LQ, NL, STREAM_PD, NT0C, ACT, CR>;
     static std::atomic<unsigned long long> configured{0};
     if (int rc = configure_lds_once(kern, A.p.wave_lds_floats * 4, configured)) return rc;
     kern<<<dim3((unsigned)nwg, (unsigned)count), STREAM_THREADS, (size_t)A.p.wave_lds_floats * 4, s>>>(A);
@@ -1032,11 +1097,11 @@
     return 0;
 }
 
-template <int LQ, int NT0C, int ACT>
+template <int LQ, int NT0C, int CR, int ACT>
 static int launch_split(const TrainArgs& A, int nwg, int count, hipStream_t s)
 {
-    auto kern = k_train_split<LQ, NT0C, ACT>;
-    constexpr int bytes = split_lds(LQ).total * 4;
+    auto kern = k_train_split<LQ, NT0C, ACT, CR>;
+    constexpr int bytes = split_lds(LQ, CR).total * 4;
     static std::atomic<unsigned long long> configured{0};
     if (int rc = configure_lds_once(kern, bytes, configured)) return rc;
     kern<<<dim3((unsigned)nwg, (unsigned)count), WAVE_THREADS, (size_t)bytes, s>>>(A);
@@ -1056,9 +1121,18 @@
     const int nl = A.net.nl, nt0c = stream_nt0c(p.LQ, nl, p.NT0);
     const bool relu = A.net.act == LBDRN_ACT_RELU;
 #define ACTS(launch, ...) return relu ? launch<__VA_ARGS__, LBDRN_ACT_RELU>(A, nwg, count, s) : launch<__VA_ARGS__, LBDRN_ACT_SINE>(A, nwg, count, s);
-#define SPLIT(lq, c) if (split && p.LQ == lq && p.NT0 == c) ACTS(launch_split, lq, c)
-#define STREAM(lq, n, c) if (!split && p.wave == STEP_STREAM && p.LQ == lq && nl == n && nt0c == c) ACTS(launch_stream, lq, n, c)
+#define SPLIT(lq, c) if (split && p.LQ == lq && p.NT0 == c) ACTS(launch_split, lq, c, 0)
+#define STREAM(lq, n, c) if (!split && p.wave == STEP_STREAM && p.LQ == lq && nl == n && nt0c == c) ACTS(launch_stream, lq, n, c, 0)
 #define TILE(lq, n) if (!split && p.wave == STEP_TILE && p.LQ == lq && nl == n) return launch_train<lq, n>(A, nwg, s);
+    if (p.compact) {
+        static_assert(compact_nt0c(48) == 12 && compact_nt0c(24) == 6, "the compact instances below");
+        if (split && p.LQ == 48) ACTS(launch_split, 48, 12, 1)
+        if (split && p.LQ == 24) ACTS(launch_split, 24, 6, 1)
+        if (!split && p.LQ == 48) ACTS(launch_stream, 48, 2, 12, 1)
+        if (!split && p.LQ == 24) ACTS(launch_stream, 24, 2, 6, 1)
+        set_error("no compact-row step is built for LQ = %d", p.LQ);
+        return LBDRN_E_UNSUPPORTED;
+    }
     SPLIT_INSTANCES(SPLIT) STREAM_INSTANCES(STREAM) TILE_INSTANCES(TILE)
 #undef ACTS
 #undef SPLIT
@@ -1074,6 +1148,7 @@
     TrainPlan p;
     size_t need = 0, off_rows = 0;
     int LQs = 0;
+    p.compact = 0;
     if (make_train_plan(g, net, &p)) {
         const TrainWsLayout L = train_ws_layout(g, net, p, bs);
         need = L.total; off_rows = L.off_rows;
@@ -1098,22 +1173,23 @@
     LBDRN_REQUIRE((total + 255) / 256 < ((int64_t)1 << 31), "image too large for one launch");
     const int side = 2 * g.D + 1;
     const size_t ncol = (size_t)std::max(net.F - 2 * g.P, 0);
-    const size_t tile_lds = ((size_t)g.C * side * (BR_TW + 2 * g.D) + 2 * ncol + 2 * (size_t)p.RP + (size_t)g.C * BR_TW) * 4;
+    const size_t tile_lds = ((size_t)g.C * side * (BR_TW + 2 * g.D) + 2 * ncol + 2 * (size_t)(p.compact ? 4 * p.LQ + 16 : p.RP) + (size_t)g.C * BR_TW) * 4;
     const int64_t nblk = (int64_t)g.H * ((g.W + BR_TW - 1) / BR_TW);
     if (tile_lds <= 48 * 1024 && g.D < g.H && g.D < g.W && nblk < ((int64_t)1 << 31)) {
-        k_build_rows_tiled<<<(unsigned)nblk, 256, tile_lds, s>>>(g, net.F, p.RP, LQs, p.fm, msb, img, rows);
+        k_build_rows_tiled<<<(unsigned)nblk, 256, tile_lds, s>>>(g, net.F, p.RP, LQs, p.compact, p.fm, msb, img, rows);
     } else {
-        k_build_rows<<<(unsigned)((total + 255) / 256), 256, 0, s>>>(g, net.F, p.RP, LQs, p.fm, msb, img, rows);
+        k_build_rows<<<(unsigned)((total + 255) / 256), 256, 0, s>>>(g, net.F, p.RP, LQs, p.compact, p.fm, msb, img, rows);
     }
     LBDRN_LAUNCH_CHECK();
     return 0;
 }
 
 
-int mfma_train_epoch_group(int count, const lbdrn_geom& g, const lbdrn_net& net, const int64_t* const* perm, int64_t n,
+int mfma_train_epoch_group(int count, const lbdrn_geom* const* geoms, const lbdrn_net& net, const int64_t* const* perm, int64_t n,
                            int bs, float* const* params, float* const* m, float* const* v, int64_t step0, double lr,
                            float* const* losses, void* const* ws, size_t ws_bytes, hipStream_t s, bool alone)
 {
+    const lbdrn_geom& g = *geoms[0];
     TrainArgs A;
     if (!make_train_plan(g, net, &A.p)) {
         if (count != 1) { set_error("groups of fits run on the bc = 64 fused step only"); return LBDRN_E_UNSUPPORTED; }
@@ -1124,7 +1200,14 @@
         set_error("a group of %d fits is not supported by this shape's train kernel", count);
         return LBDRN_E_UNSUPPORTED;
     }
-    if (!slabs_addressable(A.p, bs)) {
+    for (int f = 1; f < count; ++f) {
+        TrainPlan pf;
+        if (!make_train_plan(*geoms[f], net, &pf) || pf.compact != A.p.compact) {
+            set_error("the fits of a group differ in their row order (fit %d: msb_max %d)", f, geoms[f]->msb_max);
+            return LBDRN_E_UNSUPPORTED;
+        }
+    }
+    if (!slabs_addressable(A.p, (size_t)bs)) {
         set_error("minibatch of %d rows: one step's gradient slabs pass 2 GiB, the fused step does not address them", bs);
         return LBDRN_E_UNSUPPORTED;
     }
@@ -1145,6 +1228,11 @@
         A.fit[f].slabs = (float*)((char*)ws[k] + L.off_slab);
         A.fit[f].loss_part = (double*)((char*)ws[k] + L.off_loss);
         A.fit[f].perm = perm[k];
+        {
+            const double inv = A.p.compact ? 1.0 / (double)geoms[k]->msb_max : 1.0;
+            A.fit[f].inv_max = R.fit[f].inv_max = (float)inv;
+            A.fit[f].inv_max_lo = R.fit[f].inv_max_lo = (float)(inv - (double)(float)inv);
+        }
         R.fit[f].slabs = A.fit[f].slabs; R.fit[f].params = params[k]; R.fit[f].m = m[k]; R.fit[f].v = v[k];
         R.fit[f].packed = packed; R.fit[f].loss_part = A.fit[f].loss_part; R.fit[f].loss_out = nullptr;
         if (f < count) {
@@ -1295,7 +1383,8 @@
                      float* m, float* v, int64_t step0, double lr, float* losses, void* ws,
                      size_t ws_bytes, hipStream_t s, bool alone)
 {
-    return mfma_train_epoch_group(1, g, net, &perm, n, bs, &params, &m, &v, step0, lr, &losses, &ws, ws_bytes, s, alone);
-}
-
-}
+    const lbdrn_geom* gp = &g;
+    return mfma_train_epoch_group(1, &gp, net, &perm, n, bs, &params, &m, &v, step0, lr, &losses, &ws, ws_bytes, s, alone);
+}
+
+}
diff --git a/lbdrn-msic_amd/csrc/train_split.inc b/lbdrn-msic_amd/csrc/train_split.inc
--- a/lbdrn-msic_amd/csrc/train_split.inc
+++ b/lbdrn-msic_amd/csrc/train_split.inc
@@ -10,15 +10,15 @@
 __host__ __device__ constexpr int split_small_through(int k, int SPI) { return k * SPI < SP_SM / 4 ? k * SPI : SP_SM / 4; }
 
 struct SplitLds { int w0, sm, x, xt, h0, red, idx, bias, h1, e, zo, zt, total; };
-__host__ __device__ constexpr SplitLds split_lds(int LQ)
+__host__ __device__ constexpr SplitLds split_lds(int LQ, int CR = 0)
 {
     SplitLds L{};
-    const int G0 = LQ / 4, RG = split_w0_groups(LQ);
+    const int RG = split_w0_groups(LQ);
     int o = 0;
     const int over = 2 * SPB * SP_HP + SPB * SP_OP + 2 * 64 * SP_PT;
     L.w0 = o; o += RG * 4 * 256 > over ? RG * 4 * 256 : over;
     L.sm = o; o += SP_SM * 256;
-    L.xt = (G0 + 1) * SGP + 16;
+    L.xt = stream_groups(LQ, CR) * SGP + 16;
     L.x = o; o += 2 * L.xt;
     L.h0 = o; o += SPB * SP_HP;
     L.red = o; o += 4 + 4 * 16 + 12;
@@ -50,14 +50,14 @@
     return c;
 }
 
-template <int LQ, int NT0C, int ACT>
+template <int LQ, int NT0C, int ACT, int CR>
 __global__ void __launch_bounds__(WAVE_THREADS, 1) k_train_split(TrainArgs A)
 {
     extern __shared__ __attribute__((aligned(16))) float lds[];
     const TrainPlan& p = A.p;
     const TrainFit& F = A.fit[blockIdx.y];
-    constexpr int NL = 2, G0 = LQ / 4, NGR = G0 + 1, HP = SP_HP, OP = SP_OP, PT = SP_PT, RPM = stream_rp(LQ);
-    constexpr SplitLds L = split_lds(LQ);
+    constexpr int NL = 2, G0 = LQ / 4, HP = SP_HP, OP = SP_OP, PT = SP_PT, RPM = stream_rp(LQ, CR);
+    constexpr SplitLds L = split_lds(LQ, CR);
     static_assert(L.total > 0 && L.total * 4 <= 160 * 1024, "LDS map does not fit");
     static_assert(16 * NT0C == 4 * LQ && G0 >= 4, "the first layer's strips fill its slots");
     constexpr int NFS = NT0C / 4, REM = NT0C % 4, NIT = NFS + REM, GA = split_w0_groups(LQ) / 2;
@@ -66,6 +66,8 @@
     constexpr bool RING = split_ring(LQ);
     constexpr int RG = split_w0_groups(LQ), HR = RG / 2, W0B = RG - GA;
     static_assert(!RING || (G0 == 2 * RG && GA == HR), "the ring holds half of W_0, its quarters land one behind the other");
+    constexpr int NGR = stream_groups(LQ, CR), GAR = CR ? (GA + 1) / 2 : GA;
+    static_assert(!CR || (!RING && LQ % 8 == 0), "compact rows: the shapes of make_train_plan");
     const int tid = threadIdx.x, lane = tid & 63;
     const int wv = __builtin_amdgcn_readfirstlane(tid >> 6);
     const int st = wv >> 1, uh = wv & 1;
@@ -141,9 +143,9 @@
         for (int g = g_lo; g < g_hi; ++g)
             if ((g & 1) == uh) stream_dma(rsrc + 16 * g, lds0 + 4u * (unsigned)(L.x + st * L.xt + g * SGP));
     };
-    row_requests(0, GA);
+    row_requests(0, GAR);
     w0_requests(GA, RG);
-    row_requests(GA, NGR);
+    row_requests(GAR, NGR);
     auto small_request = [&](int b) {
         const int blk = 4 * b + wv;
         const int src = blk < 16 ? p.pk_wh + 256 * blk : blk < 32 ? p.pk_wht + 256 * (blk - 16) : blk < 36 ? p.pk_wl + 256 * (blk - 32) : p.pk_wlt + 256 * (blk - 36);
@@ -152,7 +154,7 @@
     long long touched = 0;
     if (A.next_n > 0 && wv == 0 && lane < 8) touched = F.perm[A.batch_n + min(grp * WB + 8 * lane, A.next_n - 1)];
     STAMP(1);
-    constexpr int ROWS_B0 = split_row_requests(GA, NGR, 0), ROWS_B1 = split_row_requests(GA, NGR, 1);
+    constexpr int ROWS_B0 = split_row_requests(GAR, NGR, 0), ROWS_B1 = split_row_requests(GAR, NGR, 1);
     if (uh == 0) stream_wait_vm<W0B + ROWS_B0>(); else stream_wait_vm<W0B + ROWS_B1>();
     stream_barrier();
     STAMP(2);
@@ -172,21 +174,35 @@
         bias_last[0] = 4 * q + 0 < C ? l4.x : 0.0f; bias_last[1] = 4 * q + 1 < C ? l4.y : 0.0f;
         bias_last[2] = 4 * q + 2 < C ? l4.z : 0.0f; bias_last[3] = 4 * q + 3 < C ? l4.w : 0.0f;
     }
-    f32x4 acc[2] = {bias0[0], bias0[1]};
+    const f32x4 zero0 = {0.f, 0.f, 0.f, 0.f};
+    f32x4 acc[2] = {CR ? zero0 : bias0[0], CR ? zero0 : bias0[1]};
     {
         const float* wbase = W0s + t0 * 256 + lane * 4;
         const float* xbase = Xs + st * L.xt + (4 * split_slot(i) + q) * 4;
         float4 aq[2][2], bq[2];
+        h16x8 xq[2];
         auto reads = [&](int g) {
             aq[g & 1][0] = *reinterpret_cast<const float4*>(wbase + (g % RG) * 1024);
             aq[g & 1][1] = *reinterpret_cast<const float4*>(wbase + (g % RG) * 1024 + 256);
-            bq[g & 1] = *reinterpret_cast<const float4*>(xbase + g * SGP);
+            if constexpr (CR) {
+                if ((g & 1) == 0) xq[(g >> 1) & 1] = *reinterpret_cast<const h16x8*>(xbase + (g >> 1) * SGP);
+            } else {
+                bq[g & 1] = *reinterpret_cast<const float4*>(xbase + g * SGP);
+            }
         };
         auto mfmas = [&](int g) {
+            float bx[4];
+            if constexpr (CR) {
+#pragma unroll
+                for (int e = 0; e < 4; ++e) bx[e] = (float)xq[(g >> 1) & 1][4 * (g & 1) + e];
+            } else {
+#pragma unroll
+                for (int e = 0; e < 4; ++e) bx[e] = sel4(bq[g & 1], e);
+            }
 #pragma unroll
             for (int e = 0; e < 4; ++e)
 #pragma unroll
-                for (int tt = 0; tt < 2; ++tt) acc[tt] = MFMA16(sel4(aq[g & 1][tt], e), sel4(bq[g & 1], e), acc[tt]);
+                for (int tt = 0; tt < 2; ++tt) acc[tt] = MFMA16(sel4(aq[g & 1][tt], e), bx[e], acc[tt]);
         };
         reads(0);
 #pragma unroll
@@ -216,18 +232,34 @@
                 if (b < SP_SM / 4) small_request(b);
             reads(g);
             mfmas(g - 1);
-#pragma unroll
-            for (int k = 0; k < 3; ++k) {
-                __builtin_amdgcn_sched_group_barrier(0x100, 1, 0);
+            if (CR && (g & 1)) {
+#pragma unroll
+                for (int k = 0; k < 2; ++k) {
+                    __builtin_amdgcn_sched_group_barrier(0x100, 1, 0);
+                    __builtin_amdgcn_sched_group_barrier(0x008, 2, 0);
+                }
+                __builtin_amdgcn_sched_group_barrier(0x008, 4, 0);
+            } else {
+#pragma unroll
+                for (int k = 0; k < 3; ++k) {
+                    __builtin_amdgcn_sched_group_barrier(0x100, 1, 0);
+                    __builtin_amdgcn_sched_group_barrier(0x008, 2, 0);
+                }
                 __builtin_amdgcn_sched_group_barrier(0x008, 2, 0);
             }
-            __builtin_amdgcn_sched_group_barrier(0x008, 2, 0);
             __builtin_amdgcn_sched_barrier(0);
         }
         mfmas(G0 - 1);
         __builtin_amdgcn_sched_barrier(0);
     }
-    const float4 lab = *reinterpret_cast<const float4*>(Xs + st * L.xt + G0 * SGP + (4 * split_slot(i) + q) * 4);
+    if constexpr (CR) {
+        const float inv_max = F.inv_max, inv_lo = F.inv_max_lo;
+#pragma unroll
+        for (int tt = 0; tt < 2; ++tt)
+#pragma unroll
+            for (int r = 0; r < 4; ++r) acc[tt][r] = __builtin_fmaf(acc[tt][r], inv_max, __builtin_fmaf(acc[tt][r], inv_lo, bias0[tt][r]));
+    }
+    const float4 lab = *reinterpret_cast<const float4*>(Xs + st * L.xt + (NGR - 1) * SGP + (4 * split_slot(i) + q) * 4);
     STAMP(3);
     float hf[4][4];
     f32x4 cs[NL][2];
@@ -358,6 +390,12 @@
     auto ldx = [&](int nt, float (&dst)[8]) {
         const int f = 16 * nt + i;
         const int kq = f / LQ, fl = f - kq * LQ;
+        if constexpr (CR) {
+            const _Float16* base = reinterpret_cast<const _Float16*>(Xs + (q >> 1) * L.xt + (fl >> 3) * SGP) + kq * 8 + (fl & 7);
+#pragma unroll
+            for (int j = 0; j < 8; ++j) dst[j] = (float)base[32 * split_slot(4 * (q & 1) + (j & 3) + 8 * (j >> 2))];
+            return;
+        }
         const float* base = Xs + (q >> 1) * L.xt + (fl >> 2) * SGP + kq * 4 + (fl & 3);
 #pragma unroll
         for (int j = 0; j < 8; ++j) dst[j] = base[16 * split_slot(4 * (q & 1) + (j & 3) + 8 * (j >> 2))];
diff --git a/lbdrn-msic_amd/csrc/train_stream.inc b/lbdrn-msic_amd/csrc/train_stream.inc
--- a/lbdrn-msic_amd/csrc/train_stream.inc
+++ b/lbdrn-msic_amd/csrc/train_stream.inc
@@ -1,9 +1,10 @@
 constexpr int SGP = 260;
-__host__ __device__ constexpr int stream_groups(int LQ) { return LQ / 4 + 1; }
-__host__ __device__ constexpr int stream_rp(int LQ) { return 16 * stream_groups(LQ); }
-__host__ __device__ constexpr int stream_wpx(int LQ)
-{
-    const int n = stream_groups(LQ) * SGP;
+typedef _Float16 h16x8 __attribute__((ext_vector_type(8)));
+__host__ __device__ constexpr int stream_groups(int LQ, int CR = 0) { return (CR ? LQ / 8 : LQ / 4) + 1; }
+__host__ __device__ constexpr int stream_rp(int LQ, int CR) { return 16 * stream_groups(LQ, CR); }
+__host__ __device__ constexpr int stream_wpx(int LQ, int CR = 0)
+{
+    const int n = stream_groups(LQ, CR) * SGP;
     return n + ((16 - n % 32) + 32) % 32;
 }
 constexpr int SHP = 68, SOP = 20;
@@ -13,12 +14,12 @@
 
 constexpr int SRED = 8 + 2 * 64;
 struct StreamLds { int x, stage, h0, red, h1, zo, zt, wh, wht, idx, total, small; };
-__host__ __device__ constexpr StreamLds stream_lds(int LQ, int NL)
+__host__ __device__ constexpr StreamLds stream_lds(int LQ, int NL, int CR = 0)
 {
     StreamLds L{};
     const int G0 = LQ / 4, NST = (G0 + 2) / 2;
     L.x = 0;
-    L.stage = 4 * stream_wpx(LQ);
+    L.stage = 4 * stream_wpx(LQ, CR);
     const int stage_end = L.stage + 4 * G0 * 256;
     const bool alias = 2 * (NST - 1) - 1 >= (SHSZ + SRED + 1023) / 1024 - 1;
     int r = alias ? L.stage + ((SHSZ + SRED + 3) & ~3) : L.stage;
@@ -45,8 +46,9 @@
     return L;
 }
 
-__host__ __device__ constexpr int stream_row_cnt(int LQ, int s)
-{
+__host__ __device__ constexpr int stream_row_cnt(int LQ, int s, int CR = 0)
+{
+    if (CR) return s < stream_groups(LQ, CR) ? 1 : 0;
     int c = 0;
     for (int g = 2 * s; g < 2 * s + 2; ++g) c += g < LQ / 4 + 1;
     return c;
@@ -57,33 +59,33 @@
     for (int g = 2 * s; g < 2 * s + 2; ++g) c += g < LQ / 4;
     return c;
 }
-__host__ __device__ constexpr int stream_small_batch(int LQ, int NL, int PD, int k)
+__host__ __device__ constexpr int stream_small_batch(int LQ, int NL, int PD, int k, int CR = 0)
 {
     const int NST = (LQ / 4 + 2) / 2;
-    if (!stream_lds(LQ, NL).small || k + PD < NST) return 0;
+    if (!stream_lds(LQ, NL, CR).small || k + PD < NST) return 0;
     const int nsw = (NL - 1) * 32, per = (nsw + PD - 1) / PD, done = per * (k + PD - NST);
     return done >= nsw ? 0 : (nsw - done < per ? nsw - done : per);
 }
-__host__ __device__ constexpr int stream_vg(int LQ, int NL, int k)
+__host__ __device__ constexpr int stream_vg(int LQ, int NL, int k, int CR = 0)
 {
     const int NST = (LQ / 4 + 2) / 2;
-    if (stream_lds(LQ, NL).small) return k == NST - 1 ? 8 : 0;
+    if (stream_lds(LQ, NL, CR).small) return k == NST - 1 ? 8 : 0;
     const int nv = (NL - 1) * 32 + 8;
     const int per = (nv + NST - 1) / NST, done = per * k;
     return done >= nv ? 0 : (nv - done < per ? nv - done : per);
 }
-__host__ __device__ constexpr int stream_allow(int LQ, int NL, int PD, int s)
+__host__ __device__ constexpr int stream_allow(int LQ, int NL, int PD, int s, int CR = 0)
 {
     const int NST = (LQ / 4 + 2) / 2;
     int total = 0, last = 0;
     for (int k = 0; k < PD && k < NST; ++k) { total += 4 * stream_frag_cnt(LQ, k); if (k == s) last = total; }
-    for (int k = 0; k < PD && k < NST; ++k) { total += 4 * stream_row_cnt(LQ, k); if (k == s) last = total; }
+    for (int k = 0; k < PD && k < NST; ++k) { total += 4 * stream_row_cnt(LQ, k, CR); if (k == s) last = total; }
     for (int it = 0; it < s; ++it) {
         if (it + PD < NST) {
-            total += 4 * stream_row_cnt(LQ, it + PD) + 4 * stream_frag_cnt(LQ, it + PD);
+            total += 4 * stream_row_cnt(LQ, it + PD, CR) + 4 * stream_frag_cnt(LQ, it + PD);
             if (it + PD == s) last = total;
         } else {
-            total += stream_small_batch(LQ, NL, PD, it);
+            total += stream_small_batch(LQ, NL, PD, it, CR);
         }
     }
     return total - last;
@@ -163,15 +165,16 @@
     return g;
 }
 
-template <int LQ, int NL, int PD, int NT0C, int ACT>
+template <int LQ, int NL, int PD, int NT0C, int ACT, int CR>
 __global__ void __launch_bounds__(STREAM_THREADS, 1) k_train_stream(TrainArgs A)
 {
     extern __shared__ __attribute__((aligned(16))) float lds[];
     const TrainPlan& p = A.p;
     const TrainFit& F = A.fit[blockIdx.y];
-    constexpr int G0 = LQ / 4, NGR = G0 + 1, NST = (NGR + 1) / 2, WPX = stream_wpx(LQ), RPM = stream_rp(LQ);
+    constexpr int G0 = LQ / 4, NGR = G0 + 1, NST = (NGR + 1) / 2, WPX = stream_wpx(LQ, CR), RPM = stream_rp(LQ, CR);
+    static_assert(!CR || (LQ % 8 == 0 && NST == LQ / 8 + 1), "compact rows: a piece is two MFMA groups, the labels a stage of their own");
     constexpr int HP = SHP, OP = SOP, PT = WPT;
-    constexpr StreamLds L = stream_lds(LQ, NL);
+    constexpr StreamLds L = stream_lds(LQ, NL, CR);
     constexpr bool SMALL = L.small != 0;
     constexpr int NH = (NL - 1) * 16;
     static_assert(L.total * 4 <= 160 * 1024, "LDS map does not fit");
@@ -224,6 +227,11 @@
 #pragma unroll
         for (int v = 0; v < 4; ++v) rsrc[v] = F.rows + (size_t)__shfl(pix, 16 * v + (lane >> 2)) * RPM + 4 * (lane & 3);
         auto issue_rows = [&](int s) {
+            if constexpr (CR) {
+#pragma unroll
+                for (int v = 0; v < 4; ++v) stream_dma(rsrc[v] + 16 * s, lds0 + 4u * (unsigned)(L.x + v * WPX + s * SGP));
+                return;
+            }
 #pragma unroll
             for (int g = 2 * s; g < 2 * s + 2; ++g)
                 if (g < NGR)
@@ -243,7 +251,7 @@
         };
         stream_for<NST>([&](auto s_) {
             constexpr int s = decltype(s_)::value;
-            stream_wait_vm<stream_allow(LQ, NL, PD, s)>();
+            stream_wait_vm<stream_allow(LQ, NL, PD, s, CR)>();
             stream_barrier();
             if (s + PD < NST) { issue_rows(s + PD); issue_frags(s + PD); }
             else if (SMALL) issue_small(s);
@@ -309,18 +317,32 @@
 
     f32x4 acc[4];
 #pragma unroll
-    for (int t = 0; t < 4; ++t) acc[t] = bias[0][t];
+    for (int t = 0; t < 4; ++t) {
+        if constexpr (CR) acc[t] = f32x4{0.f, 0.f, 0.f, 0.f};
+        else acc[t] = bias[0][t];
+    }
     {
         const float* wbase = ST + lane * 4;
         const float* xbase = Xs + w * WPX + (i * 4 + q) * 4;
         float4 aq[2][4], bq[2];
+        h16x8 xq[2];
         auto reads = [&](int g) {
 #pragma unroll
             for (int t = 0; t < 4; ++t) aq[g & 1][t] = *reinterpret_cast<const float4*>(wbase + (g * 4 + t) * 256);
-            bq[g & 1] = *reinterpret_cast<const float4*>(xbase + g * SGP);
+            if constexpr (CR) {
+                if ((g & 1) == 0) xq[(g >> 1) & 1] = *reinterpret_cast<const h16x8*>(xbase + (g >> 1) * SGP);
+            } else {
+                bq[g & 1] = *reinterpret_cast<const float4*>(xbase + g * SGP);
+            }
         };
         auto mfmas = [&](int g) {
-            const float bx[4] = {bq[g & 1].x, bq[g & 1].y, bq[g & 1].z, bq[g & 1].w};
+            float bx[4];
+            if constexpr (CR) {
+#pragma unroll
+                for (int e = 0; e < 4; ++e) bx[e] = (float)xq[(g >> 1) & 1][4 * (g & 1) + e];
+            } else {
+                bx[0] = bq[g & 1].x; bx[1] = bq[g & 1].y; bx[2] = bq[g & 1].z; bx[3] = bq[g & 1].w;
+            }
 #pragma unroll
             for (int e = 0; e < 4; ++e)
 #pragma unroll
@@ -337,8 +359,8 @@
             if (s == 0) { SE(1); SE(2); }
 #endif
 #pragma unroll
-            for (int u = 0; u < stream_vg(LQ, NL, s); ++u) vg_load(vgj + u);
-            vgj += stream_vg(LQ, NL, s);
+            for (int u = 0; u < stream_vg(LQ, NL, s, CR); ++u) vg_load(vgj + u);
+            vgj += stream_vg(LQ, NL, s, CR);
             __builtin_amdgcn_sched_barrier(0);
 #pragma unroll
             for (int g = 2 * s; g < 2 * s + 2; ++g)
@@ -346,18 +368,34 @@
                     reads(g);
                     if (g > 0) {
                         mfmas(g - 1);
-#pragma unroll
-                        for (int k = 0; k < 5; ++k) {
-                            __builtin_amdgcn_sched_group_barrier(0x100, 1, 0);
-                            __builtin_amdgcn_sched_group_barrier(0x008, 2, 0);
+                        if (CR && (g & 1)) {
+#pragma unroll
+                            for (int k = 0; k < 4; ++k) {
+                                __builtin_amdgcn_sched_group_barrier(0x100, 1, 0);
+                                __builtin_amdgcn_sched_group_barrier(0x008, 2, 0);
+                            }
+                            __builtin_amdgcn_sched_group_barrier(0x008, 8, 0);
+                        } else {
+#pragma unroll
+                            for (int k = 0; k < 5; ++k) {
+                                __builtin_amdgcn_sched_group_barrier(0x100, 1, 0);
+                                __builtin_amdgcn_sched_group_barrier(0x008, 2, 0);
+                            }
+                            __builtin_amdgcn_sched_group_barrier(0x008, 6, 0);
                         }
-                        __builtin_amdgcn_sched_group_barrier(0x008, 6, 0);
                     }
                     __builtin_amdgcn_sched_barrier(0);
                 }
         });
         mfmas(G0 - 1);
         __builtin_amdgcn_sched_barrier(0);
+    }
+    if constexpr (CR) {
+        const float inv_max = F.inv_max, inv_lo = F.inv_max_lo;
+#pragma unroll
+        for (int t = 0; t < 4; ++t)
+#pragma unroll
+            for (int r = 0; r < 4; ++r) acc[t][r] = __builtin_fmaf(acc[t][r], inv_max, __builtin_fmaf(acc[t][r], inv_lo, bias[0][t][r]));
     }
     SE(3);
     float h[4][4];
@@ -436,7 +474,7 @@
             oo = MFMA16(x.w, h[tk][3], oo);
         }
         const bool live = srow < nvalid;
-        const float4 lab = *reinterpret_cast<const float4*>(Xs + w * WPX + G0 * SGP + (i * 4 + q) * 4);
+        const float4 lab = *reinterpret_cast<const float4*>(Xs + w * WPX + (stream_groups(LQ, CR) - 1) * SGP + (i * 4 + q) * 4);
         const float labv[4] = {lab.x, lab.y, lab.z, lab.w};
         float lsum = 0.0f;
 #pragma unroll
@@ -495,6 +533,12 @@
     auto ldx = [&](int nt, float (&dst)[16]) {
         const int f = 16 * nt + i;
         const int kq = f / LQ, fl = f - kq * LQ;
+        if constexpr (CR) {
+            const _Float16* base = reinterpret_cast<const _Float16*>(Xs + q * WPX + (fl >> 3) * SGP) + kq * 8 + (fl & 7);
+#pragma unroll
+            for (int s = 0; s < 16; ++s) dst[s] = (float)base[32 * s];
+            return;
+        }
         const float* base = Xs + q * WPX + (fl >> 2) * SGP + kq * 4 + (fl & 3);
 #pragma unroll
         for (int s = 0; s < 16; ++s) dst[s] = base[16 * s];
diff --git a/lbdrn-msic_amd/lbdrn_hip/codec.py b/lbdrn-msic_amd/lbdrn_hip/codec.py
--- a/lbdrn-msic_amd/lbdrn_hip/codec.py
+++ b/lbdrn-msic_amd/lbdrn_hip/codec.py
@@ -110,7 +110,7 @@
 def fit_bytes(C, H, W, K, D, base_channel, num_layers, batch_size, epochs, cfg=None):
     cfg = cfg or FeatCfg.from_constants()
     N = H * W
-    g = ops._lib.Geom(C, H, W, K, D, 1, int(cfg.use_colors), int(cfg.relative), int(cfg.P), 0, None, None)
+    g = ops._lib.Geom(C, H, W, K, D, 0, int(cfg.use_colors), int(cfg.relative), int(cfg.P), 0, None, None)
     net = ops.make_net(cfg.feature_dim(C, D), base_channel, C, num_layers, cfg.act)
     L = ops.lib()
     import ctypes
```

Result: slower. 67.84 Mpixels/s (-1.9%).
